# ebu/libear

Hardware: AMD Instinct MI355X
Metric: Msamples/s (higher is better)
Workload: dtype f32 io / f16x2-split MFMA, f32 accumulate

## Files before the change

include/earhip.h:

```cpp
#ifndef EARHIP_H
#define EARHIP_H

#include <stddef.h>
#include <stdint.h>

#ifdef __cplusplus
extern "C" {
#endif

#define EARHIP_VERSION 100

#define EARHIP_OK 0
#define EARHIP_INVALID_ARGUMENT 1
#define EARHIP_INTERNAL_ERROR 2
#define EARHIP_DEVICE_ERROR 3
#define EARHIP_NOT_IMPLEMENTED 4
#define EARHIP_UNKNOWN_LAYOUT 5
#define EARHIP_ADM_ERROR 6

int earhip_version(void);
const char *earhip_last_error(void);
int earhip_device_count(int *count);

typedef struct earhip_ctx earhip_ctx;
// ... 92 lines not shown

int earhip_layout_count(void);
const char *earhip_layout_name(int index);
int earhip_layout_num_channels(const char *layout, int *n_channels);
int earhip_layout_channel(const char *layout, int index, const char **name, double *azimuth,
                          double *elevation, int *is_lfe);
int earhip_layout_channel_ranges(const char *layout, int index, double azimuth_range[2],
                                 double elevation_range[2]);
int earhip_design_decorrelators_for_layout(const char *layout, int without_lfe, float *out);

typedef struct earhip_panner earhip_panner;
int earhip_panner_create(earhip_ctx *ctx, const char *layout, earhip_panner **out);
int earhip_panner_create_positions(earhip_ctx *ctx, const char *layout, int n_channels,
                                   const double *azimuth, const double *elevation,
                                   earhip_panner **out);
int earhip_panner_destroy(earhip_panner *p);
int earhip_panner_num_channels(const earhip_panner *p, int *n_channels);
int earhip_panner_calculate(earhip_panner *p, size_t npos, const double *azimuth,
                            const double *elevation, const double *distance, const double *gain,
                            const double *diffuse, float *direct, float *diffuse_out);
int earhip_panner_calculate_device(earhip_panner *p, size_t npos, const double *azimuth,
                                   const double *elevation, const double *distance,
                                   const double *gain, const double *diffuse, float *direct,
                                   float *diffuse_out);

int earhip_panner_calculate_extent(earhip_panner *p, size_t npos, const double *azimuth,
                                   const double *elevation, const double *distance,
                                   const double *width, const double *height, const double *depth,
                                   const double *gain, const double *diffuse, float *direct,
                                   float *diffuse_out);
int earhip_panner_calculate_extent_device(earhip_panner *p, size_t npos, const double *azimuth,
                                          const double *elevation, const double *distance,
                                          const double *width, const double *height,
                                          const double *depth, const double *gain,
                                          const double *diffuse, float *direct, float *diffuse_out);
int earhip_panner_missed(earhip_panner *p, unsigned *count);

int earhip_hoa_decode_matrix(earhip_ctx *ctx, const char *layout, int n_coef, const int *orders,
                             const int *degrees, const char *normalization, float *out);
int earhip_hoa_decode_matrix_positions(earhip_ctx *ctx, const char *layout, int n_channels,
                                       const double *azimuth, const double *elevation, int n_coef,
                                       const int *orders, const int *degrees,
                                       const char *normalization, float *out);

typedef struct earhip_direct_speakers earhip_direct_speakers;

typedef struct earhip_ds_metadata {
  int n_labels;
  const char *const *labels;
  int cartesian;
  double azimuth, elevation, distance;
  int has_azimuth_min, has_azimuth_max, has_elevation_min, has_elevation_max, has_distance_min,
      has_distance_max;
  double azimuth_min, azimuth_max, elevation_min, elevation_max, distance_min, distance_max;
  int screen_edge_lock_horizontal, screen_edge_lock_vertical;
  int has_low_pass, has_high_pass;
  double low_pass, high_pass;
  const char *audio_pack_format_id;
} earhip_ds_metadata;

int earhip_direct_speakers_create(earhip_ctx *ctx, const char *layout, int n_subst,
                                  const char *const *from, const char *const *to,
                                  earhip_direct_speakers **out);
int earhip_direct_speakers_create_positions(earhip_ctx *ctx, const char *layout, int n_channels,
                                            const double *azimuth, const double *elevation,
                                            int n_subst, const char *const *from,
                                            const char *const *to, earhip_direct_speakers **out);
int earhip_direct_speakers_destroy(earhip_direct_speakers *ds);
int earhip_direct_speakers_num_channels(const earhip_direct_speakers *ds, int *n_channels);
int earhip_direct_speakers_calculate(earhip_direct_speakers *ds, size_t n,
                                     const earhip_ds_metadata *md, float *gains,
                                     int *warnings_out);
int earhip_direct_speakers_missed(earhip_direct_speakers *ds, unsigned *count);

int earhip_conversion_to_polar(size_t n, const double *x, const double *y, const double *z,
                               const double *width, const double *height, const double *depth,
                               double *azimuth, double *elevation, double *distance,
                               double *width_out, double *height_out, double *depth_out);
int earhip_conversion_to_cartesian(size_t n, const double *azimuth, const double *elevation,
                                   const double *distance, const double *width,
                                   const double *height, const double *depth, double *x, double *y,
                                   double *z, double *width_out, double *height_out,
                                   double *depth_out);
int earhip_conversion_to_polar_device(earhip_ctx *ctx, size_t n, const double *x, const double *y,
                                      const double *z, const double *width, const double *height,
                                      const double *depth, double *azimuth, double *elevation,
                                      double *distance, double *width_out, double *height_out,
                                      double *depth_out, int *status);
int earhip_conversion_to_cartesian_device(earhip_ctx *ctx, size_t n, const double *azimuth,
                                          const double *elevation, const double *distance,
                                          const double *width, const double *height,
                                          const double *depth, double *x, double *y, double *z,
                                          double *width_out, double *height_out, double *depth_out,
                                          int *status);

typedef struct earhip_render earhip_render;

typedef struct earhip_render_config {
  int n_objects;
  int n_out;
  int block_size;
  int n_buses;
  const float *decorrelators;
  int n_taps;
  int delay;
  int max_blocks;
} earhip_render_config;

int earhip_render_create(earhip_ctx *ctx, const earhip_render_config *cfg,
                         earhip_render **out);
int earhip_render_destroy(earhip_render *r);
int earhip_render_set_object_points(earhip_render *r, int object, int npoints,
                                    const int64_t *times, const float *direct,
                                    const float *diffuse);
int earhip_render_commit(earhip_render *r);
int earhip_render_scratch_regrows(const earhip_render *r, long *count);
int earhip_render_reset(earhip_render *r, int64_t sample_time);
int earhip_render_process_device(earhip_render *r, size_t nblocks,
                                 const float *in_dev, size_t in_stride,
                                 float *out_dev, size_t out_stride);
int earhip_render_process(earhip_render *r, size_t nblocks, const float *const *in,
                          float *const *out);
typedef enum {
  EARHIP_PCM_S16 = 1,
  EARHIP_PCM_S24 = 2,
  EARHIP_PCM_S32 = 3,
  EARHIP_PCM_F32 = 4
} earhip_pcm_format;
int earhip_render_process_frames(earhip_render *r, size_t nblocks, const void *frames,
                                 earhip_pcm_format fmt, int frame_channels, int first_channel,
                                 float *const *out, int out_interleaved);
int earhip_render_process_frames_device(earhip_render *r, size_t nblocks, const void *frames_dev,
                                        earhip_pcm_format fmt, int frame_channels, int first_channel,
                                        float *out_dev, size_t out_stride, int out_interleaved);
typedef struct earhip_pcm_out {
  earhip_pcm_format format;
  int dither;
  uint32_t seed;
} earhip_pcm_out;
int earhip_render_process_frames_pcm(earhip_render *r, size_t nblocks, const void *frames,
                                     earhip_pcm_format fmt, int frame_channels, int first_channel,
                                     void *out_frames, const earhip_pcm_out *out);
int earhip_render_process_frames_pcm_device(earhip_render *r, size_t nblocks, const void *frames_dev,
                                            earhip_pcm_format fmt, int frame_channels,
                                            int first_channel, void *out_dev, size_t out_frame_bytes,
                                            size_t out_first_byte, const earhip_pcm_out *out);
int earhip_render_output_levels(earhip_render *r, float *peak, uint64_t *clipped, int reset);
int earhip_render_enable_timing(earhip_render *r, int enable);
int earhip_render_get_timing(earhip_render *r, double out[6]);
int earhip_render_gain_kernel(const earhip_render *r, int *kind);
int earhip_render_hinge_standby(earhip_render *r, int *standby);
int earhip_render_hinge_robust(earhip_render *r, int *robust);
int earhip_render_wide_form(earhip_render *r, int *wide);
int earhip_render_last_plan(const earhip_render *r, int out[4]);
int earhip_render_last_list_layout(const earhip_render *r, int *paired);
int earhip_render_last_tail_blocks(const earhip_render *r, int *blocks);
int earhip_render_last_host_chunks(const earhip_render *r, int *chunks);
int earhip_render_scratch_bytes(const earhip_render *r, size_t *bytes);

typedef struct earhip_comm earhip_comm;
int earhip_comm_unique_id(void *id128);
int earhip_comm_create(earhip_ctx *ctx, int rank, int world, const void *id128, earhip_comm **out);
int earhip_comm_destroy(earhip_comm *comm);
int earhip_comm_channel_range(int n_out, int rank, int world, int *padded_rows, int *lo, int *hi);
int earhip_render_exchange_device(earhip_comm *comm, int slot, const float *partial_dev,
                                  float *owned_dev, size_t rows_per_rank, size_t row_stride);
int earhip_comm_gather_device(earhip_comm *comm, int slot, const float *owned_dev, float *full_dev,
                              size_t rows_per_rank, size_t row_stride, int root);
int earhip_comm_wait(earhip_comm *comm, int slot);
int earhip_comm_last_exchange_ms(earhip_comm *comm, int slot, double *ms);
int earhip_comm_info(earhip_comm *comm, int info[4]);
int earhip_comm_link_probe(earhip_comm *comm, size_t bytes, int shift, int reps, double *GBps);

typedef struct earhip_loudness earhip_loudness;
int earhip_loudness_create(earhip_ctx *ctx, int n_channels, int sample_rate, const double *coeffs,
                           size_t max_steps, earhip_loudness **out);
typedef struct earhip_true_peak {
  int phases;
  int taps;
  const double *coeffs;
} earhip_true_peak;
int earhip_loudness_create_tp(earhip_ctx *ctx, int n_channels, int sample_rate, const double *coeffs,
                              size_t max_steps, const earhip_true_peak *tp, earhip_loudness **out);
int earhip_loudness_destroy(earhip_loudness *m);
int earhip_loudness_reset(earhip_loudness *m);
int earhip_loudness_process_device(earhip_loudness *m, size_t nsamples, const float *rows_dev, size_t stride);
int earhip_loudness_process(earhip_loudness *m, size_t nsamples, const float *const *rows);
int earhip_loudness_num_steps(earhip_loudness *m, size_t *steps);
int earhip_loudness_steps(earhip_loudness *m, size_t first, size_t n, double *energy);
int earhip_loudness_result(earhip_loudness *m, const double *weights, double *integrated,
                           double *max_momentary, double *max_short_term);
int earhip_loudness_peaks(earhip_loudness *m, float *true_peak, float *sample_peak);
int earhip_loudness_step_peaks(earhip_loudness *m, size_t first, size_t n, float *true_peak, float *sample_peak);
int earhip_loudness_result_range(earhip_loudness *m, const double *weights, double *lra, double *low,
                                 double *high);
int earhip_loudness_gate(size_t n_steps, int n_channels, const double *energy ,
                         const double *weights, double *integrated, double *max_momentary,
                         double *max_short_term);
int earhip_loudness_layout_weights(const char *layout, double *weights);
int earhip_loudness_range(size_t n_steps, int n_channels, const double *energy ,
                          const double *weights, double *lra, double *low, double *high);
int earhip_render_attach_loudness(earhip_render *r, earhip_loudness *m);

typedef struct earhip_firmix earhip_firmix;
typedef struct earhip_firmix_config {
  int n_in;
  int n_out;
  int block_size;
  int n_taps;
  const float *taps;
  int max_blocks;
} earhip_firmix_config;
int earhip_firmix_create(earhip_ctx *ctx, const earhip_firmix_config *config, earhip_firmix **out);
int earhip_firmix_destroy(earhip_firmix *fm);
int earhip_firmix_reset(earhip_firmix *fm);
int earhip_firmix_info(const earhip_firmix *fm, int info[5]);
int earhip_firmix_process_device(earhip_firmix *fm, size_t nblocks, const float *in_dev, size_t in_stride,
                                 float *out_dev, size_t out_stride);
int earhip_firmix_process(earhip_firmix *fm, size_t nblocks, const float *const *in, float *const *out);
int earhip_firmix_create_sets(earhip_ctx *ctx, const earhip_firmix_config *config, int n_sets, earhip_firmix **out);
int earhip_firmix_load_set(earhip_firmix *fm, int set, const float *taps);
int earhip_firmix_load_set_device(earhip_firmix *fm, int set, const float *taps_dev);
int earhip_firmix_select(earhip_firmix *fm, int set, int fade_blocks);
int earhip_firmix_state(const earhip_firmix *fm, int state[4]);
int earhip_firmix_set_info(const earhip_firmix *fm, int set, int info[2]);
int earhip_render_attach_firmix(earhip_render *r, earhip_firmix *fm, float *sink_dev, size_t sink_stride,
                                size_t sink_capacity);
int earhip_render_firmix_position(earhip_render *r, size_t *samples);

typedef struct earhip_limiter earhip_limiter;
typedef struct earhip_limiter_config {
  int n_channels;
  int sample_rate;
  float ceiling;
  int lookahead;
  int hold;
  int detect;
  const earhip_true_peak *tp;
  size_t max_samples;
} earhip_limiter_config;
int earhip_limiter_create(earhip_ctx *ctx, const earhip_limiter_config *config, earhip_limiter **out);
int earhip_limiter_destroy(earhip_limiter *lim);
int earhip_limiter_reset(earhip_limiter *lim);
int earhip_limiter_latency(const earhip_limiter *lim, int *samples);
int earhip_limiter_process_device(earhip_limiter *lim, size_t nsamples, const float *in_dev, size_t in_stride,
                                  float *out_dev, size_t out_stride, float *gain_dev);
int earhip_limiter_process(earhip_limiter *lim, size_t nsamples, const float *const *in, float *const *out,
                           float *gain);
int earhip_limiter_process_pcm_device(earhip_limiter *lim, size_t nsamples, const float *in_dev, size_t in_stride,
                                      void *out_dev, size_t out_frame_bytes, size_t out_first_byte,
                                      const earhip_pcm_out *out);
int earhip_limiter_output_levels(earhip_limiter *lim, float *peak, uint64_t *clipped, int reset);
int earhip_limiter_stats(earhip_limiter *lim, float *min_gain, uint64_t *limited_samples, int reset);
int earhip_render_attach_limiter(earhip_render *r, earhip_limiter *lim, float *sink_dev, size_t sink_stride,
                                 size_t sink_capacity);
int earhip_render_limiter_position(earhip_render *r, size_t *samples);

#ifdef __cplusplus
}
#endif
#endif
```

libear_amd/capi.py:

```python
import ctypes as C
import os

import numpy as np

from .build import lib_path

f32p = C.POINTER(C.c_float)
i64p = C.POINTER(C.c_int64)
pp_f32 = C.POINTER(f32p)

OK, INVALID_ARGUMENT, INTERNAL_ERROR, DEVICE_ERROR, NOT_IMPLEMENTED, UNKNOWN_LAYOUT, ADM_ERROR = 0, 1, 2, 3, 4, 5, 6


class EarHipError(Exception):
    def __init__(self, code, msg):
        super().__init__(msg)
        self.code = code


class InvalidArgument(EarHipError, ValueError):
    """maps to ear::invalid_argument"""


class InternalError(EarHipError, RuntimeError):
# ... 661 lines not shown

def pcm_format(fmt):
    name = _PCM_BY_CODE.get(fmt, fmt)
    if name not in _PCM:
        raise ValueError(f"unknown PCM format {fmt!r}")
    return _PCM[name]


class Renderer:

    def __init__(self, ctx, n_objects, n_out, block_size, decorrelators=None, delay=0, max_blocks=1):
        self.ctx = ctx
        self.M, self.N, self.B = n_objects, n_out, block_size
        self.K = 2 if decorrelators is not None else 1
        cfg = RenderConfig()
        cfg.n_objects, cfg.n_out, cfg.block_size, cfg.n_buses = n_objects, n_out, block_size, self.K
        if decorrelators is not None:
            self._dec = _f32(decorrelators).reshape(n_out, -1)
            cfg.decorrelators = _ptr(self._dec)
            cfg.n_taps = self._dec.shape[1]
        else:
            cfg.decorrelators = None
            cfg.n_taps = 0
        cfg.delay = delay
        cfg.max_blocks = max_blocks
        self.h = C.c_void_p()
        check(load().earhip_render_create(ctx.h, C.byref(cfg), C.byref(self.h)))

    def set_object_points(self, obj, times, direct, diffuse=None):
        t = np.ascontiguousarray(times, dtype=np.int64)
        d = _f32(direct).reshape(len(t), self.N)
        f = _f32(diffuse).reshape(len(t), self.N) if diffuse is not None else None
        check(load().earhip_render_set_object_points(self.h, obj, len(t), _ptr(t, i64p), _ptr(d),
                                                     _ptr(f) if f is not None else None))

    def commit(self):
        check(load().earhip_render_commit(self.h))

    def reset(self, sample_time=0):
        check(load().earhip_render_reset(self.h, C.c_int64(sample_time)))

    def process(self, x):
        x = _f32(x).reshape(self.M, -1)
        nblocks = x.shape[1] // self.B
        assert nblocks * self.B == x.shape[1]
        out = np.empty((self.N, x.shape[1]), np.float32)
        check(load().earhip_render_process(self.h, C.c_size_t(nblocks), _chan_ptrs(x), _chan_ptrs(out)))
        return out

    def process_into(self, x, out):
        assert x.dtype == np.float32 and out.dtype == np.float32 and x.flags["C_CONTIGUOUS"] and out.flags["C_CONTIGUOUS"]
        nblocks = x.shape[1] // self.B
        assert x.shape == (self.M, nblocks * self.B) and out.shape == (self.N, nblocks * self.B)
        check(load().earhip_render_process(self.h, C.c_size_t(nblocks), _chan_ptrs(x), _chan_ptrs(out)))
        return out

    def process_device(self, nblocks, in_ptr, in_stride, out_ptr, out_stride):
        check(load().earhip_render_process_device(self.h, C.c_size_t(nblocks), C.c_void_p(in_ptr),
                                                  C.c_size_t(in_stride), C.c_void_p(out_ptr),
                                                  C.c_size_t(out_stride)))

    def _frames_shape(self, x, fmt):
        code, dtype, cols = pcm_format(fmt)
        assert x.dtype == dtype and x.ndim == 2 and x.flags["C_CONTIGUOUS"], (x.dtype, dtype, x.shape)
        assert x.shape[1] % cols == 0
        frames, channels = x.shape[0], x.shape[1] // cols
        nblocks = frames // self.B
        assert nblocks * self.B == frames, "frames must be whole blocks"
        return code, nblocks, channels

    def process_frames(self, x, fmt, first_channel=0, interleaved_out=False):
        x = np.ascontiguousarray(x)
        frames = x.shape[0]
        out = np.empty((frames, self.N) if interleaved_out else (self.N, frames), np.float32)
        return self.process_frames_into(x, out, fmt, first_channel, interleaved_out)

    def process_frames_into(self, x, out, fmt, first_channel=0, interleaved_out=False):
        code, nblocks, channels = self._frames_shape(x, fmt)
        frames = nblocks * self.B
        assert out.dtype == np.float32 and out.flags["C_CONTIGUOUS"]
        assert out.shape == ((frames, self.N) if interleaved_out else (self.N, frames)), out.shape
        ptrs = (f32p * 1)(_ptr(out)) if interleaved_out else _chan_ptrs(out)
        check(load().earhip_render_process_frames(self.h, C.c_size_t(nblocks), C.c_void_p(x.ctypes.data), C.c_int(code),
                                                  C.c_int(channels), C.c_int(first_channel), ptrs, int(bool(interleaved_out))))
        return out

    def process_frames_device(self, nblocks, frames_ptr, fmt, frame_channels, first_channel, out_ptr, out_stride,
                              interleaved_out=False):
        code = pcm_format(fmt)[0] if isinstance(fmt, str) else int(fmt)
        check(load().earhip_render_process_frames_device(self.h, C.c_size_t(nblocks), C.c_void_p(frames_ptr), C.c_int(code),
                                                         C.c_int(frame_channels), C.c_int(first_channel), C.c_void_p(out_ptr),
                                                         C.c_size_t(out_stride), int(bool(interleaved_out))))

    def process_frames_pcm(self, x, fmt, first_channel=0, out_fmt="s16", dither=False, seed=0):
        x = np.ascontiguousarray(x)
        _, dtype, cols = pcm_format(out_fmt)
        out = np.empty((x.shape[0], self.N * cols), dtype)
        return self.process_frames_pcm_into(x, out, fmt, first_channel, out_fmt, dither, seed)

    def process_frames_pcm_into(self, x, out, fmt, first_channel=0, out_fmt="s16", dither=False, seed=0):
        code, nblocks, channels = self._frames_shape(x, fmt)
        ocode, dtype, cols = pcm_format(out_fmt)
        assert out.dtype == dtype and out.flags["C_CONTIGUOUS"] and out.shape == (nblocks * self.B, self.N * cols), out.shape
        spec = PcmOut(ocode, int(dither), int(seed) & 0xFFFFFFFF)
        check(load().earhip_render_process_frames_pcm(self.h, C.c_size_t(nblocks), C.c_void_p(x.ctypes.data), C.c_int(code),
                                                      C.c_int(channels), C.c_int(first_channel), C.c_void_p(out.ctypes.data),
                                                      C.byref(spec)))
        return out

    def process_frames_pcm_device(self, nblocks, frames_ptr, fmt, frame_channels, first_channel, out_ptr, out_frame_bytes,
                                  out_first_byte=0, out_fmt="s16", dither=False, seed=0):
        code = pcm_format(fmt)[0] if isinstance(fmt, str) else int(fmt)
        ocode = pcm_format(out_fmt)[0] if isinstance(out_fmt, str) else int(out_fmt)
        spec = PcmOut(ocode, int(dither), int(seed) & 0xFFFFFFFF)
        check(load().earhip_render_process_frames_pcm_device(self.h, C.c_size_t(nblocks), C.c_void_p(frames_ptr), C.c_int(code),
                                                             C.c_int(frame_channels), C.c_int(first_channel), C.c_void_p(out_ptr),
                                                             C.c_size_t(out_frame_bytes), C.c_size_t(out_first_byte),
                                                             C.byref(spec)))

    def output_levels(self, reset=False):
        peak, clipped = np.zeros(self.N, np.float32), np.zeros(self.N, np.uint64)
        check(load().earhip_render_output_levels(self.h, _ptr(peak), C.c_void_p(clipped.ctypes.data), int(bool(reset))))
        return peak, clipped

    def enable_timing(self, on=True):
        check(load().earhip_render_enable_timing(self.h, int(on)))

    def get_timing(self):
        out = (C.c_double * 6)()
        check(load().earhip_render_get_timing(self.h, out))
        return {"gain_mix_ms": out[0], "gain_mix_launches": out[1], "decor_ms": out[2],
                "decor_launches": out[3], "prep_ms": out[4], "prep_launches": out[5]}

    def gain_kernel(self):
        kind = C.c_int(-1)
        check(load().earhip_render_gain_kernel(self.h, C.byref(kind)))
        return kind.value

    def hinge_standby(self):
        flag = C.c_int(0)
        check(load().earhip_render_hinge_standby(self.h, C.byref(flag)))
        return bool(flag.value)

    def hinge_robust(self):
        flag = C.c_int(0)
        check(load().earhip_render_hinge_robust(self.h, C.byref(flag)))
        return bool(flag.value)

    def wide_form(self):
        flag = C.c_int(1)
        check(load().earhip_render_wide_form(self.h, C.byref(flag)))
        return None if flag.value < 0 else bool(flag.value)

    def scratch_bytes(self):
        v = C.c_size_t(0)
        check(load().earhip_render_scratch_bytes(self.h, C.byref(v)))
        return v.value

    def scratch_regrows(self):
        v = C.c_long(0)
        check(load().earhip_render_scratch_regrows(self.h, C.byref(v)))
        return v.value

    def last_tail_blocks(self):
        v = C.c_int(0)
        check(load().earhip_render_last_tail_blocks(self.h, C.byref(v)))
        return v.value

    def last_host_chunks(self):
        v = C.c_int(0)
        check(load().earhip_render_last_host_chunks(self.h, C.byref(v)))
        return v.value

    def last_list_layout(self):
        v = C.c_int(0)
        check(load().earhip_render_last_list_layout(self.h, C.byref(v)))
        return None if v.value < 0 else bool(v.value)

    def last_plan(self):
        out = (C.c_int * 4)()
        check(load().earhip_render_last_plan(self.h, out))
        return {"kernel": out[0], "tile": out[1], "ntiles": out[2], "gsplit": out[3]}

    def attach_loudness(self, meter):
        check(load().earhip_render_attach_loudness(self.h, meter.h if meter is not None else None))
        self._meter = meter

    def attach_fir_matrix(self, fm, sink_ptr=None, sink_stride=0, sink_capacity=0):
        check(load().earhip_render_attach_firmix(self.h, fm.h if fm is not None else None,
                                                 C.c_void_p(sink_ptr) if sink_ptr else None, C.c_size_t(sink_stride),
                                                 C.c_size_t(sink_capacity)))
        self._fir_matrix = fm

    def fir_matrix_position(self):
        v = C.c_size_t(0)
        check(load().earhip_render_firmix_position(self.h, C.byref(v)))
        return v.value

    def attach_limiter(self, lim, sink_ptr=None, sink_stride=0, sink_capacity=0):
        check(load().earhip_render_attach_limiter(self.h, lim.h if lim is not None else None,
                                                  C.c_void_p(sink_ptr) if sink_ptr else None, C.c_size_t(sink_stride),
                                                  C.c_size_t(sink_capacity)))
        self._limiter = lim

    def limiter_position(self):
        v = C.c_size_t(0)
        check(load().earhip_render_limiter_position(self.h, C.byref(v)))
        return v.value

    def close(self):
        if self.h:
            load().earhip_render_destroy(self.h)
            self.h = C.c_void_p()



def _f64(a):
    return np.ascontiguousarray(a, dtype=np.float64)


def loudness_gate(energy, weights):
    w = _f64(weights).reshape(-1)
    e = _f64(energy).reshape(-1, w.size)
    out = [C.c_double(0) for _ in range(3)]
    check(load().earhip_loudness_gate(C.c_size_t(e.shape[0]), C.c_int(w.size), C.c_void_p(e.ctypes.data), C.c_void_p(w.ctypes.data),
                                      *[C.byref(v) for v in out]))
    return tuple(v.value for v in out)


def loudness_range(energy, weights):
    w = _f64(weights).reshape(-1)
    e = _f64(energy).reshape(-1, w.size)
    out = [C.c_double(0) for _ in range(3)]
    check(load().earhip_loudness_range(C.c_size_t(e.shape[0]), C.c_int(w.size), C.c_void_p(e.ctypes.data), C.c_void_p(w.ctypes.data),
                                       *[C.byref(v) for v in out]))
    return tuple(v.value for v in out)


class _TruePeak(C.Structure):
    _fields_ = [("phases", C.c_int), ("taps", C.c_int), ("coeffs", C.c_void_p)]


def loudness_layout_weights(layout):
    n = C.c_int(0)
    check(load().earhip_layout_num_channels(layout.encode(), C.byref(n)))
    w = np.zeros(n.value, np.float64)
    check(load().earhip_loudness_layout_weights(layout.encode(), C.c_void_p(w.ctypes.data)))
    return w


class Loudness:

    def __init__(self, ctx, n_channels, sample_rate=48000, max_steps=36000, coeffs=None, true_peak=False):
        self.ctx, self.C = ctx, n_channels
        c = None if coeffs is None else _f64(coeffs).reshape(2, 5)
        self.h = C.c_void_p()
        kc = None if c is None else C.c_void_p(c.ctypes.data)
        if true_peak is False or true_peak is None:
            check(load().earhip_loudness_create(ctx.h, C.c_int(n_channels), C.c_int(sample_rate), kc, C.c_size_t(max_steps),
                                                C.byref(self.h)))
            return
        if true_peak is True:
            tp = _TruePeak(0, 0, None)
        else:
            phases, taps, table = true_peak
            table = _f64(table).reshape(-1)
            if table.size != max(int(phases), 0) * max(int(taps), 0):
                raise InvalidArgument(INVALID_ARGUMENT, "the true-peak table must be [phases][taps]")
            if table.size == 0:
                table = np.zeros(1)
            tp = _TruePeak(int(phases), int(taps), table.ctypes.data)
        check(load().earhip_loudness_create_tp(ctx.h, C.c_int(n_channels), C.c_int(sample_rate), kc, C.c_size_t(max_steps),
                                               C.byref(tp), C.byref(self.h)))

    def process(self, x):
        x = _f32(x).reshape(self.C, -1)
        check(load().earhip_loudness_process(self.h, C.c_size_t(x.shape[1]), _chan_ptrs(x)))

    def process_device(self, nsamples, rows_ptr, stride):
        check(load().earhip_loudness_process_device(self.h, C.c_size_t(nsamples), C.c_void_p(rows_ptr), C.c_size_t(stride)))

    def num_steps(self):
        v = C.c_size_t(0)
        check(load().earhip_loudness_num_steps(self.h, C.byref(v)))
        return v.value

    def steps(self, first=0, n=None):
        if n is None:
            n = self.num_steps() - first
        e = np.zeros((n, self.C), np.float64)
        check(load().earhip_loudness_steps(self.h, C.c_size_t(first), C.c_size_t(n), C.c_void_p(e.ctypes.data)))
        return e

    def result(self, weights):
        w = _f64(weights).reshape(self.C)
        out = [C.c_double(0) for _ in range(3)]
        check(load().earhip_loudness_result(self.h, C.c_void_p(w.ctypes.data), *[C.byref(v) for v in out]))
        return tuple(v.value for v in out)

    def peaks(self):
        t, s = np.zeros(self.C, np.float32), np.zeros(self.C, np.float32)
        check(load().earhip_loudness_peaks(self.h, C.c_void_p(t.ctypes.data), C.c_void_p(s.ctypes.data)))
        return t, s

    def step_peaks(self, first=0, n=None):
        if n is None:
# ... 174 lines not shown
```

libear_amd/csrc/api_core.hip:

```cpp
#include <cctype>
#include <cerrno>
#include <cmath>
#include <cstdlib>
#include <string>
#include <memory>
#include <mutex>

#include "common.h"
#include "curves.h"
#include "gain_kernels.h"
#include "gain_mfma.h"
#include "gain_h2.h"
#include "gain_h2_t1.h"
#include "gain_p2.h"
#include "gain_hg.h"
#include "gain_f32g.h"

namespace earhip {

static_assert(kSplitTile == 256, "MixLaunch::tile() and tiles_aligned(256, ...) assume the 4-wave tile");

static thread_local std::string g_last_error;
void set_last_error(const std::string &msg) { g_last_error = msg; }

size_t mix_lds_bytes(const ColumnPlan &cp, const MixLaunch &ml) {
  if (ml.wsplit <= 1 || ml.split || ml.pieces || ml.hinge) return 0;
  if (ml.mfma) return (size_t)cp.mgroups * ml.tpw * cp.nct * 16 * ml.tile() * sizeof(float);
  return (size_t)cp.ngroups * cp.nout * ml.tile() * sizeof(float);
}

template <int NCT, int NRT>
static void launch_mfma_t(const GainMixParams &P, dim3 grid, dim3 block, size_t lds,
                          hipStream_t s) {
  hipLaunchKernelGGL((k_gain_mix_mfma<NCT, NRT>), grid, block, lds, s, P);
}

template <int NOUT, int SPL, bool STRICT>
static void launch_mix_t(const GainMixParams &P, dim3 grid, dim3 block, size_t lds,
                         hipStream_t s) {
  hipLaunchKernelGGL((k_gain_mix<NOUT, SPL, STRICT>), grid, block, lds, s, P);
}

void launch_gain_mix(earhip_ctx *ctx, const CurveSet &cs, const MixLaunch &ml, bool strict,
                     int64_t t_call, int nsamples, const float *in_dev, size_t in_stride,
                     float *out_dev, size_t out_stride, size_t part_stride, SegDesc *desc,
                     hipEvent_t *ev) {
  const ColumnPlan &cp = cs.plan();
  const PointStore ps = cs.device();
  const int M = cs.M();
  const bool slots = ml.mfma && !ml.split && !ml.pieces && !ml.hinge && !ml.f32grid;
  if (slots && M > kMaxSlotObjects) fail_internal("slot lists address objects with 16 bits");
  if (ev) EARHIP_HIP(hipEventRecord(ev[0], ctx->stream));
  const bool fused_prep = slots && (size_t)ps.npoints <= (size_t)8 * M;
  LevelProbe probe;
  unsigned *level_cur = nullptr, *level_next = nullptr;
  unsigned *wide_cur = nullptr, *wide_next = nullptr;
  unsigned *gate = nullptr;
  ctx->last_gate_idx = -1;
  ctx->last_wide_idx = -1;
  unsigned *const record = ctx->record_slot;
  ctx->record_slot = nullptr;
  const bool hg_robust = ml.hinge && ctx->get(OPT_HG_ROBUST, 1) != 0;
  if ((ml.split || ml.pieces || ml.hinge) && ctx->x_scale_auto && in_stride % 4 == 0 && ((uintptr_t)in_dev & 15) == 0) {
    if (!ctx->level.p) ctx->level.alloc_zero(4, ctx->stream), ctx->lazy_allocs++;
    level_cur = ctx->level.p + ctx->level_idx;
    level_next = ctx->level.p + (ctx->level_idx ^ 1);
    if ((size_t)ml.ntiles * ml.gsplit >= 2 * (size_t)ctx->num_cus) wide_cur = ctx->level.p + 2 + ctx->level_idx;
    wide_next = ctx->level.p + 2 + (ctx->level_idx ^ 1);
    gate = ctx->level.p + 2 + ctx->level_idx;
    ctx->last_gate_idx = ml.hinge ? ctx->level_idx : -1;
    ctx->last_hinge_robust = hg_robust;
    ctx->last_wide_idx = wide_cur ? ctx->level_idx : -1;
    ctx->level_idx ^= 1;
    if (ctx->obj_level_cap < M) {
      EARHIP_HIP(hipStreamSynchronize(ctx->stream));
      ctx->obj_level_cap = M + M / 2 + 64;
      ctx->obj_level.alloc_zero(2 * (size_t)ctx->obj_level_cap, ctx->stream);
      ctx->lazy_allocs++;
    }
    probe.obj_level = ctx->obj_level.p;
    probe.level = level_cur;
    const int probe_runs = [&] {
      const int v = ctx->get(OPT_PROBE_RUNS);
      return v >= 1 && v <= 64 && (v & (v - 1)) == 0 ? v : 16;
    }();
    hipLaunchKernelGGL(k_level_probe, dim3((M + kProbeObjects - 1) / kProbeObjects), dim3(64 * kProbeObjects), 0, ctx->stream, in_dev,
                       in_stride, nsamples, M, level_cur, ctx->obj_level.p, ctx->obj_level_cap, probe_runs);
  }
  PieceLists pl;
  pl.pieces = reinterpret_cast<Piece *>(desc);
  pl.M = M;
  pl.paired = ml.paired ? 1 : 0;
  const int ptile = ml.hinge ? 64 * ml.pw : ml.tile();
  const int pnt = ml.hinge ? (nsamples + ptile - 1) / ptile : ml.ntiles;
  pl.slots = cs.piece_cap(ptile, ml.paired);
  pl.count = reinterpret_cast<int *>(pl.pieces + (size_t)pl.cap() * pnt);
  pl.ovf = pl.count + (size_t)8 * pnt;
  unsigned *slow_cur = nullptr, *slow_next = nullptr;
  if (ml.split) {
    if (ctx->tile_slow_cap < (size_t)ml.ntiles) {
      EARHIP_HIP(hipStreamSynchronize(ctx->stream));
      ctx->tile_slow_cap = std::max<size_t>(2 * (size_t)ml.ntiles, 1024);
      ctx->tile_slow.alloc_zero(2 * ctx->tile_slow_cap, ctx->stream);
      ctx->lazy_allocs++;
    }
    slow_cur = ctx->tile_slow.p + (size_t)ctx->tile_slow_idx * ctx->tile_slow_cap;
    slow_next = ctx->tile_slow.p + (size_t)(ctx->tile_slow_idx ^ 1) * ctx->tile_slow_cap;
    ctx->tile_slow_idx ^= 1;
  }
  HingeLists hl = hinge_lists(desc, M, ml.ntiles);
  if (ml.hinge) {
    if (M > kMaxHingeCached || (ml.tile() != 256 && ml.tile() != 512)) fail_internal("hinge lists: object count or tile out of range");
    if (!ps.kink_row0) fail_internal("hinge kernel: the curve set has no kink rows");
    if (!hinge_addressable(M, in_stride, nsamples, (size_t)ps.kink_row0 + ps.rows, ps.row)) fail_internal("hinge kernel: buffers beyond its 32-bit offsets");
    unsigned *obj_lv = probe.obj_level;
    if (gate) hipLaunchKernelGGL(k_hinge_gate, dim3((M + 255) / 256), dim3(256), 0, ctx->stream, obj_lv, ctx->obj_level_cap, M, level_cur, gate, wide_cur != nullptr, hg_robust);
    int tpw = 1;
    const size_t cached_max = std::min((size_t)kMaxHingeCached, ctx->hinge_build_lds / sizeof(HingeCached));
    if ((size_t)M > cached_max) fail_internal("hinge lists: more objects than the builder's LDS holds on this device");
    while (tpw < 8 && ml.ntiles / (2 * tpw) >= ctx->num_cus && (size_t)M * (2 * tpw) <= cached_max) tpw *= 2;
    if (ctx->has(OPT_HBUILD_TPW)) {
      const int v = ctx->get(OPT_HBUILD_TPW);
      if ((v == 1 || v == 2 || v == 4 || v == 8) && (size_t)M * v <= cached_max) tpw = v;
    }
    const HingeCached *stage = nullptr;
    if (ctx->get(OPT_BUILD_2K, 0) != 0) {
      HingeCached *st = reinterpret_cast<HingeCached *>(desc) + hinge_units((size_t)M, (size_t)ml.ntiles);
      stage = st;
      const dim3 cgrid((ml.ntiles + 63) / 64, (M + kClassifyObjects - 1) / kClassifyObjects);
      if (ml.tile() == 256)
        hipLaunchKernelGGL((k_hinge_classify<4>), cgrid, dim3(64 * kClassifyObjects), 0, ctx->stream, ps, M, ml.ntiles, t_call, t_call + nsamples, st,
                           obj_lv, level_cur, hg_robust ? nullptr : gate, hg_robust ? gate : nullptr);
      else
        hipLaunchKernelGGL((k_hinge_classify<8>), cgrid, dim3(64 * kClassifyObjects), 0, ctx->stream, ps, M, ml.ntiles, t_call, t_call + nsamples, st,
                           obj_lv, level_cur, hg_robust ? nullptr : gate, hg_robust ? gate : nullptr);
      if (!ctx->has(OPT_HBUILD_TPW)) {
        tpw = 1;
        while (tpw < 8 && ml.ntiles / (2 * tpw) >= 2 * ctx->num_cus) tpw *= 2;
      }
    }
    const dim3 bgrid((ml.ntiles + tpw - 1) / tpw);
    const size_t lds = stage ? 0 : sizeof(HingeCached) * (size_t)M * tpw;
#define EARHIP_HBUILD_ONE(T_, NW_)                                                                                    \
  hipLaunchKernelGGL((k_hinge_build<T_, NW_>), bgrid, dim3(kHingeBuildThreads), lds, ctx->stream, ps, M, ml.ntiles, t_call, \
                     t_call + nsamples, hl, obj_lv, level_cur, hg_robust ? nullptr : gate, hg_robust ? gate : nullptr, stage);
#define EARHIP_HBUILD_CASE(T_)                                                                                        \
  if (tpw == T_) {                                                                                                    \
    if (ml.tile() == 256) EARHIP_HBUILD_ONE(T_, 4)                                                                    \
    else EARHIP_HBUILD_ONE(T_, 8)                                                                                     \
  }
    EARHIP_HBUILD_CASE(1) EARHIP_HBUILD_CASE(2) EARHIP_HBUILD_CASE(4) EARHIP_HBUILD_CASE(8)
#undef EARHIP_HBUILD_CASE
#undef EARHIP_HBUILD_ONE
  }
  const bool one_pass = ml.pieces || ml.hinge;
  if (ml.pieces || (ml.hinge && gate && !hg_robust)) {
    if (M > kMaxPieceObjects || ptile > kPieceMaxTile) fail_internal("piece lists: object index or tile out of range");
    unsigned *obj_lv = probe.obj_level;
    int tpw = 1;
    while (tpw < 8 && pnt / (2 * tpw) >= ctx->num_cus) tpw *= 2;
    if (ctx->has(OPT_BUILD_TPW)) {
      const int v = ctx->get(OPT_BUILD_TPW);
      if (v == 1 || v == 2 || v == 4 || v == 8) tpw = v;
    }
    const dim3 bgrid((pnt + tpw - 1) / tpw);
    PairRec *stage = nullptr;
    if (ctx->has(OPT_BUILD_2K) ? ctx->get(OPT_BUILD_2K) != 0 : ml.paired) {
      stage = reinterpret_cast<PairRec *>(desc) + piece_units((size_t)M, (size_t)pnt, (size_t)pl.slots);
      hipLaunchKernelGGL(k_piece_classify, dim3((pnt + 63) / 64, (M + kClassifyObjects - 1) / kClassifyObjects), dim3(64 * kClassifyObjects), 0,
                         ctx->stream, ps, M, pnt, ptile, t_call, t_call + nsamples, pl.paired, stage, obj_lv, level_cur,
                         ml.hinge ? gate : nullptr);
    }
#define EARHIP_BUILD_CASE(T_)                                                                                          \
  if (tpw == T_)                                                                                                       \
    hipLaunchKernelGGL(k_piece_build<T_>, bgrid, dim3(kBuildThreads), 0, ctx->stream, ps, M, pnt, ptile, t_call, \
                       t_call + nsamples, pl, obj_lv, level_cur, ml.hinge ? gate : nullptr, ctx->obj_level_cap, wide_cur, stage);
    EARHIP_BUILD_CASE(1) EARHIP_BUILD_CASE(2) EARHIP_BUILD_CASE(4) EARHIP_BUILD_CASE(8)
#undef EARHIP_BUILD_CASE
  }
  if (!fused_prep && !one_pass) {
    const dim3 ogrid((M + 15) / 16);
    QuietMark qm;
    if (probe.obj_level) {
      qm.obj_level = probe.obj_level, qm.cap = ctx->obj_level_cap, qm.level = level_cur;
      qm.wide = ml.split ? wide_cur : nullptr;
    }
    if (ml.ntiles >= 2048)
      hipLaunchKernelGGL(k_seg_prep<4>, dim3((ml.ntiles + 63) / 64, ogrid.x), dim3(256), 0, ctx->stream, ps, M,
                         ml.ntiles, ml.tile(), t_call, t_call + nsamples, desc, qm, slow_cur);
    else
      hipLaunchKernelGGL(k_seg_prep<2>, dim3((ml.ntiles + 31) / 32, ogrid.x), dim3(256), 0, ctx->stream, ps, M,
                         ml.ntiles, ml.tile(), t_call, t_call + nsamples, desc, qm, slow_cur);
  }
  SlotLists sl;
  sl.slots = reinterpret_cast<Slot *>(desc + (size_t)M * ml.ntiles);
  sl.count = reinterpret_cast<int *>(sl.slots + (size_t)kTileSlots * M * ml.ntiles);
  sl.ovf = sl.count + (size_t)4 * ml.ntiles;
  sl.M = M;
  if (slots)
    hipLaunchKernelGGL(k_slot_list, dim3(ml.ntiles), dim3(256), 0, ctx->stream, ps, M, ml.tile(),
                       t_call, t_call + nsamples, fused_prep ? nullptr : desc, sl);
  if (ev) EARHIP_HIP(hipEventRecord(ev[1], ctx->stream));
  GainMixParams P;
  P.mode_word = gate;
  P.record = gate ? record : nullptr;
  P.sl = sl;
  P.in = in_dev;
  P.in_stride = in_stride;
  P.out = out_dev;
  P.out_stride = out_stride;
  P.part_stride = part_stride;
  P.desc = desc;
  P.ps = ps;
  P.t_call = t_call;
  P.nsamples = nsamples;
  P.ntiles = ml.ntiles;
  P.M = M;
  P.ncols = cs.ncols();
  P.ngroups = ml.mfma ? cp.mgroups : cp.ngroups;
  P.wsplit = ml.wsplit;
  P.tiles_per_wg = ml.mfma ? ml.tpw : 1;
  P.vec_ok = (in_stride % 4 == 0 && out_stride % 4 == 0 && part_stride % 4 == 0 &&
              ((uintptr_t)in_dev & 15) == 0 && ((uintptr_t)out_dev & 15) == 0)
                 ? 1
                 : 0;
  const dim3 grid(ml.mfma ? (ml.ntiles + ml.tpw - 1) / ml.tpw : ml.ntiles, ml.gsplit,
                  ml.mfma ? cp.mnz : cp.nz);
  const dim3 block(64 * P.ngroups * P.tiles_per_wg * ml.wsplit);
  const size_t lds = mix_lds_bytes(cp, ml);
  if (ev) EARHIP_HIP(hipEventRecord(ev[2], ctx->stream));
  bool launched = false;
  if (ml.hinge) {
    const dim3 bgrid(ml.ntiles, ml.gsplit, cp.mnz * cp.mgroups);
    const float xs = std::ldexp(1.0f, ctx->x_scale_log2);
    const float *gs = cs.column_scales();
#define EARHIP_HG_LAUNCH(NCT_, NW_)                                                                                  \
  hipLaunchKernelGGL((k_gain_mix_hg<NCT_, NW_>), bgrid, dim3(64 * NW_), 0, ctx->stream, P, hl, xs, gs, level_cur,     \
                     level_next, wide_cur, wide_next, hg_robust ? nullptr : gate, hg_robust ? gate : nullptr);
#define EARHIP_HG_CASE(NCT_)                                                                                          \
  if (cp.nct == NCT_) {                                                                                               \
    if (ml.tile() == 256) EARHIP_HG_LAUNCH(NCT_, 4)                                                                   \
    else EARHIP_HG_LAUNCH(NCT_, 8)                                                                                    \
  }
    EARHIP_HG_CASE(1) EARHIP_HG_CASE(2) EARHIP_HG_CASE(3)
#undef EARHIP_HG_CASE
#undef EARHIP_HG_LAUNCH
    launched = true;
  }
  if (ml.pieces || (ml.hinge && gate && !hg_robust)) {
    int wgs = std::max(8, (ctx->num_cus * (ml.pw == 4 ? 2 : 1) / std::max(1, ml.gsplit * cp.mnz * cp.mgroups)) & ~7);
    if (ctx->has(OPT_P2_WGS)) wgs = ctx->get(OPT_P2_WGS) > 0 ? ctx->get(OPT_P2_WGS) : pnt;
    if (!p2_persistent(cp.nct, ml.pw, ml.paired)) wgs = pnt;
    const dim3 bgrid(std::min(pnt, wgs), ml.gsplit, cp.mnz * cp.mgroups);
    const float xs = std::ldexp(1.0f, ctx->x_scale_log2);
    const float *gs = cs.column_scales();
#define EARHIP_P2_LAUNCH(NCT_, NW_, PR_)                                                                             \
  hipLaunchKernelGGL((k_gain_mix_p2<NCT_, NW_, PR_>), bgrid, dim3(64 * NW_), 0, ctx->stream, P, pl, xs, gs,         \
                     level_cur, level_next, wide_cur, wide_next, ml.hinge ? gate : nullptr, pnt);
#define EARHIP_P2_CASE(NCT_, PR_)                                                                                   \
  if (cp.nct == NCT_ && ml.paired == PR_) {                                                                         \
    if (ml.pw == 4) EARHIP_P2_LAUNCH(NCT_, 4, PR_)                                                                  \
    else EARHIP_P2_LAUNCH(NCT_, 8, PR_)                                                                             \
  }
    EARHIP_P2_CASE(1, false) EARHIP_P2_CASE(2, false) EARHIP_P2_CASE(3, false)
    EARHIP_P2_CASE(1, true) EARHIP_P2_CASE(2, true) EARHIP_P2_CASE(3, true)
#undef EARHIP_P2_CASE
#undef EARHIP_P2_LAUNCH
    launched = true;
  }
  if (ml.f32grid) {
    if (nsamples % kF32GridTile != 0) fail_internal("f32 grid kernel: the call is not whole tiles");
    const dim3 bgrid(ml.ntiles, ml.gsplit, cp.mnz * cp.mgroups);
#define EARHIP_F32G_CASE(NCT_)                                                                       \
  if (cp.nct == NCT_) hipLaunchKernelGGL((k_gain_mix_f32g<NCT_>), bgrid, dim3(512), 0, ctx->stream, P, ps.zero_row);
    EARHIP_F32G_CASE(1) EARHIP_F32G_CASE(2) EARHIP_F32G_CASE(3)
#undef EARHIP_F32G_CASE
    launched = true;
  }
  if (ml.split) {
    const int per_cu = ml.tile() == 512 ? 1 : (cp.nct == 1 ? 3 : 2);
    int wgs = std::max(8, (ctx->num_cus * per_cu / std::max(1, ml.gsplit * cp.mnz * cp.mgroups)) & ~7);
    if (ctx->has(OPT_H2_WGS)) wgs = std::max(1, ctx->get(OPT_H2_WGS));
    wgs = std::max(wgs, ((ml.ntiles + 63) / 64 + 7) & ~7);
    P.tile_runs = ctx->has(OPT_H2_RUNS) ? (ctx->get(OPT_H2_RUNS) != 0) : 0;
    if (!h2_persistent(cp.nct, ml.tile() == 512 ? 8 : 4)) wgs = ml.ntiles;
    const dim3 bgrid(std::min(ml.ntiles, wgs), ml.gsplit, cp.mnz * cp.mgroups);
    const float xs = std::ldexp(1.0f, ctx->x_scale_log2);
    const float *gs = cs.column_scales();
    const bool two_launches = ctx->get(OPT_H2_PAIR, 0) != 0;
#define EARHIP_H2_LAUNCH(NCT_, NW_, WIDE_)                                                                          \
  hipLaunchKernelGGL((k_gain_mix_h2<NCT_, NW_, WIDE_>), bgrid, dim3(64 * NW_), 0, ctx->stream, P, ps.zero_row, xs,  \
                     gs, level_cur, level_next, slow_cur, slow_next, wide_cur, wide_next);
#define EARHIP_H2T1_LAUNCH(NCT_, NW_, WIDE_)                                                                        \
  hipLaunchKernelGGL((k_gain_mix_h2_t1<NCT_, NW_, WIDE_>), bgrid, dim3(64 * NW_), 0, ctx->stream, P, ps.zero_row, xs, \
                     gs, level_cur, level_next, slow_cur, slow_next, wide_cur, wide_next);
#define EARHIP_H2_CASE(NCT_)                                                                                        \
  if (cp.nct == NCT_) {                                                                                             \
    if (ml.tile() == 512) {                                                                                         \
      if (wide_cur && !two_launches) EARHIP_H2_LAUNCH(NCT_, 8, 2)                                                   \
      else {                                                                                                        \
        if (wide_cur) EARHIP_H2_LAUNCH(NCT_, 8, 0)                                                                  \
        EARHIP_H2_LAUNCH(NCT_, 8, 1)                                                                                \
      }                                                                                                             \
    } else if (NCT_ == 1) {                                                                                         \
      if (wide_cur) EARHIP_H2_LAUNCH(1, 4, 0)                                                                       \
      EARHIP_H2_LAUNCH(1, 4, 1)                                                                                     \
    } else {                                                                                                        \
      if (wide_cur) EARHIP_H2T1_LAUNCH(NCT_, 4, false)                                                              \
      EARHIP_H2T1_LAUNCH(NCT_, 4, true)                                                                             \
    }                                                                                                               \
  }
    EARHIP_H2_CASE(1) EARHIP_H2_CASE(2) EARHIP_H2_CASE(3)
#undef EARHIP_H2_CASE
#undef EARHIP_H2_LAUNCH
#undef EARHIP_H2T1_LAUNCH
    launched = true;
  }
#define EARHIP_MIX_CASE(NOUT_, SPL_, STRICT_)                                   \
  if (cp.nout == NOUT_ && ml.spl == SPL_ && strict == STRICT_) {                 \
    launch_mix_t<NOUT_, SPL_, STRICT_>(P, grid, block, lds, ctx->stream);        \
    launched = true;                                                             \
  }
#define EARHIP_MFMA_CASE(NCT_, NRT_)                                            \
  if (slots && cp.nct == NCT_ && ml.nrt == NRT_) {                                          \
    launch_mfma_t<NCT_, NRT_>(P, grid, block, lds, ctx->stream);                 \
    launched = true;                                                             \
  }
  EARHIP_MFMA_CASE(1, 8) EARHIP_MFMA_CASE(2, 8) EARHIP_MFMA_CASE(3, 8)
  EARHIP_MFMA_CASE(1, 4) EARHIP_MFMA_CASE(2, 4) EARHIP_MFMA_CASE(3, 4)
#undef EARHIP_MFMA_CASE
  if (!ml.mfma && !launched) {
  EARHIP_MIX_CASE(8, 4, false) EARHIP_MIX_CASE(8, 4, true)
  EARHIP_MIX_CASE(16, 4, false) EARHIP_MIX_CASE(16, 4, true)
  EARHIP_MIX_CASE(24, 4, false) EARHIP_MIX_CASE(24, 4, true)
  EARHIP_MIX_CASE(8, 2, false) EARHIP_MIX_CASE(8, 2, true)
  EARHIP_MIX_CASE(16, 2, false) EARHIP_MIX_CASE(16, 2, true)
  EARHIP_MIX_CASE(24, 2, false) EARHIP_MIX_CASE(24, 2, true)
  }
#undef EARHIP_MIX_CASE
  if (!launched) fail_internal("no gain_mix instantiation for this column plan");
  if (ev) EARHIP_HIP(hipEventRecord(ev[3], ctx->stream));
  EARHIP_HIP(hipGetLastError());
}

void reserve_call_words(earhip_ctx *ctx, int M, size_t max_samples) {
  if (!ctx->level.p) ctx->level.alloc_zero(4, ctx->stream);
  const size_t ntiles = (max_samples + 255) / 256;
  const bool grow_obj = ctx->obj_level_cap < M, grow_tiles = ctx->tile_slow_cap < ntiles;
  if (grow_obj || grow_tiles) EARHIP_HIP(hipStreamSynchronize(ctx->stream));
  if (grow_obj) {
    ctx->obj_level_cap = M + M / 2 + 64;
    ctx->obj_level.alloc_zero(2 * (size_t)ctx->obj_level_cap, ctx->stream);
  }
  if (grow_tiles) {
    ctx->tile_slow_cap = std::max<size_t>(ntiles + ntiles / 4, 1024);
    ctx->tile_slow.alloc_zero(2 * ctx->tile_slow_cap, ctx->stream);
    ctx->tile_slow_idx = 0;
  }
}

size_t hinge_build_allow_lds(const hipDeviceProp_t &prop) {
  const size_t want = 128 * 1024, dflt = 64 * 1024;
  const size_t device_max = std::max((size_t)prop.sharedMemPerBlock, (size_t)prop.maxSharedMemoryPerMultiProcessor);
  size_t ask = std::min(want, device_max > 4096 ? device_max - 4096 : dflt);
  if (ask <= dflt) return dflt;
  bool ok = true;
#define EARHIP_HBUILD_ATTR(T_, NW_)                                                                       \
  ok = ok && hipFuncSetAttribute(reinterpret_cast<const void *>(&k_hinge_build<T_, NW_>),                 \
                                 hipFuncAttributeMaxDynamicSharedMemorySize, (int)ask) == hipSuccess;
  EARHIP_HBUILD_ATTR(1, 4) EARHIP_HBUILD_ATTR(2, 4) EARHIP_HBUILD_ATTR(4, 4) EARHIP_HBUILD_ATTR(8, 4)
  EARHIP_HBUILD_ATTR(1, 8) EARHIP_HBUILD_ATTR(2, 8) EARHIP_HBUILD_ATTR(4, 8) EARHIP_HBUILD_ATTR(8, 8)
#undef EARHIP_HBUILD_ATTR
  if (!ok) (void)hipGetLastError();
  return ok ? ask : dflt;
}

struct GainStage {
  earhip_ctx *ctx;
  int n_in, n_out;
  CurveSet curves;
  DevBuf<SegDesc> desc;
  DevBuf<float> parts;
  std::vector<float> rows;
  bool force_ramp;
  GainStage(earhip_ctx *c, int ni, int no, bool ramp = false)
      : ctx(c), n_in(ni), n_out(no), curves(ni, no, 1, ramp), force_ramp(ramp) {}

  void run_device(int64_t t_call, int nsamples, const float *in_dev, size_t in_stride,
                  float *out_dev, size_t out_stride) {
    curves.commit(ctx);
    const bool strict = ctx->strict || n_in == 1 || force_ramp;
    MixLaunch ml = plan_mix(ctx, curves.plan(), n_in, nsamples, strict, 32,
                            curves.aligned_tile(t_call), curves.ramp_share(), curves.gain_scale(), curves.point_density_all(),
                            curves.pair_waste(256), curves.pair_waste(512), curves.hinge_exact_share(in_stride, (size_t)nsamples), false,
                            curves.deltas_per_pair(256));
    if (ml.hinge) curves.ensure_kinks(ctx);
    desc.reserve(scratch_units(curves, ml, n_in));
    if (ml.gsplit == 1) {
      launch_gain_mix(ctx, curves, ml, strict, t_call, nsamples, in_dev, in_stride, out_dev,
                      out_stride, 0, desc.p, nullptr);
    } else {
      const size_t row_stride = ((size_t)nsamples + 3) & ~(size_t)3;
      const size_t part_stride = row_stride * n_out;
      parts.reserve(part_stride * ml.gsplit);
      launch_gain_mix(ctx, curves, ml, strict, t_call, nsamples, in_dev, in_stride, parts.p,
                      row_stride, part_stride, desc.p, nullptr);
      hipLaunchKernelGGL(k_sum_parts, dim3((nsamples + 255) / 256, n_out), dim3(256), 0,
                         ctx->stream, parts.p, part_stride, ml.gsplit, row_stride, n_out,
                         nsamples, out_dev, out_stride);
      EARHIP_HIP(hipGetLastError());
    }
  }

  void run_host(int64_t t_call, const float *const *in, float *const *out, int64_t r0,
                int64_t r1) {
    const int n = (int)(r1 - r0);
    if (n <= 0) return;
    const size_t stride = ((size_t)n + 3) & ~(size_t)3;
    ctx->pin_in.reserve(stride * n_in);
    ctx->pin_out.reserve(stride * n_out);
    ctx->dev_in.reserve(stride * n_in);
    ctx->dev_out.reserve(stride * n_out);
    for (int c = 0; c < n_in; c++)
      std::memcpy(ctx->pin_in.p + c * stride, in[c] + r0, sizeof(float) * n);
    EARHIP_HIP(hipMemcpyAsync(ctx->dev_in.p, ctx->pin_in.p, sizeof(float) * stride * n_in,
                              hipMemcpyHostToDevice, ctx->stream));
    run_device(t_call, n, ctx->dev_in.p, stride, ctx->dev_out.p, stride);
    EARHIP_HIP(hipMemcpyAsync(ctx->pin_out.p, ctx->dev_out.p, sizeof(float) * stride * n_out,
                              hipMemcpyDeviceToHost, ctx->stream));
    EARHIP_HIP(hipStreamSynchronize(ctx->stream));
    for (int c = 0; c < n_out; c++)
      std::memcpy(out[c] + r0, ctx->pin_out.p + c * stride, sizeof(float) * n);
  }
};

}

using namespace earhip;

static const char *const kOptNames[OPT_COUNT] = {
    "SPL", "MFMA", "XSCALE", "WAVES", "TPW", "NRT", "H2_TILE", "H2_WGS", "H2_RUNS", "P2_TILE", "P2_PAIRS", "P2_WGS", "HINGE", "HG_TILE", "HBUILD_TPW",
    "BUILD_TPW", "K2_WG", "K2_OWN_BLOCK", "RUN", "GSPLIT", "PROBE_RUNS", "BLOCK_GROUPS", "DEBUG_TIMING", "TAILCUT", "HOST_CHUNK_MB", "HOST_THREADS", "HG_ROBUST", "BUILD_2K", "HOST_BIND", "HOST_NT", "HOST_FIRST", "H2_PAIR"};

static int parse_option_value(const std::string &key, const char *text) {
  char *end = nullptr;
  errno = 0;
  const long v = std::strtol(text, &end, 10);
  while (end && *end && std::isspace((unsigned char)*end)) end++;
  if (end == text || (end && *end) || errno == ERANGE || v < -(1L << 30) || v > (1L << 30))
    fail_invalid("option '" + key + "': '" + std::string(text) + "' is not an integer");
  return (int)v;
}

void earhip_ctx::apply_options() {
  spl = 4, use_mfma = 3, x_scale_log2 = 14, x_scale_auto = true, max_waves = 4, tiles_per_wg = 4, tiles_per_wg_forced = false, nrt = 8;
  if (has(OPT_SPL) && (get(OPT_SPL) == 2 || get(OPT_SPL) == 4)) spl = get(OPT_SPL);
  if (has(OPT_MFMA)) use_mfma = get(OPT_MFMA);
  if (has(OPT_XSCALE) && get(OPT_XSCALE) >= -64 && get(OPT_XSCALE) <= 64)
    x_scale_log2 = get(OPT_XSCALE), x_scale_auto = false;
  if (has(OPT_WAVES) && get(OPT_WAVES) >= 1 && get(OPT_WAVES) <= 8) max_waves = get(OPT_WAVES);
  if (has(OPT_TPW) && get(OPT_TPW) >= 1 && get(OPT_TPW) <= 8) tiles_per_wg = get(OPT_TPW), tiles_per_wg_forced = true;
  if (has(OPT_NRT) && (get(OPT_NRT) == 4 || get(OPT_NRT) == 8)) nrt = get(OPT_NRT);
}

struct earhip_gain_interp {
  std::unique_ptr<GainStage> stage;
};

struct PolicyCache {
  std::vector<std::unique_ptr<GainStage>> stages;
  GainStage *get(earhip_ctx *ctx, int n_in, int n_out, bool ramp) {
    for (auto &s : stages)
      if (s->n_in == n_in && s->n_out == n_out && s->force_ramp == ramp) return s.get();
    stages.emplace_back(new GainStage(ctx, n_in, n_out, ramp));
    return stages.back().get();
  }
};
static std::vector<std::pair<earhip_ctx *, std::unique_ptr<PolicyCache>>> g_policy;
static std::mutex g_policy_mutex;
static PolicyCache *policy_cache(earhip_ctx *ctx) {
  std::lock_guard<std::mutex> lock(g_policy_mutex);
  for (auto &p : g_policy)
    if (p.first == ctx) return p.second.get();
  g_policy.emplace_back(ctx, std::unique_ptr<PolicyCache>(new PolicyCache));
  return g_policy.back().second.get();
}

static __global__ void k_clock_probe(unsigned long long *out) {
  out[0] = clock64();
  out[1] = wall_clock64();
}

static __global__ void __launch_bounds__(256) k_read_linear(const f32x4 *in, float *out, size_t n4) {
  f32x4 acc = {0.0f, 0.0f, 0.0f, 0.0f};
  size_t i = (size_t)blockIdx.x * 256 + threadIdx.x;
  const size_t step = (size_t)gridDim.x * 256;
  for (; i + 3 * step < n4; i += 4 * step) {
    const f32x4 a = __builtin_nontemporal_load(in + i), b = __builtin_nontemporal_load(in + i + step);
    const f32x4 c = __builtin_nontemporal_load(in + i + 2 * step), d = __builtin_nontemporal_load(in + i + 3 * step);
    acc += (a + b) + (c + d);
  }
  for (; i < n4; i += step) acc += __builtin_nontemporal_load(in + i);
  if (acc[0] + acc[1] + acc[2] + acc[3] == 123.456f) out[0] = 1.0f;
}
static __global__ void __launch_bounds__(256) k_read_rows(const float *in, float *out, int rows, size_t stride) {
  constexpr int DEPTH = 4;
  const int lane = threadIdx.x & 63, w = threadIdx.x >> 6, li = lane & 15, kg = lane >> 4;
  const float *base = in + (size_t)blockIdx.x * 256 + w * 64 + li * 4;
  auto row = [&](int r) { return base + (size_t)min(r, rows - 1) * stride; };
  f32x4 acc = {0.0f, 0.0f, 0.0f, 0.0f};
  f32x4 ring[DEPTH][8];
#pragma unroll
  for (int d = 0; d < DEPTH; d++)
#pragma unroll
    for (int q = 0; q < 8; q++)
      ring[d][q] = __builtin_nontemporal_load((const f32x4 *)row(d * 32 + kg * 8 + q));
  for (int r0 = 0; r0 < rows; r0 += 32 * DEPTH) {
#pragma unroll
    for (int d = 0; d < DEPTH; d++) {
#pragma unroll
      for (int q = 0; q < 8; q++) acc += ring[d][q];
      const int rn = r0 + 32 * DEPTH + d * 32;
      if (rn < rows)
#pragma unroll
        for (int q = 0; q < 8; q++)
          ring[d][q] = __builtin_nontemporal_load((const f32x4 *)row(rn + kg * 8 + q));
    }
  }
  if (acc[0] + acc[1] + acc[2] + acc[3] == 123.456f) out[0] = 1.0f;
}

extern "C" {

int earhip_debug_read_bandwidth(earhip_ctx *ctx, const float *in_dev, size_t rows, size_t stride,
                                size_t nsamples, int reps, double ms[2]) {
  return guarded([&] {
    require(ctx != nullptr && in_dev != nullptr && ms != nullptr, "NULL argument");
    require(rows >= 1 && rows < ((size_t)1 << 24) && reps >= 1 && reps <= 1000, "rows / reps out of range");
    require(stride % 256 == 0 && nsamples % 256 == 0 && nsamples >= 256 && nsamples <= stride &&
                ((uintptr_t)in_dev & 15) == 0,
            "buffer must be 16-byte aligned with stride and nsamples multiples of 256");
    ctx->use();
    if (!ctx->level.p) ctx->level.alloc_zero(4, ctx->stream);
    float *sink = reinterpret_cast<float *>(ctx->level.p);
    hipEvent_t e[4];
    for (auto &x : e) EARHIP_HIP(hipEventCreate(&x));
    const size_t n4 = rows * stride / 4;
    const unsigned lin_blocks = (unsigned)std::min<size_t>((n4 + 255) / 256, (size_t)ctx->num_cus * 32);
    auto linear = [&] {
      hipLaunchKernelGGL(k_read_linear, dim3(lin_blocks), dim3(256), 0, ctx->stream,
                         reinterpret_cast<const f32x4 *>(in_dev), sink, n4);
    };
    auto pattern = [&] {
      hipLaunchKernelGGL(k_read_rows, dim3((unsigned)(nsamples / 256)), dim3(256), 0, ctx->stream, in_dev, sink,
                         (int)rows, stride);
    };
    linear();
    EARHIP_HIP(hipEventRecord(e[0], ctx->stream));
    for (int i = 0; i < reps; i++) linear();
    EARHIP_HIP(hipEventRecord(e[1], ctx->stream));
    pattern();
    EARHIP_HIP(hipEventRecord(e[2], ctx->stream));
    for (int i = 0; i < reps; i++) pattern();
    EARHIP_HIP(hipEventRecord(e[3], ctx->stream));
    EARHIP_HIP(hipGetLastError());
    EARHIP_HIP(hipEventSynchronize(e[3]));
    float t = 0.0f;
    EARHIP_HIP(hipEventElapsedTime(&t, e[0], e[1]));
    ms[0] = (double)t / reps;
    EARHIP_HIP(hipEventElapsedTime(&t, e[2], e[3]));
    ms[1] = (double)t / reps;
    for (auto &x : e) (void)hipEventDestroy(x);
  });
}

int earhip_debug_copy_bandwidth(earhip_ctx *ctx, void *host, size_t bytes, int reps, double ms[2]) {
  return guarded([&] {
    require(ctx != nullptr && host != nullptr && ms != nullptr, "NULL argument");
    require(bytes >= 4 && reps >= 1 && reps <= 1000, "bytes / reps out of range");
    ctx->use();
    DevBuf<char> dev;
    dev.alloc(bytes);
    hipEvent_t e[2];
    for (auto &x : e) EARHIP_HIP(hipEventCreate(&x));
    for (int dir = 0; dir < 2; dir++) {
      auto copy = [&] {
        if (dir == 0) EARHIP_HIP(hipMemcpyAsync(dev.p, host, bytes, hipMemcpyHostToDevice, ctx->stream));
        else EARHIP_HIP(hipMemcpyAsync(host, dev.p, bytes, hipMemcpyDeviceToHost, ctx->stream));
      };
      copy();
      EARHIP_HIP(hipEventRecord(e[0], ctx->stream));
      for (int i = 0; i < reps; i++) copy();
      EARHIP_HIP(hipEventRecord(e[1], ctx->stream));
      EARHIP_HIP(hipEventSynchronize(e[1]));
      float t = 0.0f;
// ... 336 lines not shown
```

libear_amd/csrc/api_render.hip:

```cpp
#include <cmath>
#include <cstdlib>
#include <atomic>
#include <chrono>
#include <condition_variable>
#include <memory>
#include <mutex>
#include <thread>
#include <vector>


#include "common.h"
#include "curves.h"
#include "host_gather.h"
#include "pcm_kernels.h"
#include "pcm_out_kernels.h"
#include "fft_kernels.h"
#include "render_kernels.h"

using namespace earhip;

namespace earhip {
std::vector<cf> make_twiddles(int L) {
  std::vector<cf> tw(L);
  const double pi = 3.14159265358979323846264338327950288;
// ... 87 lines not shown
  std::vector<std::thread> threads;
  std::mutex mu;
  std::condition_variable go, finished_cv;
  uint64_t generation = 0;
  int finished = 0;
  bool quit = false;
  const float *const *in = nullptr;
  float *dst = nullptr;
  size_t n = 0;
  size_t cstart[kMaxGroups + 1] = {0};
  int M = 0, groups = 0;
  const unsigned char *src_bytes = nullptr;
  unsigned char *dst_bytes = nullptr;
  size_t unit = 0;
  std::atomic<int> done[kMaxGroups];
  int nthreads() const { return (int)threads.size(); }
  size_t group_len(int g) const { return cstart[g + 1] - cstart[g]; }
  void start(int count) {
    for (int t = 0; t < count; t++)
      threads.emplace_back([this, t] {
        uint64_t seen = 0;
        int my_node = -1;
        for (;;) {
          int want_node;
          const cpu_set_t *want_cpus;
          {
            std::unique_lock<std::mutex> lk(mu);
            go.wait(lk, [&] { return quit || generation != seen; });
            if (quit) return;
            seen = generation;
            want_node = job_node, want_cpus = job_cpus;
          }
          if (want_node != my_node) {
            if (want_node >= 0 && want_cpus) {
              if (sched_setaffinity(0, sizeof(cpu_set_t), want_cpus) == 0) my_node = want_node;
            } else if (numa.ok && sched_setaffinity(0, sizeof(cpu_set_t), &numa.allowed) == 0) {
              my_node = -1;
            }
          }
          const int nt = nthreads();
          for (int g = 0; g < groups; g++) {
            const size_t len = group_len(g), at = cstart[g];
            float *base = dst + (size_t)M * at;
            if (src_bytes) {
              size_t lo, hi;
              range_slice(len * unit, t, nt, &lo, &hi);
              const size_t o = at * unit + lo;
              if (hi > lo) {
                if (streaming) stream_copy_bytes(dst_bytes + o, src_bytes + o, hi - lo);
                else std::memcpy(dst_bytes + o, src_bytes + o, hi - lo);
              }
#if defined(__x86_64__)
              if (streaming) _mm_sfence();
#endif
            } else if (streaming) {
              for (int m = t; m < M; m += nt) stream_copy(base + (size_t)m * len, in[m] + at, len);
#if defined(__x86_64__)
              _mm_sfence();
#endif
            } else {
              for (int m = t; m < M; m += nt) std::memcpy(base + (size_t)m * len, in[m] + at, sizeof(float) * len);
            }
            done[g].fetch_add(1, std::memory_order_release);
          }
          std::lock_guard<std::mutex> lk(mu);
          if (++finished == nt) finished_cv.notify_one();
        }
      });
  }
  void submit(const float *const *in_, float *dst_, size_t n_, const size_t *starts, int nchunks, int M_, bool bind, bool nt) {
    const int node = bind && numa.ok ? NumaMap::rows_node(in_, M_, n_) : -1;
    std::lock_guard<std::mutex> lk(mu);
    in = in_, dst = dst_, n = n_, M = M_;
    src_bytes = nullptr;
    for (int g = 0; g <= nchunks; g++) cstart[g] = starts[g];
    streaming = nt;
    job_cpus = numa.cpus_of(node);
    job_node = job_cpus ? node : -1;
    groups = nchunks;
    for (auto &d : done) d.store(0);
    finished = 0;
    generation++;
    go.notify_all();
  }
  void submit_range(const void *src, void *dst_, size_t unit_, const size_t *starts, int nchunks, bool bind, bool nt) {
    const int node = bind && numa.ok ? NumaMap::range_node(src, starts[nchunks] * unit_) : -1;
    std::lock_guard<std::mutex> lk(mu);
    src_bytes = static_cast<const unsigned char *>(src), dst_bytes = static_cast<unsigned char *>(dst_), unit = unit_;
    in = nullptr, dst = nullptr, n = starts[nchunks], M = 0;
    for (int g = 0; g <= nchunks; g++) cstart[g] = starts[g];
    streaming = nt;
    job_cpus = numa.cpus_of(node);
    job_node = job_cpus ? node : -1;
    groups = nchunks;
    for (auto &d : done) d.store(0);
    finished = 0;
    generation++;
    go.notify_all();
  }
  void wait_all() {
    std::unique_lock<std::mutex> lk(mu);
    finished_cv.wait(lk, [&] { return finished == nthreads(); });
  }
  ~GatherPool() {
    {
      std::lock_guard<std::mutex> lk(mu);
      quit = true;
    }
    go.notify_all();
    for (auto &th : threads) th.join();
  }
};

struct StreamPipe {
  hipStream_t in = nullptr, out = nullptr;
  hipEvent_t ev_in[GatherPool::kMaxGroups], ev_k[GatherPool::kMaxGroups], ev_out[GatherPool::kMaxGroups];
  bool made = false;
  void make() {
    if (made) return;
    EARHIP_HIP(hipStreamCreateWithFlags(&in, hipStreamNonBlocking));
    EARHIP_HIP(hipStreamCreateWithFlags(&out, hipStreamNonBlocking));
    for (int i = 0; i < GatherPool::kMaxGroups; i++) {
      EARHIP_HIP(hipEventCreateWithFlags(&ev_in[i], hipEventDisableTiming));
      EARHIP_HIP(hipEventCreateWithFlags(&ev_k[i], hipEventDisableTiming));
      EARHIP_HIP(hipEventCreateWithFlags(&ev_out[i], hipEventDisableTiming));
    }
    made = true;
  }
  ~StreamPipe() {
    if (!made) return;
    for (int i = 0; i < GatherPool::kMaxGroups; i++) {
      (void)hipEventDestroy(ev_in[i]);
      (void)hipEventDestroy(ev_k[i]);
      (void)hipEventDestroy(ev_out[i]);
    }
    (void)hipStreamDestroy(in);
    (void)hipStreamDestroy(out);
  }
};

struct earhip_render {
  earhip_ctx *ctx = nullptr;
  int M = 0, N = 0, B = 0, K = 1, D = 0, T = 0;
  int Bk = 0, Lk = 0;
  int NP = 1;
  std::unique_ptr<CurveSet> curves;
  int64_t t = 0;
  int last_plan[3] = {0, 0, 0};
  int last_paired = -1;
  size_t last_scratch_bytes = 0;
  long scratch_regrows = 0;
  DevBuf<unsigned> rec;
  bool last_gated = false;
  bool last_device_form = false;
  bool last_hg_robust = false;
  int last_kind = -1;
  int run_len = 11;
  bool run_len_set = false;

  DevBuf<SegDesc> desc;
  DevBuf<float> bus;
  int max_gsplit = 1;
  DevBuf<cf> H, tw;
  DevBuf<float> tail[2], dly[2], hist[2];
  DevBuf<float> ztail, zdly, zhist;
  bool fresh = true;
  int cur = 0;
  DevBuf<float> d_in, d_out;
  PinBuf<float> p_in, p_out;
  std::unique_ptr<GatherPool> gather;
  StreamPipe pipe;
  int last_host_chunks = 0;
  PinBuf<unsigned char> p_bytes;
  DevBuf<unsigned char> d_bytes;
  DevBuf<float> d_ilv, d_rows, d_rows_out;
  DevBuf<unsigned char> d_pcm;
  PinBuf<unsigned char> p_pcm;
  DevBuf<unsigned> d_peak;
  DevBuf<unsigned long long> d_clip;
  bool timing = false;
  bool last_timed = false;
  int timing_every = 1;
  long timing_calls = 0;
  hipEvent_t ev[6] = {nullptr, nullptr, nullptr, nullptr, nullptr, nullptr};
  struct Pending { hipEvent_t e[6]; bool has_k2; bool continues; };
  std::vector<Pending> pending;
  std::vector<hipEvent_t> pool;
  double acc_ms[3] = {0, 0, 0};
  double acc_n[3] = {0, 0, 0};

  ~earhip_render() {
    for (auto &p : pending)
      for (auto e : p.e)
        if (e) (void)hipEventDestroy(e);
    for (auto e : pool) (void)hipEventDestroy(e);
  }

  hipEvent_t get_event() {
    if (!pool.empty()) {
      hipEvent_t e = pool.back();
      pool.pop_back();
      return e;
    }
    hipEvent_t e;
    EARHIP_HIP(hipEventCreate(&e));
    return e;
  }

  void drain_timing() {
    EARHIP_HIP(hipStreamSynchronize(ctx->stream));
    for (auto &p : pending) {
      float ms = 0;
      const double one = p.continues ? 0.0 : 1.0;
      EARHIP_HIP(hipEventElapsedTime(&ms, p.e[0], p.e[1]));
      acc_ms[2] += ms; acc_n[2] += one;
      EARHIP_HIP(hipEventElapsedTime(&ms, p.e[2], p.e[3]));
      acc_ms[0] += ms; acc_n[0] += one;
      if (p.has_k2) {
        EARHIP_HIP(hipEventElapsedTime(&ms, p.e[4], p.e[5]));
        acc_ms[1] += ms; acc_n[1] += one;
      }
      for (auto e : p.e)
        if (e) pool.push_back(e);
    }
    pending.clear();
  }

  size_t direct_stride(const float *const *ch, int count, size_t n) const {
    if (ctx->host_ranges.empty() || count < 1) return 0;
    const uintptr_t a0 = (uintptr_t)ch[0];
    const uintptr_t step = count > 1 ? (uintptr_t)ch[1] - a0 : sizeof(float) * n;
    if ((a0 & 15) != 0 || step % 16 != 0 || step < sizeof(float) * n || step > ((uintptr_t)1 << 40)) return 0;
    for (int c = 1; c < count; c++)
      if ((uintptr_t)ch[c] - (uintptr_t)ch[c - 1] != step) return 0;
    return ctx->host_reachable(ch[0], step * (count - 1) + sizeof(float) * n) ? (size_t)(step / sizeof(float)) : 0;
  }

  void reserve_levels() {
    if (d_peak.p) return;
    EARHIP_HIP(hipStreamSynchronize(ctx->stream));
    d_peak.alloc_zero((size_t)kLevelSlots * N, ctx->stream);
    d_clip.alloc_zero((size_t)kLevelSlots * N, ctx->stream);
  }
  void zero_levels() {
    if (!d_peak.p) return;
    EARHIP_HIP(hipMemsetAsync(d_peak.p, 0, sizeof(unsigned) * kLevelSlots * N, ctx->stream));
    EARHIP_HIP(hipMemsetAsync(d_clip.p, 0, sizeof(unsigned long long) * kLevelSlots * N, ctx->stream));
  }
  void reserve_pcm_out(size_t bytes, bool pinned) {
    reserve_levels();
    d_pcm.reserve(bytes);
    if (pinned) p_pcm.reserve(bytes);
  }

  HostChunkPlan host_plan(size_t nblocks, bool direct) const {
    return plan_host_chunks(nblocks, B, M, direct, ctx->has(OPT_HOST_CHUNK_MB), ctx->get(OPT_HOST_CHUNK_MB), ctx->get(OPT_HOST_FIRST, 0));
  }

  MixLaunch plan_call(size_t nblocks, size_t in_stride) {
    const int nsamples = (int)(nblocks * (size_t)B);
    MixLaunch ml = plan_mix(ctx, curves->plan(), M, nsamples, ctx->strict, max_gsplit, curves->aligned_tile(t),
                            curves->ramp_share(), curves->gain_scale(), curves->point_density_all(), curves->pair_waste(256), curves->pair_waste(512),
                            curves->hinge_exact_share(in_stride, (size_t)nsamples), curves->tiles_aligned(kF32GridTile, t),
                            curves->deltas_per_pair(256));
    const size_t bus_stride = ((size_t)nsamples + 3) & ~(size_t)3;
    while (ml.gsplit > 1 && bus_stride * K * N * ml.gsplit > bus.n) ml.gsplit /= 2;
    return ml;
  }

  size_t last_in_stride = 0;
  void reserve_for_curves() {
    size_t need = 0;
    bool hinge = false;
    const size_t lens[3] = {(size_t)T, (size_t)std::max(1, T / 2), (size_t)1};
    for (size_t nb : lens) {
      const MixLaunch ml = plan_call(nb, last_in_stride ? last_in_stride : nb * (size_t)B);
      need = std::max(need, scratch_units(*curves, ml, M));
      hinge = hinge || ml.hinge;
    }
    if (hinge) curves->ensure_kinks(ctx);
    if (need > desc.n) {
      EARHIP_HIP(hipStreamSynchronize(ctx->stream));
      desc.reserve(need + need / 4);
    }
  }

  int resident_workgroups(const MixLaunch &ml) const {
    if (!(ml.split || ml.pieces || ml.hinge)) return 0;
    return ctx->num_cus * (ml.tile() >= 512 ? 1 : 2);
  }

  earhip_loudness *meter = nullptr;
  void check_meter(size_t nblocks) const {
    if (meter) loudness_check_room(meter, nblocks * (size_t)B);
  }
  earhip_firmix *fm = nullptr;
  float *fm_sink = nullptr;
  size_t fm_sink_stride = 0, fm_sink_cap = 0, fm_pos = 0;
  void check_firmix(size_t nblocks) const {
    if (!fm) return;
    firmix_check_room(fm, nblocks);
    if (fm_pos + nblocks * (size_t)B > fm_sink_cap)
      fail_invalid("the call would pass the FIR matrix's sink_capacity (nothing was rendered)");
  }
  earhip_limiter *lim = nullptr;
  float *lim_sink = nullptr;
  size_t lim_sink_stride = 0, lim_sink_cap = 0, lim_pos = 0;
  void check_limiter(size_t nblocks) const {
    if (!lim) return;
    limiter_check_room(lim, nblocks * (size_t)B);
    if (lim_pos + nblocks * (size_t)B > lim_sink_cap)
      fail_invalid("the call would pass the limiter's sink_capacity (nothing was rendered)");
  }
  void process_device(size_t nblocks, const float *in_dev, size_t in_stride, float *out_dev, size_t out_stride) {
    if (!meter && !fm && !lim) return render_spans(nblocks, in_dev, in_stride, out_dev, out_stride);
    if (meter) loudness_check_room(meter, nblocks * (size_t)B);
    check_firmix(nblocks);
    check_limiter(nblocks);
    render_spans(nblocks, in_dev, in_stride, out_dev, out_stride);
    if (meter) loudness_feed(meter, nblocks * (size_t)B, out_dev, out_stride);
    if (fm) {
      firmix_feed(fm, nblocks, out_dev, out_stride, fm_sink + fm_pos, fm_sink_stride);
      fm_pos += nblocks * (size_t)B;
    }
    if (lim) {
      limiter_feed(lim, nblocks * (size_t)B, out_dev, out_stride, lim_sink + lim_pos, lim_sink_stride);
      lim_pos += nblocks * (size_t)B;
    }
  }
  void render_spans(size_t nblocks, const float *in_dev, size_t in_stride, float *out_dev, size_t out_stride) {
    MixLaunch whole;
    bool have_plan = false;
    if (!ctx->strict && ctx->get(OPT_TAILCUT, 1) != 0 && nblocks >= 2) {
      last_in_stride = in_stride;
      if (curves->dirty()) {
        curves->commit(ctx);
        reserve_for_curves();
      }
      const MixLaunch ml = whole = plan_call(nblocks, in_stride);
      have_plan = true;
      const int W = resident_workgroups(ml);
      if (W > 0 && ml.gsplit == 1 && ml.ntiles > W) {
        const size_t tile = (size_t)ml.tile();
        const size_t full = (size_t)ml.ntiles / (size_t)W, rest = (size_t)ml.ntiles % (size_t)W;
        const size_t main_samples = full * (size_t)W * tile;
        const size_t eighths = (size_t)std::min(std::max(ctx->get(OPT_TAILCUT, 2), 0), 7);
        if (rest > 0 && rest <= (size_t)W * eighths / 8 && main_samples % (size_t)B == 0) {
          const size_t main_blocks = main_samples / (size_t)B;
          process_span(main_blocks, in_dev, in_stride, out_dev, out_stride, false);
          const int kind = last_kind, plan3[3] = {last_plan[0], last_plan[1], last_plan[2]};
          const size_t scratch = last_scratch_bytes;
          const bool gated = last_gated, device_form = last_device_form, hg_robust = last_hg_robust;
          const int paired = last_paired;
          process_span(nblocks - main_blocks, in_dev + main_samples, in_stride, out_dev + main_samples, out_stride, true);
          last_kind = kind;
          last_gated = gated, last_device_form = device_form, last_paired = paired, last_hg_robust = hg_robust;
          for (int i = 0; i < 3; i++) last_plan[i] = plan3[i];
          last_scratch_bytes = scratch;
          last_tail_blocks = (int)(nblocks - main_blocks);
          return;
        }
      }
    }
    last_tail_blocks = 0;
    process_span(nblocks, in_dev, in_stride, out_dev, out_stride, false, have_plan ? &whole : nullptr);
  }
  int last_tail_blocks = 0;

  void process_span(size_t nblocks, const float *in_dev, size_t in_stride, float *out_dev,
                    size_t out_stride, bool continues, const MixLaunch *planned = nullptr) {
    const int nsamples = (int)(nblocks * (size_t)B);
    last_in_stride = in_stride;
    if (curves->dirty()) {
      curves->commit(ctx);
      reserve_for_curves();
    }
    const bool strict = ctx->strict;
    MixLaunch ml = planned ? *planned : plan_call(nblocks, in_stride);
    if (ml.hinge) curves->ensure_kinks(ctx);

    last_kind = ml.f32grid ? 2 : ml.hinge ? 5 : ml.pieces ? 4 : ml.split ? 3 : ml.mfma ? 1 : 0;
    {
      const size_t need = scratch_units(*curves, ml, M);
      if (need > desc.n) {
        EARHIP_HIP(hipStreamSynchronize(ctx->stream));
        desc.reserve(need + need / 2);
        scratch_regrows++;
      }
      last_scratch_bytes = need * 16;
    }
    const size_t bus_stride = ((size_t)nsamples + 3) & ~(size_t)3;
    const size_t part_stride = bus_stride * K * N;
    if (part_stride * ml.gsplit > bus.n) fail_internal("bus buffer too small for this launch plan");
    last_paired = (ml.pieces || ml.hinge) ? (ml.paired ? 1 : 0) : -1;
    last_plan[0] = ml.tile();
    last_plan[1] = ml.ntiles;
    last_plan[2] = ml.gsplit;
    Pending pd;
    hipEvent_t *evp = nullptr;
    const bool timed = timing && (continues ? last_timed : (timing_calls++ % timing_every) == 0);
    last_timed = timed;
    if (timed) {
      for (int i = 0; i < 6; i++) pd.e[i] = get_event();
      pd.has_k2 = K == 2;
      pd.continues = continues;
      evp = pd.e;
    }
    const long lazy_before = ctx->lazy_allocs;
    ctx->record_slot = rec.p + (continues ? 1 : 0);
    if (K == 1) {
      if (ml.gsplit == 1) {
        launch_gain_mix(ctx, *curves, ml, strict, t, nsamples, in_dev, in_stride, out_dev,
                        out_stride, 0, desc.p, evp);
      } else {
        launch_gain_mix(ctx, *curves, ml, strict, t, nsamples, in_dev, in_stride, bus.p,
                        bus_stride, part_stride, desc.p, evp);
        hipLaunchKernelGGL(k_sum_parts, dim3((nsamples + 255) / 256, N), dim3(256), 0,
                           ctx->stream, bus.p, part_stride, ml.gsplit, bus_stride, N, nsamples,
                           out_dev, out_stride);
        EARHIP_HIP(hipGetLastError());
      }
    } else {
      launch_gain_mix(ctx, *curves, ml, strict, t, nsamples, in_dev, in_stride, bus.p,
                      bus_stride, part_stride, desc.p, evp);
      DecorParams P;
      P.bus = bus.p;
      P.bus_stride = bus_stride;
      P.part_stride = part_stride;
      P.nparts = ml.gsplit;
      const bool wave_k2 = Lk == 1024 && NP == 1 && !ctx->get(OPT_K2_WG);
      const int kblocks = (int)(nblocks * (size_t)(B / Bk));
      if (wave_k2 && ml.gsplit > 1) {
        if (evp) EARHIP_HIP(hipEventRecord(evp[4], ctx->stream));
        hipLaunchKernelGGL(k_sum_parts, dim3((nsamples + 255) / 256, K * N), dim3(256), 0, ctx->stream, bus.p,
                           part_stride, ml.gsplit, bus_stride, K * N, nsamples, bus.p, bus_stride);
        EARHIP_HIP(hipGetLastError());
        P.nparts = 1;
      }
      P.out = out_dev;
      P.out_stride = out_stride;
      P.tw = tw.p;
      P.dly_in = fresh ? zdly.p : dly[cur].p;
      P.dly_out = dly[cur ^ 1].p;
      P.N = N;
      P.T = kblocks;
      const int R = wave_k2 && !run_len_set ? wave_run_len(kblocks, N, ctx->num_cus) : run_len;
      P.R = R;
      P.D = D;
      P.hist_len = (NP - 1) * Bk;
      P.hist_in = fresh ? zhist.p : hist[cur].p;
      P.hist_out = hist[cur ^ 1].p;
      const dim3 grid((unsigned)((kblocks + R - 1) / R), N);
      if (evp && P.nparts == ml.gsplit) EARHIP_HIP(hipEventRecord(evp[4], ctx->stream));
      for (int part = 0; part < NP; part++) {
        P.H = H.p + (size_t)part * N * Lk;
        P.tail_in = (fresh ? ztail.p : tail[cur].p) + (fresh ? 0 : (size_t)part * N * Bk);
        P.tail_out = tail[cur ^ 1].p + (size_t)part * N * Bk;
        P.shift = part * Bk;
        P.accumulate = part > 0 ? 1 : 0;
        if (wave_k2) {
          hipLaunchKernelGGL(k_decorrelate_wave, dim3((grid.x + kDecorWaves - 1) / kDecorWaves, grid.y), dim3(64 * kDecorWaves),
                             0, ctx->stream, P);
          EARHIP_HIP(hipGetLastError());
        } else {
          launch_decor(Lk, P, grid, ctx->stream, true);
        }
      }
      if (evp) EARHIP_HIP(hipEventRecord(evp[5], ctx->stream));
      cur ^= 1;
      fresh = false;
    }
    if (timed) pending.push_back(pd);
    last_gated = ctx->last_gate_idx >= 0;
    last_device_form = ctx->last_wide_idx >= 0;
    last_hg_robust = last_gated && ctx->last_hinge_robust;
    if (ctx->lazy_allocs != lazy_before) scratch_regrows++;
    t += nsamples;
  }
};

extern "C" {

int earhip_render_create(earhip_ctx *ctx, const earhip_render_config *cfg, earhip_render **out) {
  return guarded([&] {
    require(ctx != nullptr && cfg != nullptr && out != nullptr, "NULL argument");
    require(cfg->n_objects >= 1 && cfg->n_out >= 1, "n_objects and n_out must be >= 1");
    require(cfg->n_buses == 1 || cfg->n_buses == 2, "n_buses must be 1 or 2");
    FftShape shape;
    require(cfg->block_size >= 16 && cfg->block_size <= 4096 && fft_make_shape(2 * cfg->block_size, &shape),
            "block_size must be in [16, 4096]");
    require(cfg->max_blocks >= 1, "max_blocks must be >= 1");
    require((int64_t)cfg->max_blocks * cfg->block_size < ((int64_t)1 << 30),
            "max_blocks * block_size too large");
    require(cfg->delay >= 0, "delay must be >= 0");
    if (cfg->n_buses == 2) {
      require(cfg->decorrelators != nullptr && cfg->n_taps >= 1,
              "n_buses == 2 needs decorrelator filters");
      require((cfg->n_taps + cfg->block_size - 1) / cfg->block_size <= 64,
              "decorrelator filters of more than 64 blocks are not supported by the fused render "
              "(use BlockConvolver)");
    } else {
      require(cfg->delay == 0, "delay needs n_buses == 2");
    }
    ctx->use();
    std::unique_ptr<earhip_render> r(new earhip_render);
    r->ctx = ctx;
    r->M = cfg->n_objects;
    r->N = cfg->n_out;
    r->B = cfg->block_size;
    r->K = cfg->n_buses;
    r->D = cfg->delay;
    r->T = cfg->max_blocks;
    r->Bk = r->B;
    if (r->K == 2 && r->B > 512 && r->B % 512 == 0 && cfg->n_taps <= 512 && !ctx->get(OPT_K2_OWN_BLOCK)) r->Bk = 512;
    r->Lk = 2 * r->Bk;
    if (r->Lk == 2048) r->run_len = 7;
    if (ctx->has(OPT_RUN)) {
      const int v = ctx->get(OPT_RUN);
      if (v >= 1 && v <= 255) r->run_len = v | 1, r->run_len_set = true;
    }
    r->curves.reset(new CurveSet(r->M, r->K * r->N, r->K, false));
    const size_t max_samples = (size_t)r->T * r->B;
    reserve_call_words(ctx, r->M, max_samples);
    r->rec.alloc_zero(2, ctx->stream);
    const size_t min_tile = (size_t)std::min(16 * ctx->nrt, std::min(64 * ctx->spl, 256));
    const size_t max_tiles = (max_samples + min_tile - 1) / min_tile;
    r->desc.alloc((size_t)r->M * ((max_samples + 255) / 256) + 1);
    (void)max_tiles;
    r->max_gsplit = 16;
    if (ctx->has(OPT_GSPLIT)) {
      const int v = ctx->get(OPT_GSPLIT);
      if (v >= 1 && v <= 32) r->max_gsplit = v;
    }
    r->bus.alloc_zero((size_t)r->K * r->N * bus_samples_bound(ctx, max_samples, r->max_gsplit), ctx->stream);
    if (r->K == 2) {
      const auto tw = make_twiddles(r->Lk);
      r->tw.alloc(r->Lk);
      EARHIP_HIP(hipMemcpy(r->tw.p, tw.data(), sizeof(cf) * r->Lk, hipMemcpyHostToDevice));
      r->NP = (cfg->n_taps + r->Bk - 1) / r->Bk;
      const size_t rows = (size_t)r->NP * r->N;
      std::vector<float> parts(rows * r->Bk, 0.0f);
      for (int n = 0; n < r->N; n++)
        for (int t = 0; t < cfg->n_taps; t++)
          parts[((size_t)(t / r->Bk) * r->N + n) * r->Bk + t % r->Bk] = cfg->decorrelators[(size_t)n * cfg->n_taps + t];
      DevBuf<float> taps;
      taps.alloc(parts.size());
      EARHIP_HIP(hipMemcpy(taps.p, parts.data(), sizeof(float) * parts.size(), hipMemcpyHostToDevice));
      r->H.alloc(rows * r->Lk);
      launch_spectrum(r->Lk, taps.p, r->Bk, r->Bk, r->tw.p, r->H.p, (int)rows, ctx->stream);
      EARHIP_HIP(hipStreamSynchronize(ctx->stream));
      std::vector<cf> h(rows * r->Lk);
      EARHIP_HIP(hipMemcpy(h.data(), r->H.p, sizeof(cf) * h.size(), hipMemcpyDeviceToHost));
      for (size_t n = 0; n < rows; n++) {
        cf *hn = h.data() + n * r->Lk;
        hn[0].y = 0.0f;
        hn[r->Bk].y = 0.0f;
        for (int k = 1; k < r->Bk; k++) hn[r->Lk - k] = cf_conj(hn[k]);
      }
      EARHIP_HIP(hipMemcpy(r->H.p, h.data(), sizeof(cf) * h.size(), hipMemcpyHostToDevice));
      const size_t hist_n = (size_t)r->N * std::max((r->NP - 1) * r->Bk, 1);
      for (int i = 0; i < 2; i++) {
        r->tail[i].alloc_zero(rows * r->Bk, ctx->stream);
        r->dly[i].alloc_zero((size_t)r->N * std::max(r->D, 1), ctx->stream);
        r->hist[i].alloc_zero(hist_n, ctx->stream);
        if (i == 0) {
          r->ztail.alloc_zero((size_t)r->N * r->Bk, ctx->stream);
          r->zdly.alloc_zero((size_t)r->N * std::max(r->D, 1), ctx->stream);
          r->zhist.alloc_zero(hist_n, ctx->stream);
        }
      }
    }
    EARHIP_HIP(hipStreamSynchronize(ctx->stream));
    *out = r.release();
  });
}

int earhip_render_destroy(earhip_render *r) {
  return guarded([&] {
    if (!r) return;
    (void)hipSetDevice(r->ctx->device);
    (void)hipStreamSynchronize(r->ctx->stream);
    delete r;
  });
}

int earhip_render_set_object_points(earhip_render *r, int object, int npoints,
                                    const int64_t *times, const float *direct,
                                    const float *diffuse) {
  return guarded([&] {
    require(r != nullptr, "render must not be NULL");
    require(npoints >= 1, "interp_points must not be empty");
    require(times != nullptr && direct != nullptr, "times/direct must not be NULL");
    require(r->K == 1 || diffuse != nullptr, "diffuse gains must not be NULL when n_buses == 2");
    const int N = r->N, cols = r->K * N;
    std::vector<float> rows((size_t)npoints * cols);
    for (int k = 0; k < npoints; k++) {
      std::memcpy(&rows[(size_t)k * cols], direct + (size_t)k * N, sizeof(float) * N);
      if (r->K == 2)
        std::memcpy(&rows[(size_t)k * cols + N], diffuse + (size_t)k * N, sizeof(float) * N);
    }
    r->curves->set_object(object, npoints, times, rows.data());
  });
}

int earhip_render_commit(earhip_render *r) {
  return guarded([&] {
    require(r != nullptr, "render must not be NULL");
    r->ctx->use();
    r->curves->commit(r->ctx);
    r->reserve_for_curves();
  });
}

int earhip_render_reset(earhip_render *r, int64_t sample_time) {
  return guarded([&] {
    require(r != nullptr, "render must not be NULL");
    r->ctx->use();
    r->t = sample_time;
    r->fresh = true;
    r->zero_levels();
  });
}

int earhip_render_attach_loudness(earhip_render *r, earhip_loudness *m) {
  return guarded([&] {
    require(r != nullptr, "render must not be NULL");
    if (m) {
// ... 449 lines not shown
    require(out_frames != nullptr, "out_frames must not be NULL");
    require(So == 3 || reinterpret_cast<uintptr_t>(out_frames) % So == 0, "out_frames not aligned to the sample size");
    if (nblocks == 0) return;
    process_frames_host(r, nblocks, frames, fmt, frame_channels, first_channel, nullptr, 1, out, out_frames);
  });
}

int earhip_render_process_frames_pcm_device(earhip_render *r, size_t nblocks, const void *frames_dev, earhip_pcm_format fmt,
                                            int frame_channels, int first_channel, void *out_dev, size_t out_frame_bytes,
                                            size_t out_first_byte, const earhip_pcm_out *out) {
  return guarded([&] {
    check_frames_args(r, nblocks, frames_dev, fmt, frame_channels, first_channel);
    const size_t So = check_pcm_out(out);
    require(out_dev != nullptr, "out_dev must not be NULL");
    require(So == 3 || reinterpret_cast<uintptr_t>(out_dev) % So == 0, "out_dev not aligned to the sample size");
    require(out_frame_bytes >= (size_t)r->N * So, "out_frame_bytes smaller than n_out samples");
    require(out_first_byte <= out_frame_bytes - (size_t)r->N * So, "out_first_byte + n_out samples exceed out_frame_bytes");
    require(So == 3 || (out_frame_bytes % So == 0 && out_first_byte % So == 0), "out_frame_bytes / out_first_byte not multiples of the sample size");
    if (nblocks == 0) return;
    earhip_ctx *ctx = r->ctx;
    ctx->use();
    const size_t S = (size_t)pcm_sample_bytes(fmt);
    const size_t n = nblocks * r->B, cap = (size_t)r->T * r->B;
    if (r->d_rows.n < cap * r->M || r->d_rows_out.n < cap * r->N) {
      EARHIP_HIP(hipStreamSynchronize(ctx->stream));
      r->d_rows.reserve(cap * r->M);
      r->d_rows_out.reserve(cap * r->N);
    }
    r->reserve_levels();
    launch_pcm_to_rows(fmt, frames_dev, (size_t)frame_channels * S, (size_t)first_channel * S, r->M, n, r->d_rows.p, n, ctx->stream);
    const int64_t t0 = r->t;
    r->process_device(nblocks, r->d_rows.p, n, r->d_rows_out.p, n);
    launch_rows_to_pcm(*out, r->d_rows_out.p, n, r->N, n, static_cast<unsigned char *>(out_dev), out_frame_bytes, out_first_byte,
                       r->d_peak.p, r->d_clip.p, t0, ctx->stream);
  });
}

int earhip_render_output_levels(earhip_render *r, float *peak, uint64_t *clipped, int reset) {
  return guarded([&] {
    require(r != nullptr, "render must not be NULL");
    require(peak != nullptr && clipped != nullptr, "peak and clipped must not be NULL");
    earhip_ctx *ctx = r->ctx;
    ctx->use();
    EARHIP_HIP(hipStreamSynchronize(ctx->stream));
    if (!r->d_peak.p) {
      for (int c = 0; c < r->N; c++) peak[c] = 0.f, clipped[c] = 0;
      return;
    }
    const size_t cnt = (size_t)kLevelSlots * r->N;
    std::vector<unsigned> pk(cnt);
    std::vector<unsigned long long> cl(cnt);
    EARHIP_HIP(hipMemcpy(pk.data(), r->d_peak.p, sizeof(unsigned) * cnt, hipMemcpyDeviceToHost));
    EARHIP_HIP(hipMemcpy(cl.data(), r->d_clip.p, sizeof(unsigned long long) * cnt, hipMemcpyDeviceToHost));
    for (int c = 0; c < r->N; c++) {
      unsigned m = 0;
      uint64_t sum = 0;
      for (int k = 0; k < kLevelSlots; k++) m = std::max(m, pk[(size_t)k * r->N + c]), sum += cl[(size_t)k * r->N + c];
      std::memcpy(&peak[c], &m, sizeof(float));
      clipped[c] = sum;
    }
    if (reset) r->zero_levels();
  });
}

int earhip_debug_k2_prof(earhip_ctx *ctx, unsigned long long *out64) {
  return guarded([&] {
    require(ctx != nullptr && out64 != nullptr, "NULL argument");
#ifdef EARHIP_K2_PROF
    ctx->use();
    EARHIP_HIP(hipStreamSynchronize(ctx->stream));
    EARHIP_HIP(hipMemcpyFromSymbol(out64, HIP_SYMBOL(g_k2_prof), sizeof(unsigned long long) * 64));
#else
    fail_invalid("this build has no K2 phase stamps (-DEARHIP_K2_PROF)");
#endif
  });
}

int earhip_render_enable_timing(earhip_render *r, int enable) {
  return guarded([&] {
    require(r != nullptr, "render must not be NULL");
    r->ctx->use();
    if (r->timing) r->drain_timing();
    r->timing = enable != 0;
    r->timing_every = enable > 1 ? enable : 1;
    r->timing_calls = 0;
    for (int i = 0; i < 3; i++) r->acc_ms[i] = r->acc_n[i] = 0;
  });
}

int earhip_render_get_timing(earhip_render *r, double out[6]) {
  return guarded([&] {
    require(r != nullptr && out != nullptr, "NULL argument");
    r->ctx->use();
    r->drain_timing();
    out[0] = r->acc_ms[0]; out[1] = r->acc_n[0];
    out[2] = r->acc_ms[1]; out[3] = r->acc_n[1];
    out[4] = r->acc_ms[2]; out[5] = r->acc_n[2];
  });
}

int earhip_render_gain_kernel(const earhip_render *r, int *kind) {
  return guarded([&] {
    require(r != nullptr && kind != nullptr, "NULL argument");
    *kind = r->last_kind;
  });
}

int earhip_render_hinge_standby(earhip_render *r, int *standby) {
  return guarded([&] {
    require(r != nullptr && standby != nullptr, "NULL argument");
    *standby = 0;
    earhip_ctx *ctx = r->ctx;
    if (r->last_kind != 5 || !r->last_gated || r->last_hg_robust) return;
    ctx->use();
    unsigned word = 0;
    EARHIP_HIP(hipMemcpyAsync(&word, r->rec.p, sizeof(word), hipMemcpyDeviceToHost, ctx->stream));
    EARHIP_HIP(hipStreamSynchronize(ctx->stream));
    if (!(word & kModeRecorded)) fail_internal("no gain kernel recorded the call's mode word");
    *standby = (word & kGateHingeUnsafe) ? 1 : 0;
  });
}

int earhip_render_hinge_robust(earhip_render *r, int *robust) {
  return guarded([&] {
    require(r != nullptr && robust != nullptr, "NULL argument");
    *robust = 0;
    earhip_ctx *ctx = r->ctx;
    if (r->last_kind != 5 || !r->last_hg_robust) return;
    ctx->use();
    unsigned word = 0;
    EARHIP_HIP(hipMemcpyAsync(&word, r->rec.p, sizeof(word), hipMemcpyDeviceToHost, ctx->stream));
    EARHIP_HIP(hipStreamSynchronize(ctx->stream));
    if (!(word & kModeRecorded)) fail_internal("no gain kernel recorded the call's mode word");
    *robust = hinge_span_exceeded(word, r->M) ? 1 : 0;
  });
}

int earhip_render_wide_form(earhip_render *r, int *wide) {
  return guarded([&] {
    require(r != nullptr && wide != nullptr, "NULL argument");
    *wide = 1;
    earhip_ctx *ctx = r->ctx;
    if (r->last_kind < 3) *wide = -1;
    if (r->last_kind < 3 || !r->last_device_form) return;
    ctx->use();
    unsigned word = 0;
    EARHIP_HIP(hipMemcpyAsync(&word, r->rec.p, sizeof(word), hipMemcpyDeviceToHost, ctx->stream));
    EARHIP_HIP(hipStreamSynchronize(ctx->stream));
    if (!(word & kModeRecorded)) fail_internal("no gain kernel recorded the call's mode word");
    *wide = (word & 1u) ? 1 : 0;
  });
}

int earhip_render_scratch_bytes(const earhip_render *r, size_t *bytes) {
  return guarded([&] {
    require(r != nullptr && bytes != nullptr, "NULL argument");
    *bytes = r->last_scratch_bytes;
  });
}

int earhip_render_scratch_regrows(const earhip_render *r, long *count) {
  return guarded([&] {
    require(r != nullptr && count != nullptr, "NULL argument");
    *count = r->scratch_regrows;
  });
}

int earhip_render_last_tail_blocks(const earhip_render *r, int *blocks) {
  return guarded([&] {
    require(r != nullptr && blocks != nullptr, "NULL argument");
    *blocks = r->last_tail_blocks;
  });
}

int earhip_render_last_host_chunks(const earhip_render *r, int *chunks) {
  return guarded([&] {
    require(r != nullptr && chunks != nullptr, "NULL argument");
    *chunks = r->last_host_chunks;
  });
}

int earhip_render_last_list_layout(const earhip_render *r, int *paired) {
  return guarded([&] {
    require(r != nullptr && paired != nullptr, "NULL argument");
    *paired = r->last_paired;
  });
}

int earhip_render_last_plan(const earhip_render *r, int out[4]) {
  return guarded([&] {
    require(r != nullptr && out != nullptr, "NULL argument");
    out[0] = r->last_kind;
    for (int i = 0; i < 3; i++) out[1 + i] = r->last_plan[i];
  });
}

}

namespace earhip {
size_t pcm_out_check(const earhip_pcm_out *out) { return check_pcm_out(out); }
int pcm_level_slots() { return kLevelSlots; }
void pcm_out_rows(const earhip_pcm_out &o, const float *in, size_t in_stride, int N, size_t len, unsigned char *out, size_t frame_bytes,
                  size_t first_byte, unsigned *peak, unsigned long long *clipped, int64_t t0, hipStream_t s) {
  launch_rows_to_pcm(o, in, in_stride, N, len, out, frame_bytes, first_byte, peak, clipped, t0, s);
}
}
```

libear_amd/csrc/common.h:

```cpp
#pragma once

#include <hip/hip_runtime.h>

#include <cstdint>
#include <cstdio>
#include <string>
#include <vector>

#include "../../include/earhip.h"

namespace earhip {

struct Error {
  int code;
  std::string msg;
};

void set_last_error(const std::string &msg);

template <typename F>
int guarded(F &&f) {
  try {
    f();
    return EARHIP_OK;
  } catch (const Error &e) {
    set_last_error(e.msg);
    return e.code;
  } catch (const std::bad_alloc &) {
    set_last_error("out of host memory");
    return EARHIP_INTERNAL_ERROR;
  } catch (const std::exception &e) {
    set_last_error(e.what());
    return EARHIP_INTERNAL_ERROR;
  }
}

[[noreturn]] inline void fail_invalid(const std::string &m) {
  throw Error{EARHIP_INVALID_ARGUMENT, m};
}
[[noreturn]] inline void fail_internal(const std::string &m) {
  throw Error{EARHIP_INTERNAL_ERROR, "internal error: " + m};
}
inline void require(bool ok, const char *m) {
  if (!ok) fail_invalid(m);
}

#define EARHIP_HIP(expr)                                                        \
  do {                                                                          \
    hipError_t e_ = (expr);                                                     \
    if (e_ != hipSuccess)                                                       \
      throw ::earhip::Error{EARHIP_DEVICE_ERROR,                                \
                            std::string("internal error: HIP: ") +              \
                                hipGetErrorString(e_) + " in " #expr};          \
  } while (0)

inline bool is_pow2(size_t v) { return v && !(v & (v - 1)); }

template <typename T>
struct DevBuf {
  T *p = nullptr;
  size_t n = 0;
  DevBuf() = default;
  DevBuf(const DevBuf &) = delete;
  DevBuf &operator=(const DevBuf &) = delete;
  ~DevBuf() { release(); }
  void release() {
    if (p) (void)hipFree(p);
    p = nullptr;
    n = 0;
  }
  void alloc(size_t count) {
    release();
    if (count == 0) count = 1;
    EARHIP_HIP(hipMalloc((void **)&p, count * sizeof(T)));
    n = count;
  }
  void alloc_zero(size_t count, hipStream_t s) {
    alloc(count);
    EARHIP_HIP(hipMemsetAsync(p, 0, n * sizeof(T), s));
  }
  void reserve(size_t count) {
    if (count > n) alloc(count);
  }
};

template <typename T>
struct PinBuf {
  T *p = nullptr;
  size_t n = 0;
  PinBuf() = default;
  PinBuf(const PinBuf &) = delete;
  PinBuf &operator=(const PinBuf &) = delete;
  ~PinBuf() {
    if (p) (void)hipHostFree(p);
  }
  void reserve(size_t count) {
    if (count <= n) return;
    if (p) (void)hipHostFree(p);
    p = nullptr;
    n = 0;
    EARHIP_HIP(hipHostMalloc((void **)&p, count * sizeof(T), hipHostMallocDefault));
    n = count;
  }
};

}

struct earhip_vbs;
namespace earhip {
void vbs_orphan(earhip_vbs *v);
}

namespace earhip {
enum Opt {
  OPT_SPL, OPT_MFMA, OPT_XSCALE, OPT_WAVES, OPT_TPW, OPT_NRT,
  OPT_H2_TILE, OPT_H2_WGS, OPT_H2_RUNS, OPT_P2_TILE, OPT_P2_PAIRS, OPT_P2_WGS, OPT_HINGE, OPT_HG_TILE, OPT_HBUILD_TPW, OPT_BUILD_TPW,
  OPT_K2_WG, OPT_K2_OWN_BLOCK, OPT_RUN, OPT_GSPLIT,
  OPT_PROBE_RUNS, OPT_BLOCK_GROUPS, OPT_DEBUG_TIMING, OPT_TAILCUT, OPT_HOST_CHUNK_MB, OPT_HOST_THREADS, OPT_HG_ROBUST, OPT_BUILD_2K,
  OPT_HOST_BIND, OPT_HOST_NT, OPT_HOST_FIRST, OPT_H2_PAIR, OPT_COUNT
};
struct OptVal {
  bool set = false;
  int v = 0;
};
}

struct earhip_ctx {
  earhip::OptVal opt[earhip::OPT_COUNT];
  bool has(earhip::Opt o) const { return opt[o].set; }
  int get(earhip::Opt o, int dflt = 0) const { return opt[o].set ? opt[o].v : dflt; }
  void apply_options();
  int device = 0;
  hipStream_t stream = nullptr;
  bool own_stream = false;
  bool strict = false;
  int spl = 4;
  int use_mfma = 3;
  int x_scale_log2 = 14;
  bool x_scale_auto = true;
  earhip::DevBuf<unsigned> level;
  int level_idx = 0;
  int last_gate_idx = -1;
  bool last_hinge_robust = false;
  int last_wide_idx = -1;
  earhip::DevBuf<unsigned> tile_slow;
  size_t tile_slow_cap = 0;
  int tile_slow_idx = 0;
  earhip::DevBuf<unsigned> obj_level;
  int obj_level_cap = 0;
  long lazy_allocs = 0;
  unsigned *record_slot = nullptr;
  int max_waves = 4;
  int tiles_per_wg = 4;
  bool tiles_per_wg_forced = false;
  int nrt = 8;
  int num_cus = 256;
  size_t hinge_build_lds = 64 * 1024;
  struct HostRange {
    const char *base;
    size_t bytes;
    bool owned;
  };
  std::vector<HostRange> host_ranges;
  std::vector<earhip_vbs *> pinned_adapters;
  bool host_reachable(const void *p, size_t bytes) const {
    const char *c = static_cast<const char *>(p);
    for (const auto &r : host_ranges)
      if (c >= r.base && c + bytes <= r.base + r.bytes) return true;
    return false;
  }
  earhip::PinBuf<float> pin_in, pin_out;
  earhip::DevBuf<float> dev_in, dev_out, dev_pts;
  void use() const { EARHIP_HIP(hipSetDevice(device)); }
};

namespace earhip {
int panner_create(earhip_ctx *ctx, const char *layout, int n_channels, const double *azimuth, const double *elevation,
                  earhip_panner **out, bool with_extent);
}

struct earhip_loudness;
namespace earhip {
void loudness_check_room(const earhip_loudness *m, size_t nsamples);
void loudness_feed(earhip_loudness *m, size_t nsamples, const float *rows, size_t stride);
const earhip_ctx *loudness_ctx(const earhip_loudness *m);
int loudness_channels(const earhip_loudness *m);
}

struct earhip_firmix;
namespace earhip {
void firmix_check_room(const earhip_firmix *fm, size_t nblocks);
void firmix_feed(earhip_firmix *fm, size_t nblocks, const float *in, size_t in_stride, float *out, size_t out_stride);
const earhip_ctx *firmix_ctx(const earhip_firmix *fm);
int firmix_inputs(const earhip_firmix *fm);
int firmix_outputs(const earhip_firmix *fm);
int firmix_block(const earhip_firmix *fm);
}

struct earhip_limiter;
namespace earhip {
void limiter_check_room(const earhip_limiter *lim, size_t nsamples);
void limiter_feed(earhip_limiter *lim, size_t nsamples, const float *in, size_t in_stride, float *out, size_t out_stride);
const earhip_ctx *limiter_ctx(const earhip_limiter *lim);
int limiter_channels(const earhip_limiter *lim);
size_t pcm_out_check(const earhip_pcm_out *out);
int pcm_level_slots();
void pcm_out_rows(const earhip_pcm_out &o, const float *in, size_t in_stride, int N, size_t len, unsigned char *out, size_t frame_bytes,
                  size_t first_byte, unsigned *peak, unsigned long long *clipped, int64_t t0, hipStream_t s);
}
```

libear_amd/csrc/curves.h:

```cpp
#pragma once

#include <chrono>
#include <cmath>
#include <cstdio>
#include <cstdlib>

#include <algorithm>
#include <cstring>
#include <vector>

#include "common.h"
#include "gain_kernels.h"
#include "gain_p2.h"
#include "gain_hg.h"
#include "gain_f32g.h"

namespace earhip {

struct ColumnPlan {
  int nout = 24;
  int ngroups = 1;
  int nz = 1;
  int nct = 1;
  int mgroups = 1;
  int mnz = 1;
  int row = 24;
  static ColumnPlan make(int ncols) {
    ColumnPlan p;
    int groups = (ncols + 23) / 24;
    const int per = (ncols + groups - 1) / groups;
    p.nout = per <= 8 ? 8 : per <= 16 ? 16 : 24;
    groups = (ncols + p.nout - 1) / p.nout;
    p.ngroups = std::min(groups, 8);
    p.nz = (groups + p.ngroups - 1) / p.ngroups;
    int mg = (ncols + 47) / 48;
    p.nct = mg > 1 ? 3 : (ncols + 15) / 16;
    p.mgroups = std::min(mg, 8);
    p.mnz = (mg + p.mgroups - 1) / p.mgroups;
    p.row = std::max(p.nz * p.ngroups * p.nout, p.mnz * p.mgroups * p.nct * 16);
    return p;
  }
};

struct CurveImage {
  ObjHdr *hdr;
  int32_t *off, *cnt;
  int64_t *time;
  uint8_t *flat;
  PointRec *rec;
  float *gain;
};
static __global__ void __launch_bounds__(256)
k_curve_upload(CurveImage src, CurveImage dst, const int32_t *changed, int row) {
  const int m = changed[blockIdx.x];
  const int off = src.off[m], n = src.cnt[m];
  if (threadIdx.x == 0) dst.off[m] = off, dst.cnt[m] = n, dst.hdr[m] = src.hdr[m];
  for (int i = threadIdx.x; i < n; i += 256) {
    dst.time[off + i] = src.time[off + i];
    dst.flat[off + i] = src.flat[off + i];
    dst.rec[off + i] = src.rec[off + i];
  }
  const size_t g0 = (size_t)off * row, gn = (size_t)n * row;
  const float4 *sg = reinterpret_cast<const float4 *>(src.gain + g0);
  float4 *dg = reinterpret_cast<float4 *>(dst.gain + g0);
  for (size_t i = threadIdx.x; i < gn / 4; i += 256) dg[i] = sg[i];
}

class CurveSet {
 public:
  CurveSet(int M, int ncols, int nbus = 1, bool force_ramp = false)
      : M_(M), ncols_(ncols), nbus_(nbus), force_ramp_(force_ramp), plan_(ColumnPlan::make(ncols)), obj_(M) {
    for (int m = 0; m < M; m++) {
      obj_[m].t.assign(1, 0);
      obj_[m].g.assign(plan_.row, 0.0f);
      obj_[m].flat.assign(1, 0);
      obj_[m].dirty = true;
      dirty_list_.push_back(m);
    }
    cmax_.assign(plan_.row, 0.0f);
    obj_cmax_.assign((size_t)M * plan_.row, 0.0f);
    cm_scratch_.assign(plan_.row, 0.0f);
    shrunk_cols_.assign(plan_.row, 0);
    dirty_list_.reserve(M);
    for (auto &p : phases_) p.items.reserve(M);
  }
  ~CurveSet() {
    if (staged_) (void)hipEventDestroy(staged_);
  }
  int M() const { return M_; }
  int ncols() const { return ncols_; }
  const ColumnPlan &plan() const { return plan_; }

  void set_object(int m, int npoints, const int64_t *times, const float *rows,
                  const uint8_t *flat_override = nullptr) {
    if (m < 0 || m >= M_) fail_invalid("object index out of range");
    if (npoints < 1) fail_invalid("interp_points must not be empty");
    if (npoints > kMaxPointsPerObject) fail_invalid("too many interpolation points for one object");
    for (int k = 1; k < npoints; k++) {
      if (times[k] < times[k - 1]) fail_invalid("interpolation points are not sorted");
      if (times[k] - times[k - 1] > (int64_t)0x7fffffff)
        fail_invalid("interpolation ramp longer than 2^31-1 samples is not supported");
    }
    Obj &o = obj_[m];
    const size_t row = (size_t)plan_.row;
    o.t.assign(times, times + npoints);
    o.g.assign((size_t)npoints * row, 0.0f);
    for (int k = 0; k < npoints; k++)
      std::memcpy(&o.g[(size_t)k * row], rows + (size_t)k * ncols_, sizeof(float) * ncols_);
    o.flat.assign(npoints, 0);
    const int bc = ncols_ / nbus_;
    for (int k = 1; k < npoints; k++) {
      if (flat_override) {
        o.flat[k] = flat_override[k];
        continue;
      }
      for (int b = 0; b < nbus_; b++) {
        bool same = true;
        for (int c = b * bc; same && c < (b + 1) * bc; c++)
          same = rows[(size_t)(k - 1) * ncols_ + c] == rows[(size_t)k * ncols_ + c];
        if (same) o.flat[k] |= (uint8_t)(1 << b);
      }
    }
    {
      int w = 1;
      for (int k = 1; k < npoints; k++) {
        const bool repeat = o.t[k] == o.t[w - 1] && std::memcmp(&o.g[(size_t)k * row], &o.g[(size_t)(w - 1) * row], sizeof(float) * row) == 0;
        if (repeat) continue;
        if (w != k) {
          o.t[w] = o.t[k];
          o.flat[w] = o.flat[k];
          std::memmove(&o.g[(size_t)w * row], &o.g[(size_t)k * row], sizeof(float) * row);
        }
        w++;
      }
      o.t.resize(w);
      o.flat.resize(w);
      o.g.resize((size_t)w * row);
    }
    if (!o.dirty) o.dirty = true, dirty_list_.push_back(m);
  }

  void commit(earhip_ctx *ctx) {
    if (dirty_list_.empty()) return;
#ifdef EARHIP_COMMIT_TIMING
    static double acc[6] = {0, 0, 0, 0, 0, 0};
    static long ncalls = 0;
    auto now = [] { return std::chrono::duration<double, std::micro>(std::chrono::steady_clock::now().time_since_epoch()).count(); };
    double tq = now();
    auto lap = [&](int i) { const double t = now(); acc[i] += t - tq; tq = t; };
    struct Print { ~Print() { if (ncalls) fprintf(stderr, "commit timing (us/call over %ld): sync %.2f regions %.2f mirror+stats %.2f finish %.2f upload %.2f tail %.2f\n", ncalls, acc[0]/ncalls, acc[1]/ncalls, acc[2]/ncalls, acc[3]/ncalls, acc[4]/ncalls, acc[5]/ncalls); } };
    static Print printer;
    ncalls++;
#define EARHIP_LAP(i) lap(i)
#else
#define EARHIP_LAP(i)
#endif
    const size_t row = (size_t)plan_.row;
    if (staged_) EARHIP_HIP(hipEventSynchronize(staged_));
    EARHIP_LAP(0);
    bool full_upload = !uploaded_once_;
    for (int m : dirty_list_) {
      Obj &o = obj_[m];
      const int n = (int)o.t.size();
      if (n > o.cap) {
        abandoned_ += (size_t)o.cap;
        o.cap = std::max(16, n + n / 2);
        o.off = (int)arena_used_;
        arena_used_ += (size_t)o.cap;
      }
    }
    if (abandoned_ > arena_used_ / 2 && abandoned_ > 4096) {
      arena_used_ = 2;
      abandoned_ = 0;
      for (int m = 0; m < M_; m++) {
        Obj &o = obj_[m];
        o.cap = std::max(16, (int)o.t.size() + (int)o.t.size() / 2);
        o.off = (int)arena_used_;
        arena_used_ += (size_t)o.cap;
        if (!o.dirty) o.dirty = true, dirty_list_.push_back(m);
      }
      full_upload = true;
    }
    if (arena_used_ >= ((size_t)1 << 31)) fail_invalid("too many interpolation points");
    if (arena_used_ > arena_cap_) {
      const size_t cap = arena_used_ + arena_used_ / 2 + 64;
      EARHIP_HIP(hipStreamSynchronize(ctx->stream));
      PinBuf<int64_t> nt;
      PinBuf<uint8_t> nf;
      PinBuf<PointRec> nr;
      PinBuf<float> ng;
      nt.reserve(cap), nf.reserve(cap), nr.reserve(cap), ng.reserve(cap * row);
      if (arena_cap_) {
        std::memcpy(nt.p, h_time_.p, arena_cap_ * sizeof(int64_t));
        std::memcpy(nf.p, h_flat_.p, arena_cap_);
        std::memcpy(nr.p, h_rec_.p, arena_cap_ * sizeof(PointRec));
        std::memcpy(ng.p, h_gain_.p, arena_cap_ * row * sizeof(float));
      } else {
        std::memset(ng.p, 0, 2 * row * sizeof(float));
        std::memset(nt.p, 0, 2 * sizeof(int64_t));
        std::memset(nf.p, 0, 2);
        std::memset(nr.p, 0, 2 * sizeof(PointRec));
      }
      std::swap(h_time_.p, nt.p), std::swap(h_time_.n, nt.n);
      std::swap(h_flat_.p, nf.p), std::swap(h_flat_.n, nf.n);
      std::swap(h_rec_.p, nr.p), std::swap(h_rec_.n, nr.n);
      std::swap(h_gain_.p, ng.p), std::swap(h_gain_.n, ng.n);
      d_time_.alloc(cap), d_flat_.alloc(cap), d_rec_.alloc(cap), d_gain_.alloc(cap * row * (kinks_ ? 2 : 1));
      arena_cap_ = cap;
      full_upload = true;
    }
    if (!h_off_.p) {
      h_off_.reserve(M_), h_cnt_.reserve(M_), h_changed_.reserve(M_), h_gcol_.reserve(row), h_hdr_.reserve(M_);
      d_off_.alloc(M_), d_cnt_.alloc(M_), d_gcol_.alloc(row), d_hdr_.alloc(M_);
    }
    EARHIP_LAP(1);
    const float old_scale = gain_scale();
    bool cmax_shrunk = false;
    for (int m : dirty_list_) {
      Obj &o = obj_[m];
      const int n = (int)o.t.size();
      h_off_.p[m] = o.off;
      h_cnt_.p[m] = n;
      h_hdr_.p[m] = ObjHdr{o.off, n, o.t[0], o.t[n - 1], 0};
      std::memcpy(h_time_.p + o.off, o.t.data(), (size_t)n * sizeof(int64_t));
      std::memcpy(h_flat_.p + o.off, o.flat.data(), (size_t)n);
      std::memcpy(h_gain_.p + (size_t)o.off * row, o.g.data(), (size_t)n * row * sizeof(float));
      for (int k = 0; k < n; k++) {
        PointRec &r = h_rec_.p[o.off + k];
        r.time = o.t[k];
        const int64_t len = k ? o.t[k] - o.t[k - 1] : 0;
        r.scale = len > 0 ? 1.0f / (float)len : 0.0f;
        r.flat = o.flat[k];
      }
      float *cm = obj_cmax_.data() + (size_t)m * row;
      if (o.has_stats) cmax_shrunk = retire(o.st, cm) || cmax_shrunk;
      o.st = stats_of(o, cm);
      admit(o.st, cm);
      o.has_stats = true;
    }
    if (cmax_shrunk) {
      for (size_t c = 0; c < row; c++) {
        if (!shrunk_cols_[c]) continue;
        shrunk_cols_[c] = 0;
        float v = 0.0f;
        for (int m = 0; m < M_; m++) {
          const float a = obj_cmax_[(size_t)m * row + c];
          v = a <= v ? v : a;
        }
        cmax_[c] = v;
      }
    }
    EARHIP_LAP(2);
    finish_stats();
    const float set_scale = gain_scale();
    bool gcol_changed = !uploaded_once_ || set_scale != old_scale;
    for (size_t c = 0; c < row; c++) {
      const float cm = cmax_[c];
      int e;
      std::frexp(cm, &e);
      const float v = (cm >= 1e-30f && cm < 1e30f) ? std::ldexp(1.0f, 14 - e) : (set_scale > 0.0f ? set_scale : 1.0f);
      gcol_changed = gcol_changed || v != h_gcol_.p[c];
      h_gcol_.p[c] = v;
    }
    EARHIP_LAP(3);
    if (gcol_changed) EARHIP_HIP(hipMemcpyAsync(d_gcol_.p, h_gcol_.p, row * sizeof(float), hipMemcpyHostToDevice, ctx->stream));
    if (full_upload || dirty_list_.size() > (size_t)M_ / 4) {
      EARHIP_HIP(hipMemcpyAsync(d_off_.p, h_off_.p, M_ * sizeof(int32_t), hipMemcpyHostToDevice, ctx->stream));
      EARHIP_HIP(hipMemcpyAsync(d_cnt_.p, h_cnt_.p, M_ * sizeof(int32_t), hipMemcpyHostToDevice, ctx->stream));
      EARHIP_HIP(hipMemcpyAsync(d_hdr_.p, h_hdr_.p, M_ * sizeof(ObjHdr), hipMemcpyHostToDevice, ctx->stream));
      EARHIP_HIP(hipMemcpyAsync(d_time_.p, h_time_.p, arena_used_ * sizeof(int64_t), hipMemcpyHostToDevice, ctx->stream));
      EARHIP_HIP(hipMemcpyAsync(d_flat_.p, h_flat_.p, arena_used_, hipMemcpyHostToDevice, ctx->stream));
      EARHIP_HIP(hipMemcpyAsync(d_rec_.p, h_rec_.p, arena_used_ * sizeof(PointRec), hipMemcpyHostToDevice, ctx->stream));
      EARHIP_HIP(hipMemcpyAsync(d_gain_.p, h_gain_.p, arena_used_ * row * sizeof(float), hipMemcpyHostToDevice, ctx->stream));
    } else {
      for (size_t i = 0; i < dirty_list_.size(); i++) h_changed_.p[i] = dirty_list_[i];
      CurveImage src{h_hdr_.p, h_off_.p, h_cnt_.p, h_time_.p, h_flat_.p, h_rec_.p, h_gain_.p};
      CurveImage dst{d_hdr_.p, d_off_.p, d_cnt_.p, d_time_.p, d_flat_.p, d_rec_.p, d_gain_.p};
      hipLaunchKernelGGL(k_curve_upload, dim3((unsigned)dirty_list_.size()), dim3(256), 0, ctx->stream, src, dst, h_changed_.p,
                         (int)row);
      EARHIP_HIP(hipGetLastError());
    }
    EARHIP_LAP(4);
    if (kinks_) {
      const bool all = full_upload || gcol_changed || dirty_list_.size() > (size_t)M_ / 4;
      if (!all)
        for (size_t i = 0; i < dirty_list_.size(); i++) h_changed_.p[i] = dirty_list_[i];
      derive_kinks(ctx, all ? nullptr : h_changed_.p, all ? M_ : (int)dirty_list_.size());
    }
    if (!staged_) EARHIP_HIP(hipEventCreateWithFlags(&staged_, hipEventDisableTiming));
    EARHIP_HIP(hipEventRecord(staged_, ctx->stream));
    for (int m : dirty_list_) obj_[m].dirty = false;
    dirty_list_.clear();
    uploaded_once_ = true;
    EARHIP_LAP(5);
  }
#undef EARHIP_LAP

  void ensure_kinks(earhip_ctx *ctx) {
    if (kinks_) return;
    kinks_ = true;
    const size_t row = (size_t)plan_.row;
    EARHIP_HIP(hipStreamSynchronize(ctx->stream));
    d_gain_.alloc(arena_cap_ * row * 2);
    EARHIP_HIP(hipMemcpyAsync(d_gain_.p, h_gain_.p, arena_used_ * row * sizeof(float), hipMemcpyHostToDevice, ctx->stream));
    derive_kinks(ctx, nullptr, M_);
    if (!staged_) EARHIP_HIP(hipEventCreateWithFlags(&staged_, hipEventDisableTiming));
    EARHIP_HIP(hipEventRecord(staged_, ctx->stream));
  }
  bool has_kinks() const { return kinks_; }
  bool dirty() const { return !dirty_list_.empty(); }

  bool tiles_aligned(int tile, int64_t t_call) const {
    const int64_t d = t_call >= t_ref_ ? t_call - t_ref_ : t_ref_ - t_call;
    return d % tile == 0 && grid_ % (uint64_t)tile == 0;
  }

  int aligned_tile(int64_t t_call) const {
    const int grids[2] = {512, 256};
    for (int gi = 0; gi < 2; gi++) {
      const int64_t G = grids[gi];
      const int si = 1 - gi;
      int off_grid_limit = M_ / 64;
      if (ramp_share() < 0.5) {
        const double deltas = deltas_per_pair(si ? 512 : 256);
        off_grid_limit = (int)(M_ * std::min(1.0 / 64, deltas / 200.0));
      }
      if (tiles_aligned((int)G, t_call)) return (int)G;
      if (grid_off_[gi] <= off_grid_limit && (((t_call - grid_phase_[gi]) % G) + G) % G == 0) return (int)G;
    }
    return 0;
  }

  double deltas_per_pair(int tile) const {
    const int gi = tile >= 512 ? 1 : 0;
    return tot_.tiles[gi] > 0 ? tot_.incid[gi] / tot_.tiles[gi] * moving_share() : 0.0;
  }
  double moving_share() const { return M_ > 0 ? (double)tot_.moving / M_ : 0.0; }
  double point_density_all() const { return point_density() * moving_share(); }
  double ramp_share() const { return tot_.span > 0 ? tot_.ramp / tot_.span : 0.0; }
  double point_density() const { return tot_.span > 0 ? tot_.npts / tot_.span : 0.0; }
  double pair_waste(int tile) const {
    const int gi = tile >= 512 ? 1 : 0;
    return (tot_.incid[gi] - tot_.touched[gi]) / std::max(1.0, tot_.tiles[gi] + tot_.incid[gi]);
  }
  double hinge_exact_share(size_t in_stride, size_t nsamples) const {
    if (force_ramp_ || !hinge_addressable((size_t)M_, in_stride, nsamples, 2 * arena_cap_, (size_t)plan_.row)) return 2.0;
    return tot_.span > 0 ? std::min(1.0, tot_.bad / std::max(1.0, tot_.span / kHingeTile)) : 0.0;
  }

  int piece_cap(int tile, bool paired) const {
    const int gi = tile >= 512 ? 1 : 0;
    const long slots = paired ? (long)((M_ + 63) & ~63) + 2 * tot_.sum_r7[gi] : (long)M_ + tot_.sum_r15[gi];
    return (int)std::min<long>(slots + 128, (long)kPieceCapPerObject * M_ + 128);
  }

  float gain_scale() const {
    if (!(gain_max_ < 1e30f)) return 0.0f;
    if (gain_max_ < 1e-18f) return 1.0f;
    int e;
    std::frexp(gain_max_, &e);
    return std::ldexp(1.0f, 14 - e);
  }

  const float *column_scales() const { return d_gcol_.p; }

  PointStore device() const {
    PointStore ps;
    ps.hdr = d_hdr_.p;
    ps.off = d_off_.p;
    ps.cnt = d_cnt_.p;
    ps.time = d_time_.p;
    ps.flat = d_flat_.p;
    ps.rec = d_rec_.p;
    ps.gain = d_gain_.p;
    ps.row = plan_.row;
    ps.bus_cols = ncols_ / nbus_;
    ps.nbus = nbus_;
    ps.zero_row = 0;
    ps.npoints = (int)tot_.points;
    ps.rows = (int)arena_used_;
    ps.kink_row0 = kinks_ ? (int)arena_cap_ : 0;
    ps.force_ramp = force_ramp_ ? 1 : 0;
    return ps;
  }

 private:
  void derive_kinks(earhip_ctx *ctx, const int32_t *objects, int count) {
    const size_t row = (size_t)plan_.row;
    uint32_t *kink = reinterpret_cast<uint32_t *>(d_gain_.p + arena_cap_ * row);
    EARHIP_HIP(hipMemsetAsync(kink, 0, 2 * row * sizeof(uint32_t), ctx->stream));
    hipLaunchKernelGGL(k_kink_rows, dim3((unsigned)count), dim3(256), 0, ctx->stream, d_off_.p, d_cnt_.p, d_rec_.p, d_gain_.p, kink,
                       d_gcol_.p, objects, (int)row, nbus_);
    EARHIP_HIP(hipGetLastError());
  }
  struct ObjStats {
    uint64_t gcd = 0;
    int64_t first = 0;
    int64_t phase[2] = {-1, -1};
    double span = 0, ramp = 0, npts = 0, bad = 0, points = 0;
    double incid[2] = {0, 0}, touched[2] = {0, 0}, tiles[2] = {0, 0};
    int maxr[2] = {0, 0};
  };
  struct Obj {
    std::vector<int64_t> t;
    std::vector<float> g;
    std::vector<uint8_t> flat;
    int off = 0, cap = 0;
    bool dirty = false, has_stats = false;
    ObjStats st;
  };

  ObjStats stats_of(const Obj &o, float *cm) const {
    ObjStats s;
    const auto &t = o.t;
    const size_t row = (size_t)plan_.row, n = t.size();
    const int allflat = (1 << nbus_) - 1;
    s.first = t[0];
    s.points = (double)n;
    for (size_t k = 1; k < n && s.gcd != 1; k++) {
      uint64_t a = (uint64_t)(t[k] - t[k - 1]), b = s.gcd;
      while (a) {
        const uint64_t r = b % a;
        b = a;
        a = r;
      }
      s.gcd = b;
    }
    const int64_t grids[2] = {512, 256};
    for (int gi = 0; gi < 2; gi++) {
      const int64_t G = grids[gi];
      const int64_t p0 = ((t[0] % G) + G) % G;
      bool same = s.gcd % (uint64_t)G == 0;
      s.phase[gi] = same ? p0 : -1;
    }
    for (size_t k = 1; k < n; k++) {
      const int64_t len = t[k] - t[k - 1];
      const bool is_ramp = (o.flat[k] & allflat) != allflat;
      s.span += (double)len;
      if (is_ramp) s.ramp += (double)len;
      if (len < kHingeMinLen) s.bad += is_ramp ? 1.0 + (double)len / kHingeTile : 0.5;
    }
    if (n > 1) s.npts = (double)(n - 1);
    for (int gi = 0; gi < 2; gi++) {
      const int64_t T = gi ? 512 : 256;
      auto tile_of = [T](int64_t a) { return a >= 0 ? a / T : -((-a + T - 1) / T); };
      if (n > 1) s.tiles[gi] = (double)(t.back() - t.front()) / (double)T;
      int64_t last_tile = INT64_MIN;
      for (size_t k = 1; k < n; k++) {
        if ((o.flat[k] & allflat) == allflat) continue;
        const int64_t a = t[k] > t[k - 1] ? t[k - 1] : t[k] - 1, b = t[k];
        const int64_t ta = tile_of(a), tb = tile_of(b - 1);
        s.incid[gi] += (double)(tb - ta + 1);
        s.touched[gi] += (double)(tb - ta + 1) - (ta == last_tile ? 1.0 : 0.0);
        last_tile = tb;
      }
    }
    for (int gi = 0; gi < 2; gi++) {
      const int64_t T = gi ? 512 : 256;
      auto is_r = [&](size_t k) { return (o.flat[k] & allflat) != allflat; };
      auto ra = [&](size_t k) { return t[k] > t[k - 1] ? t[k - 1] : t[k] - 1; };
      int best = 0, inside = 0;
      size_t j = 1;
      for (size_t i = 1; i < n; i++) {
        if (!is_r(i)) continue;
        if (j < i) j = i, inside = 0;
        while (j < n && (!is_r(j) || ra(j) < t[i] - 1 + T)) {
          if (is_r(j)) inside++;
          j++;
        }
        best = std::max(best, inside);
        inside--;
      }
      s.maxr[gi] = force_ramp_ ? 1 : best;
    }
    for (size_t c = 0; c < row; c++) cm[c] = 0.0f;
    for (size_t k = 0; k < n; k++) {
      const float *g = o.g.data() + k * row;
      for (size_t c = 0; c < row; c++) {
        const float a = std::fabs(g[c]);
        cm[c] = a <= cm[c] ? cm[c] : a;
      }
    }
    return s;
  }
  bool retire(const ObjStats &s, const float *cm) {
    tot_.span -= s.span, tot_.ramp -= s.ramp, tot_.npts -= s.npts, tot_.bad -= s.bad, tot_.points -= s.points;
    tot_.moving -= s.npts > 0 ? 1 : 0;
    for (int gi = 0; gi < 2; gi++) {
      tot_.incid[gi] -= s.incid[gi], tot_.touched[gi] -= s.touched[gi], tot_.tiles[gi] -= s.tiles[gi];
      tot_.sum_r15[gi] -= std::min(s.maxr[gi], kPieceMaxPerObject), tot_.sum_r7[gi] -= std::min(s.maxr[gi], kPairMaxPerObject);
      if (s.phase[gi] >= 0) phases_[gi].add(s.phase[gi], -1);
    }
    grid_stale_ = true;
    bool shrunk = false;
    for (size_t c = 0; c < cmax_.size(); c++) {
      const bool was_max = cm[c] != cm[c] || (cm[c] > 0.0f && !(cm[c] < cmax_[c]));
      if (was_max) shrunk_cols_[c] = 1, shrunk = true;
    }
    return shrunk;
  }
  void admit(const ObjStats &s, const float *cm) {
    tot_.span += s.span, tot_.ramp += s.ramp, tot_.npts += s.npts, tot_.bad += s.bad, tot_.points += s.points;
    tot_.moving += s.npts > 0 ? 1 : 0;
    for (int gi = 0; gi < 2; gi++) {
      tot_.incid[gi] += s.incid[gi], tot_.touched[gi] += s.touched[gi], tot_.tiles[gi] += s.tiles[gi];
      tot_.sum_r15[gi] += std::min(s.maxr[gi], kPieceMaxPerObject), tot_.sum_r7[gi] += std::min(s.maxr[gi], kPairMaxPerObject);
      if (s.phase[gi] >= 0) phases_[gi].add(s.phase[gi], +1);
    }
    grid_stale_ = true;
    for (size_t c = 0; c < cmax_.size(); c++) cmax_[c] = cm[c] <= cmax_[c] ? cmax_[c] : cm[c];
  }
  void finish_stats() {
    if (grid_stale_) {
      t_ref_ = obj_[0].st.first;
      uint64_t g = 0;
      auto fold = [&g](uint64_t a) {
        uint64_t b = g;
        while (a) {
          const uint64_t r = b % a;
          b = a;
          a = r;
        }
        g = b;
      };
      for (int m = 0; m < M_ && g != 1; m++) {
        const ObjStats &s = obj_[m].st;
        fold(s.gcd);
        fold((uint64_t)(s.first >= t_ref_ ? s.first - t_ref_ : t_ref_ - s.first));
      }
      grid_ = g;
      grid_stale_ = false;
    }
    for (int gi = 0; gi < 2; gi++) {
      int64_t best = 0;
      int best_n = 0;
      for (const auto &kv : phases_[gi].items)
        if (kv.second > best_n) best_n = kv.second, best = kv.first;
      grid_phase_[gi] = best;
      grid_off_[gi] = M_ - best_n;
    }
    float gmax = 0.0f;
    for (float v : cmax_) gmax = v <= gmax ? gmax : v;
    gain_max_ = gmax;
  }

  int M_, ncols_, nbus_;
  bool force_ramp_;
  ColumnPlan plan_;
  std::vector<Obj> obj_;
  std::vector<int> dirty_list_;
  bool uploaded_once_ = false;
  size_t arena_used_ = 2, arena_cap_ = 0, abandoned_ = 0;
  struct Totals {
    double span = 0, ramp = 0, npts = 0, bad = 0, points = 0;
    long moving = 0;
    double incid[2] = {0, 0}, touched[2] = {0, 0}, tiles[2] = {0, 0};
    long sum_r15[2] = {0, 0}, sum_r7[2] = {0, 0};
  } tot_;
  struct PhaseCounts {
    std::vector<std::pair<int64_t, int>> items;
    void add(int64_t phase, int d) {
      for (size_t i = 0; i < items.size(); i++)
        if (items[i].first == phase) {
          items[i].second += d;
          if (items[i].second <= 0) items[i] = items.back(), items.pop_back();
          return;
        }
      if (d > 0) items.emplace_back(phase, d);
    }
  } phases_[2];
  std::vector<float> obj_cmax_;
  std::vector<float> cm_scratch_;
  std::vector<uint8_t> shrunk_cols_;
  bool grid_stale_ = true;
  int64_t t_ref_ = 0;
  uint64_t grid_ = 0;
  int64_t grid_phase_[2] = {0, 0};
  int grid_off_[2] = {0, 0};
  std::vector<float> cmax_;
  float gain_max_ = 0;
  DevBuf<int32_t> d_off_, d_cnt_;
  DevBuf<ObjHdr> d_hdr_;
  PinBuf<ObjHdr> h_hdr_;
  DevBuf<int64_t> d_time_;
  DevBuf<uint8_t> d_flat_;
  DevBuf<PointRec> d_rec_;
  DevBuf<float> d_gcol_, d_gain_;
  bool kinks_ = false;
  PinBuf<float> h_gcol_, h_gain_;
  PinBuf<int32_t> h_off_, h_cnt_, h_changed_;
  PinBuf<int64_t> h_time_;
  PinBuf<uint8_t> h_flat_;
  PinBuf<PointRec> h_rec_;
  hipEvent_t staged_ = nullptr;
};

struct MixLaunch {
  bool mfma;
  bool split = false;
  bool wide = false;
  bool pieces = false;
  int pw = 2;
  bool paired = false;
  bool f32grid = false;
  bool hinge = false;
  int hinge_tile = 512;
  int spl;
  int nrt;
  int ntiles, wsplit, gsplit;
  int tpw = 1;
  int tile() const { return f32grid ? kF32GridTile : hinge ? hinge_tile : pieces ? 64 * pw : split ? (wide ? 512 : 256) : mfma ? 16 * nrt : 64 * spl; }
};

inline MixLaunch plan_mix(const earhip_ctx *ctx, const ColumnPlan &cp, int M, int nsamples,
                          bool strict, int max_gsplit, int aligned_tile = 0, double ramp_share = 1.0,
                          float gain_scale = 0.0f, double point_density = 0.0, double pair_waste256 = 1.0,
                          double pair_waste512 = 1.0, double hinge_exact_share = 2.0, bool grid512_strict = false,
                          double deltas256 = 0.0) {
  const bool aligned = aligned_tile >= 256;
  MixLaunch L;
  L.mfma = !strict && ctx->use_mfma;
  L.split = L.mfma && M >= 32 && gain_scale > 0.0f && ctx->use_mfma != 5 && ctx->use_mfma != 6 &&
            (ctx->use_mfma == 4 || (ctx->use_mfma == 3 && aligned));
  const int forced = ctx->get(OPT_H2_TILE);
  L.pieces = L.mfma && !L.split && M >= 32 && M <= kMaxPieceObjects && gain_scale > 0.0f &&
             (ctx->use_mfma == 3 || ctx->use_mfma == 5 || ctx->use_mfma == 6);
  if ((ctx->use_mfma == 5 || ctx->use_mfma == 6) && L.pieces) L.split = false;
  if (L.pieces) {
    const int ptile = ctx->get(OPT_P2_TILE);
    const double kPairWaste = 0.06;
    const double kMostlyRamping = cp.nct == 3 && M <= 1024 ? 0.7 : 0.5;
    const bool paired_by_rule = pair_waste256 < kPairWaste && ramp_share < kMostlyRamping;
    L.paired = paired_by_rule;
    if (ctx->has(OPT_P2_PAIRS)) L.paired = ctx->get(OPT_P2_PAIRS) != 0;
    const bool long_call = nsamples / 512 >= 2 * ctx->num_cus;
    L.pw = ptile == 512 ? 8 : ptile == 256 ? 4 : (L.paired && long_call && pair_waste512 < kPairWaste) ? 8 : 4;
    const double kHingeExact = 0.005, kHingeRamps = 0.5;
    const int hinge_max = (int)std::min((size_t)kMaxHingeCached, ctx->hinge_build_lds / 16);
    L.hinge = M <= hinge_max && hinge_exact_share <= kHingeExact && ramp_share >= kHingeRamps && !(paired_by_rule && L.paired);
    if (ctx->has(OPT_HINGE)) L.hinge = ctx->get(OPT_HINGE) != 0 && M <= hinge_max && hinge_exact_share <= 1.0;
    if (ctx->use_mfma == 6) L.hinge = M <= hinge_max && hinge_exact_share <= 1.0;
    if (ctx->use_mfma == 5) L.hinge = false;
    if (L.hinge && !ctx->has(OPT_HINGE) && ctx->use_mfma == 3 && cp.nct == 3 && deltas256 > 0.0 && point_density > 0.0) {
      const double hinge_est = 0.56 + 0.077 * (point_density * 512.0), lists_est = 0.151 + 0.238 * (1.0 + deltas256);
      if (lists_est < 0.97 * hinge_est) L.hinge = false;
    }
    if (L.hinge) {
      if (ctx->has(OPT_HG_TILE)) L.hinge_tile = ctx->get(OPT_HG_TILE) == 256 ? 256 : 512;
      L.pieces = false, L.paired = false, L.pw = 4;
    }
  }
  L.wide = L.split && aligned_tile >= 512 && forced != 256 && (forced == 512 || nsamples / 512 >= 2 * ctx->num_cus);
  L.f32grid = L.mfma && !L.split && !L.pieces && !L.hinge && ctx->use_mfma == 1 && grid512_strict && gain_scale > 0.0f &&
              nsamples % kF32GridTile == 0 && M >= 16;
  if (L.mfma && !L.split && !L.pieces && !L.hinge && !L.f32grid && M > kMaxSlotObjects) L.mfma = false;
  L.spl = ctx->spl;
  L.nrt = ctx->nrt;
  L.ntiles = (nsamples + L.tile() - 1) / L.tile();
  if (L.split || L.pieces || L.hinge || L.f32grid) {
    L.wsplit = 1;
    L.tpw = 1;
    int g = 1;
    const int nz = cp.mnz * cp.mgroups;
    while (g < max_gsplit && L.ntiles * nz * g < 2 * ctx->num_cus && M / (g * 2) >= 64) g *= 2;
    L.gsplit = g;
    return L;
  }
  if (strict) {
    L.wsplit = 1;
    L.gsplit = 1;
    return L;
  }
  const int groups = L.mfma ? cp.mgroups : cp.ngroups;
  if (L.mfma) L.tpw = std::max(1, std::min(std::min(ctx->tiles_per_wg, L.ntiles), ctx->max_waves / groups));
  if (L.mfma && !ctx->tiles_per_wg_forced) L.tpw = std::max(1, std::min(L.tpw, (ctx->max_waves / groups) / std::max(1, (M + 127) / 128)));
  L.wsplit = std::max(1, std::min(std::max(1, ctx->max_waves / (groups * L.tpw)), std::max(1, M / 8)));
  const int per_wg = std::max(1, M / L.wsplit);
  int g = 1;
  const int want = 2 * ctx->num_cus;
  while (g < max_gsplit && (L.ntiles / L.tpw) * (L.mfma ? cp.mnz : cp.nz) * g < want && per_wg / (g * 2) >= 8) g *= 2;
  L.gsplit = g;
  return L;
}

inline size_t bus_samples_bound(const earhip_ctx *ctx, size_t max_samples, int max_gsplit) {
  const size_t pad = (max_samples + 3) & ~(size_t)3;
  const size_t tpw_max = (size_t)std::max(1, std::min(ctx->tiles_per_wg, ctx->max_waves));
  const size_t split_tiles = (size_t)4 * ctx->num_cus + max_gsplit;
  const size_t split = std::max(split_tiles * 512, split_tiles * tpw_max * 16 * (size_t)ctx->nrt) + 4 * (size_t)max_gsplit;
  return std::max(pad, std::min(pad * (size_t)max_gsplit, split));
}

size_t mix_lds_bytes(const ColumnPlan &cp, const MixLaunch &ml);
void reserve_call_words(earhip_ctx *ctx, int M, size_t max_samples);

inline size_t scratch_units(const CurveSet &cs, const MixLaunch &ml, int M) {
  const size_t nt = (size_t)ml.ntiles;
  if (ml.hinge) {
    const size_t pnt = nt * (size_t)std::max(1, ml.tile() / (64 * ml.pw));
    return std::max(hinge_units((size_t)M, nt) + (size_t)M * nt,
                    piece_units((size_t)M, pnt, (size_t)cs.piece_cap(64 * ml.pw, ml.paired)) + (size_t)M * pnt);
  }
  if (ml.pieces) return piece_units((size_t)M, nt, (size_t)cs.piece_cap(ml.tile(), ml.paired)) + (size_t)M * nt;
  if (ml.split || ml.f32grid || !ml.mfma) return (size_t)M * nt + 1;
  return desc_units((size_t)M, nt);
}

void launch_gain_mix(earhip_ctx *ctx, const CurveSet &cs, const MixLaunch &ml, bool strict,
                     int64_t t_call, int nsamples, const float *in_dev, size_t in_stride,
                     float *out_dev, size_t out_stride, size_t part_stride, SegDesc *desc,
                     hipEvent_t *ev );

}
```

libear_amd/csrc/gain_h2.h:

```cpp
#pragma once

#include <hip/hip_runtime.h>

#include <type_traits>

#include "gain_kernels.h"
#include "gain_mfma.h"

namespace earhip {

typedef uint32_t u32x4 __attribute__((ext_vector_type(4)));
typedef float f32x2 __attribute__((ext_vector_type(2)));

constexpr int kSplitTile = 256;
constexpr int kSplitChunk = 32;

typedef _Float16 f16x8 __attribute__((ext_vector_type(8)));
typedef _Float16 f16x2_t __attribute__((ext_vector_type(2)));

__device__ __forceinline__ uint32_t pack_f16(float a, float b) {
  const f32x2 v = {a, b};
  return __builtin_bit_cast(uint32_t, __builtin_convertvector(v, f16x2_t));
}
__device__ __forceinline__ float f16_lo(uint32_t u) { return (float)__builtin_bit_cast(f16x2_t, u)[0]; }
__device__ __forceinline__ float f16_hi(uint32_t u) { return (float)__builtin_bit_cast(f16x2_t, u)[1]; }
__device__ __forceinline__ float sub_f16_lo(float v, uint32_t u) {
  float r;
  asm("v_fma_mix_f32 %0, %1, -1.0, %2 op_sel:[0,0,0] op_sel_hi:[1,0,0]" : "=v"(r) : "v"(u), "v"(v));
  return r;
}
__device__ __forceinline__ float sub_f16_hi(float v, uint32_t u) {
  float r;
  asm("v_fma_mix_f32 %0, %1, -1.0, %2 op_sel:[1,0,0] op_sel_hi:[1,0,0]" : "=v"(r) : "v"(u), "v"(v));
  return r;
}

constexpr float kLowPieceScale = 2048.0f;
__device__ __forceinline__ uint32_t scale_f16x2_down(uint32_t h) {
  const f16x2_t k = {(_Float16)0.00048828125f, (_Float16)0.00048828125f};
  return __builtin_bit_cast(uint32_t, __builtin_bit_cast(f16x2_t, h) * k);
}

__device__ __forceinline__ f32x4 mfma_f16(const u32x4 &a, const u32x4 &b, const f32x4 &c) {
  return __builtin_amdgcn_mfma_f32_16x16x32_f16(__builtin_bit_cast(f16x8, a), __builtin_bit_cast(f16x8, b), c,
                                                0, 0, 0);
}

constexpr bool h2_persistent(int nct, int nw) { return nw == 8 || nct == 1; }
template <int NCT, int NW, int FORM>
__global__ void __launch_bounds__(64 * NW, NCT == 1 && NW == 8 ? 2 : (NW == 4 ? 2 : 1))
k_gain_mix_h2(GainMixParams P, int zero_row, float x_scale, const float *__restrict__ gcol, const unsigned *level_cur,
              unsigned *level_next, const unsigned *slow_cur, unsigned *slow_next, const unsigned *wide_cur, unsigned *wide_next) {
  if (FORM != 2 && wide_cur && ((*wide_cur & 1u) != 0u) != (FORM == 1)) return;
  constexpr int NRT = 4, TS = 16 * NRT, CH = kSplitChunk;
  constexpr int NQ = CH / NW;
  constexpr int NFRAG = 2 * NCT * 3;
  __shared__ u32x4 bfrag[2][NFRAG + 6][64];
  constexpr int OP = TS + 4;
  __shared__ __attribute__((aligned(16))) float otile[NW][16 * OP];
  __shared__ float inv_gcol[16 * NCT];
  __shared__ unsigned long long redo_tiles[NW];
  auto body = [&](auto wide_tag) __attribute__((always_inline)) {
  constexpr bool WIDE = decltype(wide_tag)::value;
  if (threadIdx.x < 16 * NCT) inv_gcol[threadIdx.x] = 1.0f / gcol[blockIdx.z * 16 * NCT + threadIdx.x];
  __syncthreads();
  const int lane = threadIdx.x & 63;
  const int w = __builtin_amdgcn_readfirstlane(threadIdx.x >> 6);
  const int li = lane & 15, kg = lane >> 4;
  const int ntl = P.ntiles, gx = gridDim.x;
  const bool runs = P.tile_runs != 0;
  const int run_first = (int)(((int64_t)ntl * blockIdx.x) / gx), run_end = (int)(((int64_t)ntl * (blockIdx.x + 1)) / gx);
  const int vb0 = runs ? run_first : (int)blockIdx.x, vstep = runs ? 1 : gx;
  const int vb_last = runs ? max(run_end - 1, run_first) : ntl - 1;
  const int my_tiles = runs ? run_end - run_first : (ntl - (int)blockIdx.x + gx - 1) / gx;
  auto tile_at = [&](int vb) { return runs ? min(vb, ntl - 1) : xcd_tile(vb, ntl); };
  if (blockIdx.x == 0 && blockIdx.y == 0 && blockIdx.z == 0 && threadIdx.x == 0) {
    if (wide_next) *wide_next = 0u;
    record_mode(P, wide_cur != nullptr);
  }
  if (level_cur) {
    const unsigned lv = *level_cur;
    if (lv) {
      const int E = max(-60, min(20, (int)(lv >> 23) - 127));
      x_scale = __uint_as_float((unsigned)(127 + 7 - E) << 23);
    }
    if (blockIdx.x == 0 && blockIdx.y == 0 && blockIdx.z == 0 && threadIdx.x == 0) *level_next = 0;
  }
  const int nparts = gridDim.y;
  const int part = blockIdx.y;
  const int m_lo = (int)(((int64_t)P.M * part) / nparts);
  const int m_hi = (int)(((int64_t)P.M * (part + 1)) / nparts);
  const int col0 = blockIdx.z * 16 * NCT;
  const float *__restrict__ gain = P.ps.gain;
  const unsigned rowlen = (unsigned)P.ps.row;
  auto tile_first = [&](int t) { return t * (TS * NW) + w * TS; };
  auto tile_length = [&](int t) { return max(0, min(TS, P.nsamples - tile_first(t))); };
  auto opaque_lane = [&]() __attribute__((always_inline)) {
    int l = lane;
    asm volatile("" : "+v"(l));
    return l;
  };

  f32x4 tot0[NRT][NCT], tot1[NRT][NCT];
  auto clear_totals = [&]() {
#pragma unroll
    for (int r = 0; r < NRT; r++)
#pragma unroll
      for (int c = 0; c < NCT; c++) tot0[r][c] = tot1[r][c] = f32x4{0.0f, 0.0f, 0.0f, 0.0f};
  };
  clear_totals();

  auto single_object = [&](int t, int m, float sx, bool sg, int khint = -1) __attribute__((always_inline)) {
    const int tile_s0 = tile_first(t), tile_len = tile_length(t);
    if (tile_len <= 0) return;
    const int64_t tile_t0 = P.t_call + tile_s0, tile_t1 = tile_t0 + tile_len;
    const int ol = opaque_lane(), li = ol & 15, kg = ol >> 4;
    float gsc[NCT];
#pragma unroll
    for (int c = 0; c < NCT; c++) gsc[c] = sg ? gcol[col0 + c * 16 + li] : 1.0f;
    const int base = P.ps.off[m], n = P.ps.cnt[m];
    const float *row = P.in + (size_t)m * P.in_stride + tile_s0;
    const bool is_b = kg & 1;
    const bool slot0 = kg < 2;
    int k;
    if (khint >= 0) {
      k = min(khint, n);
      while (k < n && P.ps.time[base + k] <= tile_t0) k++;
    } else {
      k = upper_bound_time(P.ps.time + base, n, tile_t0);
    }
    int cur = 0;
    while (cur < tile_len) {
      const SegDesc dk = describe_segment(P.ps, base, n, k, tile_t0, tile_t1);
      const int r1 = min(seg_r1(dk.info), tile_len);
      if (r1 > cur) {
        const bool ramp = dk.info & kSegRamp;
        float a[NRT], gv[NCT];
#pragma unroll
        for (int r = 0; r < NRT; r++) {
          const int s = li * NRT + r;
          const float x = row[min(s, tile_len - 1)];
          const float p = (float)(dk.d0 + s) * dk.scale;
          float coef = ramp ? (is_b ? p : 1.0f - p) : (is_b ? 0.0f : 1.0f);
          coef = (slot0 && s >= cur && s < r1) ? coef : 0.0f;
          a[r] = (x * coef) * sx;
        }
        const int grow = dk.row + ((ramp && is_b && slot0) ? 1 : 0);
        const float *gp = gain + (size_t)grow * rowlen + col0 + li;
#pragma unroll
        for (int c = 0; c < NCT; c++) gv[c] = gp[c * 16] * gsc[c];
#pragma unroll
        for (int r = 0; r < NRT; r++)
#pragma unroll
          for (int c = 0; c < NCT; c++)
            tot0[r][c] = __builtin_amdgcn_mfma_f32_16x16x4f32(a[r], gv[c], tot0[r][c], 0, 0, 0);
        cur = r1;
      }
      if (!(dk.info & kSegMulti)) break;
      k++;
    }
  };

  const int nobj = m_hi - m_lo;
  const int nch = (P.vec_ok && nobj >= CH) ? (nobj + CH - 1) / CH : 0;
  auto flush_tile = [&](int t, float inv_x, bool col_scaled) __attribute__((always_inline)) {
    const int tile_s0 = tile_first(t), tile_len = tile_length(t);
    if (tile_len > 0) {
      const int ol = opaque_lane(), li = ol & 15, kg = ol >> 4;
      const float wf0 = (float)(w * TS + kg * 16 - (TS * NW) / 2);
      float inv_gc[NCT];
#pragma unroll
      for (int c = 0; c < NCT; c++) inv_gc[c] = col_scaled ? inv_gcol[c * 16 + li] : 1.0f;
      float *op = P.out + (size_t)blockIdx.y * P.part_stride + tile_s0;
      const bool whole = P.vec_ok && tile_len == TS;
#pragma unroll
      for (int c = 0; c < NCT; c++) {
        if (whole) {
          float *ot = otile[w];
#pragma unroll
          for (int e = 0; e < 4; e++) {
            f32x4 v;
#pragma unroll
            for (int r = 0; r < NRT; r++)
              v[r] = (__builtin_fmaf(wf0 + (float)(4 * e + r), tot1[r][c][e], tot0[r][c][e]) * inv_x) * inv_gc[c];
            *reinterpret_cast<f32x4 *>(ot + li * OP + kg * 16 + e * 4) = v;
          }
#pragma unroll
          for (int j = 0; j < 4; j++) {
            const int cl = 4 * j + kg, col = col0 + c * 16 + cl;
            const f32x4 v = *reinterpret_cast<const f32x4 *>(ot + cl * OP + li * 4);
            if (col < P.ncols) __builtin_nontemporal_store(v, reinterpret_cast<f32x4 *>(op + (size_t)col * P.out_stride + li * 4));
          }
          continue;
        }
        const int col = col0 + c * 16 + li;
        if (col >= P.ncols) continue;
        float *o = op + (size_t)col * P.out_stride;
#pragma unroll
        for (int e = 0; e < 4; e++) {
          const int s = kg * 16 + e * 4;
          f32x4 v;
#pragma unroll
          for (int r = 0; r < NRT; r++)
            v[r] = (__builtin_fmaf(wf0 + (float)(4 * e + r), tot1[r][c][e], tot0[r][c][e]) * inv_x) * inv_gc[c];
          if (P.vec_ok && s + 3 < tile_len) {
            *reinterpret_cast<f32x4 *>(o + s) = v;
          } else {
#pragma unroll
            for (int i = 0; i < 4; i++)
              if (s + i < tile_len) o[s + i] = v[i];
          }
        }
      }

    }
    clear_totals();
  };

  if (lane == 0) redo_tiles[w] = 0ull;
  if (nch > 0) {
    const int nvec = (P.nsamples + 3) & ~3;
    const unsigned xrow = (unsigned)(kg * 8) * (unsigned)P.in_stride * 4u;
    const int xsl = w * TS + li * NRT;
    struct Stage {
      int tile, c;
    };
    int left = my_tiles * nch;
    int vb_c = vb0;
    auto next_stage = [&](const Stage &s) __attribute__((always_inline)) {
      Stage n;
      const bool wrap = s.c + 1 == nch;
      n.c = wrap ? 0 : s.c + 1;
      if (wrap) vb_c = min(vb_c + vstep, vb_last);
      n.tile = wrap ? tile_at(vb_c) : s.tile;
      return n;
    };
    const unsigned bcol_e = (unsigned)(col0 + min(lane, 16 * NCT - 1));
    const float g_scale = gcol[bcol_e];
    const int blane = (w * NQ / 8) * 16 + (lane & 15);
    const int bfr = lane < 16 * NCT ? (lane >> 4) * 3 : NFRAG;
    const int bfr1 = lane < 16 * NCT ? NCT * 3 : 3;
    auto chunk_base = [&](int c) { return min(m_lo + c * CH, m_hi - CH); };

    auto load_x_part = [&](const Stage &st, bool live, f32x4 (&x)[8], int q0, int n) {
      const int ts0 = st.tile * (TS * NW);
      const char *bp = reinterpret_cast<const char *>(P.in + (live ? (size_t)chunk_base(st.c) * P.in_stride + ts0 : 0));
      const size_t rstride = live ? P.in_stride * sizeof(float) : 0;
      const unsigned xo = live ? xrow + 4u * (unsigned)min(xsl, nvec - 4 - ts0) : 0u;
#pragma unroll
      for (int q = 0; q < 8; q++)
        if (q >= q0 && q < q0 + n)
          x[q] = __builtin_nontemporal_load(reinterpret_cast<const f32x4 *>(bp + (size_t)q * rstride + xo));
    };
    auto load_x = [&](const Stage &st, bool live, f32x4 (&x)[8]) { load_x_part(st, live, x, 0, 8); };
    typedef const SegDesc __attribute__((address_space(4))) *ConstDesc;
    struct ChunkDesc {
      SegDesc d[NQ];
    };
    auto load_desc = [&](const Stage &st) {
      ConstDesc dp = (ConstDesc)(P.desc + (size_t)st.tile * P.M + chunk_base(st.c) + w * NQ);
      ChunkDesc D;
#pragma unroll
      for (int q = 0; q < NQ; q++) {
        D.d[q].row = dp[q].row;
        D.d[q].d0 = dp[q].d0;
        D.d[q].scale = dp[q].scale;
        D.d[q].info = dp[q].info;
      }
      return D;
    };
    struct ChunkCoef {
      float p0[NQ], scale[NQ];
    };
    auto load_gains = [&](const ChunkDesc &R, int cc, ChunkCoef &D, float (&S)[NQ], float (&E)[NQ]) {
      const int m0 = chunk_base(cc) + w * NQ;
#pragma unroll
      for (int q = 0; q < NQ; q++) {
        const SegDesc d = R.d[q];
        const bool valid = m0 + q >= m_lo + cc * CH && !(d.info & (kSegMulti | kSegQuiet));
        const unsigned rs = (unsigned)(valid ? d.row : zero_row);
        const unsigned re = (valid && (d.info & kSegRamp)) ? (unsigned)d.row + 1u : rs;
        D.p0[q] = d.scale != 0.0f ? (float)(d.d0 + (TS * NW) / 2) * d.scale : 0.0f;
        D.scale[q] = d.scale;
        const float *rps = gain + (size_t)rs * rowlen, *rpe = gain + (size_t)re * rowlen;
        S[q] = rps[bcol_e];
        E[q] = rpe[bcol_e];
      }
    };
    auto store_b = [&](const ChunkCoef &D, const float (&S)[NQ], const float (&E)[NQ], int buf, int part) {
      uint32_t h[NQ / 2], l[NQ / 2], hs[NQ / 2];
#pragma unroll
      for (int i = 0; i < NQ / 2; i++) {
        float v[2];
#pragma unroll
        for (int j = 0; j < 2; j++) {
          const int q = 2 * i + j;
          v[j] = (part == 0 ? __builtin_fmaf(1.0f - D.p0[q], S[q], D.p0[q] * E[q]) : D.scale[q] * (E[q] - S[q])) *
                 g_scale;
        }
        const uint32_t H = pack_f16(v[0], v[1]);
        h[i] = H;
        l[i] = pack_f16(sub_f16_lo(v[0], H), sub_f16_hi(v[1], H));
        hs[i] = WIDE ? scale_f16x2_down(H) : 0u;
      }
      u32x4 *f = &bfrag[buf][bfr][blane] + (part ? bfr1 * 64 : 0);
      if constexpr (NQ == 8) {
        f[0] = u32x4{h[0], h[1], h[2], h[3]};
        f[64] = u32x4{l[0], l[1], l[2], l[3]};
        if constexpr (WIDE) f[128] = u32x4{hs[0], hs[1], hs[2], hs[3]};
      } else {
        typedef uint32_t u32x2 __attribute__((ext_vector_type(2)));
        u32x2 *g = reinterpret_cast<u32x2 *>(f) + (w & 1);
        g[0] = u32x2{h[0], h[1]};
        g[128] = u32x2{l[0], l[1]};
        if constexpr (WIDE) g[256] = u32x2{hs[0], hs[1]};
      }
    };

    f32x4 X0[8], X1[8];
    ChunkDesc L;
    Stage sa, sb, sc;
    sa.tile = tile_at(vb_c);
    sa.c = 0;
    sb = next_stage(sa);
    sc = next_stage(sb);
    int ka = 0;
    {
      float S[NQ], E[NQ];
      ChunkCoef D;
      L = load_desc(sa);
      load_gains(L, 0, D, S, E);
      load_x(sa, true, X0);
      load_x(sb, left > 1, X1);
      store_b(D, S, E, 0, 0);
      store_b(D, S, E, 0, 1);
      L = load_desc(sb);
    }
    auto chunk = [&](int buf, f32x4 (&xc)[8]) __attribute__((always_inline)) {
      __syncthreads();
      float S[NQ], E[NQ];
      ChunkCoef D;
      load_gains(L, sb.c, D, S, E);
      L = load_desc(sc);
      __builtin_amdgcn_sched_barrier(0);

      u32x4 ah[NRT], al[NRT];
#pragma unroll
      for (int qp = 0; qp < 4; qp++)
#pragma unroll
        for (int rp = 0; rp < NRT; rp += 2) {
          const f32x2 s0 = f32x2{xc[2 * qp][rp], xc[2 * qp][rp + 1]} * x_scale;
          const f32x2 s1 = f32x2{xc[2 * qp + 1][rp], xc[2 * qp + 1][rp + 1]} * x_scale;
          const uint32_t H0 = pack_f16(s0[0], s1[0]), H1 = pack_f16(s0[1], s1[1]);
          constexpr float LOW = WIDE ? kLowPieceScale : 1.0f;
          const f32x2 r0 = f32x2{sub_f16_lo(s0[0], H0), sub_f16_lo(s0[1], H1)} * LOW;
          const f32x2 r1 = f32x2{sub_f16_hi(s1[0], H0), sub_f16_hi(s1[1], H1)} * LOW;
          ah[rp][qp] = H0;
          ah[rp + 1][qp] = H1;
          al[rp][qp] = pack_f16(r0[0], r1[0]);
          al[rp + 1][qp] = pack_f16(r0[1], r1[1]);
        }
      constexpr int XB = 2 * NCT >= 4 ? 4 : 2 * NCT;
      __builtin_amdgcn_sched_barrier(0);
      constexpr int NBLK = 2 * NCT;
      u32x4 b[2][2], b2;
      auto load_b = [&](int blk, u32x4 (&bb)[2]) {
#pragma unroll
        for (int q = 0; q < 2; q++) bb[q] = bfrag[buf][((blk & 1) * NCT + (blk >> 1)) * 3 + q][lane];
      };
      load_b(0, b[0]);
      __builtin_amdgcn_sched_group_barrier(0x100, 2, 0);
#pragma unroll
      for (int blk = 0; blk < NBLK; blk++) {
        u32x4(&bc)[2] = b[blk & 1];
        const int ct = blk >> 1;
        if constexpr (WIDE) b2 = bfrag[buf][((blk & 1) * NCT + (blk >> 1)) * 3 + 2][lane];
        if (blk + 1 < NBLK) load_b(blk + 1, b[(blk + 1) & 1]);
        f32x4(&tt)[NRT][NCT] = (blk & 1) == 0 ? tot0 : tot1;
        if constexpr (WIDE) {
#pragma unroll
          for (int r = 0; r < NRT; r++) tt[r][ct] = mfma_f16(ah[r], bc[1], tt[r][ct]);
#pragma unroll
          for (int r = 0; r < NRT; r++) tt[r][ct] = mfma_f16(al[r], b2, tt[r][ct]);
        } else {
#pragma unroll
          for (int r = 0; r < NRT; r++) tt[r][ct] = mfma_f16(al[r], bc[0], tt[r][ct]);
#pragma unroll
          for (int r = 0; r < NRT; r++) tt[r][ct] = mfma_f16(ah[r], bc[1], tt[r][ct]);
        }
#pragma unroll
        for (int r = 0; r < NRT; r++) tt[r][ct] = mfma_f16(ah[r], bc[0], tt[r][ct]);
        if (blk < XB) load_x_part(sc, left > 2, xc, blk * (8 / XB), 8 / XB);
        const bool conv0 = blk == NBLK - 2, conv1 = blk == NBLK - 1;
        if (conv0) store_b(D, S, E, buf ^ 1, 0);
        if (conv1) store_b(D, S, E, buf ^ 1, 1);
        if constexpr (WIDE) {
          if (blk + 1 < NBLK) __builtin_amdgcn_sched_group_barrier(0x100, 3, 0);
          else __builtin_amdgcn_sched_group_barrier(0x100, 1, 0);
        } else {
          if (blk + 1 < NBLK) __builtin_amdgcn_sched_group_barrier(0x100, 2, 0);
        }
        if (conv0 || conv1) {
#pragma unroll
          for (int k = 0; k < 12; k++) {
            __builtin_amdgcn_sched_group_barrier(0x008, 1, 0);
            __builtin_amdgcn_sched_group_barrier(0x002, 5, 0);
          }
        } else if (blk < XB) {
#pragma unroll
          for (int k = 0; k < 8 / XB; k++) {
            __builtin_amdgcn_sched_group_barrier(0x008, 12 / (8 / XB), 0);
            __builtin_amdgcn_sched_group_barrier(0x002, 2, 0);
            __builtin_amdgcn_sched_group_barrier(0x020, 1, 0);
          }
        } else {
          __builtin_amdgcn_sched_group_barrier(0x008, 12, 0);
        }
      }
    };
    auto tile_end = [&](int t) __attribute__((always_inline)) {
      {
        typedef const unsigned __attribute__((address_space(4))) *ConstWord;
        const bool any_slow = !slow_cur || ((ConstWord)slow_cur)[t] != 0u;
        if (slow_next && blockIdx.y == 0 && blockIdx.z == 0 && threadIdx.x == 0) slow_next[t] = 0u;
        for (int b0 = 0; any_slow && b0 < nobj; b0 += 64) {
          const int ol = opaque_lane();
          const SegDesc db = (P.desc + (size_t)t * P.M)[min(m_lo + b0 + ol, m_hi - 1)];
          unsigned long long multi = __ballot((db.info & (kSegMulti | kSegQuiet)) && b0 + ol < nobj);
          while (multi) {
            const int j = __builtin_ctzll(multi);
            multi &= multi - 1;
            single_object(t, m_lo + b0 + j, x_scale, true, seg_k(__shfl(db.info, j)));
          }
        }
        bool bad = false;
#pragma unroll
        for (int r = 0; r < NRT; r++)
#pragma unroll
          for (int c = 0; c < NCT; c++)
#pragma unroll
            for (int e = 0; e < 4; e++) bad |= !(__builtin_fabsf(tot0[r][c][e]) < INFINITY) || !(__builtin_fabsf(tot1[r][c][e]) < INFINITY);
        if (__ballot(bad)) {
          if (lane == 0) redo_tiles[w] |= 1ull << ka;
          clear_totals();
        } else {
          flush_tile(t, 1.0f / x_scale, true);
        }
        ka++;
      }
    };
    auto advance = [&]() __attribute__((always_inline)) {
      if (sa.c == nch - 1) tile_end(sa.tile);
      sa = sb;
      sb = sc;
      sc = next_stage(sc);
      left--;
    };
#pragma unroll 1
    while (left > 0) {
      chunk(0, X0);
      advance();
      if (left <= 0) break;
      chunk(1, X1);
      advance();
    }
  }
  for (int k = 0; k < my_tiles; k++) {
    if (nch > 0 && !((redo_tiles[w] >> (k & 63)) & 1ull)) continue;
    const int t = tile_at(vb0 + k * vstep);
    if (nch == 0 && slow_next && blockIdx.y == 0 && blockIdx.z == 0 && threadIdx.x == 0) slow_next[t] = 0u;
    for (int m = m_lo; m < m_hi; m++) single_object(t, m, 1.0f, false);
    flush_tile(t, 1.0f, false);
  }
  };
  if constexpr (FORM == 2) {
    if (!wide_cur || (*wide_cur & 1u) != 0u) body(std::true_type{});
    else body(std::false_type{});
  } else {
    body(std::integral_constant<bool, FORM == 1>{});
  }
}

}
```

libear_amd/csrc/gain_kernels.h:

```cpp
#pragma once

#include <hip/hip_runtime.h>

#include <cstdint>

#include "search.h"

namespace earhip {

struct PointRec {
  int64_t time;
  float scale;
  uint32_t flat;
};
static_assert(sizeof(PointRec) == 16, "PointRec is loaded as one dwordx4");

struct ObjHdr {
  int32_t off, cnt;
  int64_t first, last;
  int64_t reserved;
};
static_assert(sizeof(ObjHdr) == 32, "an object's header is two dwordx4 loads");
struct PointStore {
  const ObjHdr *hdr;
  const int32_t *off;
  const int32_t *cnt;
  const int64_t *time;
  const uint8_t *flat;
  const PointRec *rec;
  const float *gain;
  int row;
  int bus_cols;
  int nbus;
  int zero_row;
  int npoints;
  int rows;
  int kink_row0;
  int force_ramp;
};

struct SegDesc {
  int32_t row;
  int32_t d0;
  float scale;
  int32_t info;
};
static_assert(sizeof(SegDesc) == 16, "SegDesc is loaded as one dwordx4");

constexpr int kSegRamp = 1;
constexpr int kSegMulti = 2;
constexpr int kSegQuiet = (int)0x80000000u;
constexpr int kMaxPointsPerObject = (1 << 18) - 1;
static_assert((((unsigned)kMaxPointsPerObject << 13) & (unsigned)kSegQuiet) == 0u, "the segment index must not reach the quiet flag");
__host__ __device__ __forceinline__ int seg_r1(int info) { return (info >> 4) & 0x1ff; }
__host__ __device__ __forceinline__ int seg_k(int info) { return (info >> 13) & 0x3ffff; }


__device__ __forceinline__ int xcd_tile(int b, int n) {
  const int per = n >> 3;
  if (b >= per * 8) return b;
  return (b & 7) * per + (b >> 3);
}

__device__ __forceinline__ SegDesc describe_segment(const PointStore &ps, int base,
                                                    int n, int k, int64_t t0,
                                                    int64_t t_end) {
  SegDesc d;
  if (ps.force_ramp) k = 1;
  const int allflat = (1 << ps.nbus) - 1;
  const int fb = (k > 0 && k < n) ? (ps.flat[base + k] & allflat) : allflat;
  const bool ramp = ps.force_ramp || fb != allflat;
  const bool multi = !ps.force_ramp && k < n && ps.time[base + k] < t_end;
  const int r1 = min((int)((multi ? ps.time[base + k] : t_end) - t0), 511);
  d.info = (k << 13) | (r1 << 4) | (fb << 2) | (multi ? kSegMulti : 0) | (ramp ? kSegRamp : 0);
  if (ramp) {
    const int64_t start = ps.time[base + k - 1], end = ps.time[base + k];
    d.row = base + k - 1;
    d.d0 = (int32_t)(t0 - start);
    d.scale = 1.0f / (float)(end - start);
  } else {
    d.row = base + (k == n ? k - 1 : k);
    d.d0 = 0;
    d.scale = 0.0f;
  }
  return d;
}

__device__ __forceinline__ SegDesc describe_segment_rec(const PointStore &ps, int base, int n, int k, int64_t t0,
                                                        int64_t t_end) {
  if (ps.force_ramp) return describe_segment(ps, base, n, k, t0, t_end);
  const int allflat = (1 << ps.nbus) - 1;
  PointRec r, q;
  r.time = t_end;
  r.scale = 0.0f;
  r.flat = (uint32_t)allflat;
  q = r;
  if (k < n) r = ps.rec[base + k];
  if (k > 0) q = ps.rec[base + k - 1];
  const int fb = (k > 0 && k < n) ? ((int)r.flat & allflat) : allflat;
  const bool ramp = fb != allflat;
  const bool multi = k < n && r.time < t_end;
  const int r1 = min((int)((multi ? r.time : t_end) - t0), 511);
  SegDesc d;
  d.info = (k << 13) | (r1 << 4) | (fb << 2) | (multi ? kSegMulti : 0) | (ramp ? kSegRamp : 0);
  if (ramp) {
    d.row = base + k - 1;
    d.d0 = (int32_t)(t0 - q.time);
    d.scale = r.scale;
  } else {
    d.row = base + (k == n ? k - 1 : k);
    d.d0 = 0;
    d.scale = 0.0f;
  }
  return d;
}

struct LevelProbe {
  const float *in = nullptr;
  size_t in_stride = 0;
  int nsamples = 0;
  int every = 1;
  unsigned *level = nullptr;
  unsigned *obj_level = nullptr;
};
constexpr int kQuietBinades = 20;
constexpr int kPlainBinades = 8;
__host__ __device__ __forceinline__ bool level_is_quiet(unsigned obj_level, unsigned call_level) {
  return obj_level != 0u && call_level != 0u && (int)(obj_level >> 23) < (int)(call_level >> 23) - kQuietBinades;
}
constexpr int kProbeInstants = 64, kProbeObjects = 16;
static __global__ void __launch_bounds__(64 * kProbeObjects)
k_level_probe(const float *in, size_t in_stride, int nsamples, int M, unsigned *level, unsigned *obj_level, int cap, int nruns) {
  __shared__ unsigned wmax[kProbeObjects];
  const int lane = threadIdx.x & 63, wv = threadIdx.x >> 6, m = blockIdx.x * kProbeObjects + wv;
  const int nvec = nsamples >> 2, ninst = min(kProbeInstants, nvec);
  unsigned v = 0u;
  if (m < M && lane < ninst) {
    const unsigned sh = (unsigned)__builtin_ctz((unsigned)nruns), per = 64u >> sh;
    const unsigned nrun = max((unsigned)ninst / per, 1u), g = min((unsigned)lane / per, nrun - 1u), sub = (unsigned)lane & (per - 1u);
    const unsigned stretch = (unsigned)nvec / nrun;
    const unsigned h = ((unsigned)m * 2654435761u) ^ (g * 40503u);
    const unsigned room = stretch > per ? stretch - per + 1u : 1u;
    const int at = (int)min(g * stretch + __umulhi(h, room) + sub, (unsigned)nvec - 1u);
    const float4 px = *reinterpret_cast<const float4 *>(in + (size_t)m * in_stride + 4 * (size_t)at);
    v = max(max(__float_as_uint(px.x) & 0x7fffffffu, __float_as_uint(px.y) & 0x7fffffffu),
            max(__float_as_uint(px.z) & 0x7fffffffu, __float_as_uint(px.w) & 0x7fffffffu));
  }
  unsigned hi_v = v, lo_v = v ? v : 0xffffffffu;
#pragma unroll
  for (int d = 32; d >= 1; d >>= 1) {
    hi_v = max(hi_v, (unsigned)__shfl_xor((int)hi_v, d));
    lo_v = min(lo_v, (unsigned)__shfl_xor((int)lo_v, d));
  }
  if (lane == 0) {
    wmax[wv] = hi_v;
    if (m < M) {
      obj_level[m] = hi_v;
      obj_level[cap + m] = lo_v == 0xffffffffu ? 0u : lo_v;
    }
  }
  __syncthreads();
  if (threadIdx.x == 0) {
    unsigned he = 0u;
#pragma unroll
    for (int i = 0; i < kProbeObjects; i++) he = max(he, wmax[i]);
    he &= 0x7f800000u;
    if (he != 0 && he > __atomic_load_n(level, __ATOMIC_RELAXED)) atomicMax(level, he);
  }
}

constexpr int kHingeSpreadBinades = 16;
constexpr unsigned kGateHingeUnsafe = 2u;
constexpr int kGateQuietShift = 8;
__host__ __device__ __forceinline__ bool hinge_span_exceeded(unsigned word, int M) {
  const int limit = M / 64 > 4 ? M / 64 : 4;
  return (word & kGateHingeUnsafe) != 0u || (int)(word >> kGateQuietShift) > limit;
}
static __global__ void __launch_bounds__(256)
k_hinge_gate(const unsigned *obj_level, int cap, int M, const unsigned *level_cur, unsigned *gate, bool wide, bool count_quiet) {
  const int m = blockIdx.x * 256 + threadIdx.x;
  bool unsafe = false, quiet = false;
  if (m < M) {
    const unsigned hi = obj_level[m], lo = obj_level[cap + m], call = *level_cur;
    const bool exact_anyway = hi != 0u && call != 0u && (int)(hi >> 23) < (int)(call >> 23) - kHingeSpreadBinades;
    unsafe = !exact_anyway && lo != 0u && call != 0u && (int)(lo >> 23) < (int)(call >> 23) - kHingeSpreadBinades;
    quiet = exact_anyway;
  }
  if (__syncthreads_or(unsafe ? 1 : 0) && threadIdx.x == 0) atomicOr(gate, kGateHingeUnsafe);
  if (count_quiet) {
    const int nq = __syncthreads_count(quiet ? 1 : 0);
    if (nq > 0 && threadIdx.x == 0) atomicAdd(gate, (unsigned)nq << kGateQuietShift);
  }
  if (wide) {
    bool wd = false;
    if (m < M) {
      const unsigned lo = obj_level[cap + m], call = *level_cur;
      wd = lo != 0u && call != 0u && (int)(lo >> 23) < (int)(call >> 23) - kPlainBinades;
    }
    if (__syncthreads_or(wd ? 1 : 0) && threadIdx.x == 0) atomicOr(gate, 1u);
  }
}

struct QuietMark {
  const unsigned *obj_level = nullptr;
  int cap = 0;
  const unsigned *level = nullptr;
  unsigned *wide = nullptr;
};
template <int kPrepRun>
// ... 411 lines not shown
```

Before: 1.096 million.

## Add rule form to h2 kernel computing segment descriptors from regular grid rules

Adds a per-object GridRule (first tile, point count, power-of-two spacing) for objects whose points fall on a regular 512-sample grid with uniform ramp segments. When every object is regular and the call is aligned, the h2 kernel derives each SegDesc arithmetically from the rule instead of reading a per-tile descriptor table. The separate descriptor-build and quiet-marking pass is skipped, and the kernel computes quiet and wide flags itself from object levels. This removes the descriptor-build launch and its memory traffic, at the cost of extra per-thread arithmetic, a per-block scan over all objects' levels at startup, and a narrower set of inputs that take the fast path.

```diff
diff --git a/include/earhip.h b/include/earhip.h
--- a/include/earhip.h
+++ b/include/earhip.h
@@ -268,6 +268,7 @@
 int earhip_render_hinge_standby(earhip_render *r, int *standby);
 int earhip_render_hinge_robust(earhip_render *r, int *robust);
 int earhip_render_wide_form(earhip_render *r, int *wide);
+int earhip_render_last_rule(const earhip_render *r, int *rule);
 int earhip_render_last_plan(const earhip_render *r, int out[4]);
 int earhip_render_last_list_layout(const earhip_render *r, int *paired);
 int earhip_render_last_tail_blocks(const earhip_render *r, int *blocks);
diff --git a/libear_amd/capi.py b/libear_amd/capi.py
--- a/libear_amd/capi.py
+++ b/libear_amd/capi.py
@@ -837,6 +837,11 @@
         check(load().earhip_render_wide_form(self.h, C.byref(flag)))
         return None if flag.value < 0 else bool(flag.value)
 
+    def last_rule(self):
+        flag = C.c_int(0)
+        check(load().earhip_render_last_rule(self.h, C.byref(flag)))
+        return bool(flag.value)
+
     def scratch_bytes(self):
         v = C.c_size_t(0)
         check(load().earhip_render_scratch_bytes(self.h, C.byref(v)))
diff --git a/libear_amd/csrc/api_core.hip b/libear_amd/csrc/api_core.hip
--- a/libear_amd/csrc/api_core.hip
+++ b/libear_amd/csrc/api_core.hip
@@ -58,6 +58,9 @@
   unsigned *gate = nullptr;
   ctx->last_gate_idx = -1;
   ctx->last_wide_idx = -1;
+  ctx->last_rule = ml.rule;
+  if (ml.rule && !(ml.split && ml.tile() == kRuleTile && ml.gsplit == 1 && nsamples % kRuleTile == 0 && cs.rule_call(t_call)))
+    fail_internal("rule form planned for a call it does not cover");
   unsigned *const record = ctx->record_slot;
   ctx->record_slot = nullptr;
   const bool hg_robust = ml.hinge && ctx->get(OPT_HG_ROBUST, 1) != 0;
@@ -178,7 +181,7 @@
     EARHIP_BUILD_CASE(1) EARHIP_BUILD_CASE(2) EARHIP_BUILD_CASE(4) EARHIP_BUILD_CASE(8)
 #undef EARHIP_BUILD_CASE
   }
-  if (!fused_prep && !one_pass) {
+  if (!fused_prep && !one_pass && !ml.rule) {
     const dim3 ogrid((M + 15) / 16);
     QuietMark qm;
     if (probe.obj_level) {
@@ -296,7 +299,12 @@
                      gs, level_cur, level_next, slow_cur, slow_next, wide_cur, wide_next);
 #define EARHIP_H2_CASE(NCT_)                                                                                        \
   if (cp.nct == NCT_) {                                                                                             \
-    if (ml.tile() == 512) {                                                                                         \
+    if (ml.rule) {                                                                                                  \
+                         \
+      P.desc = reinterpret_cast<const SegDesc *>(cs.rules());                                                       \
+      hipLaunchKernelGGL((k_gain_mix_h2<NCT_, 8, 3>), bgrid, dim3(64 * 8), 0, ctx->stream, P, ctx->obj_level_cap, xs, \
+                         gs, level_cur, level_next, probe.obj_level, slow_next, wide_cur, wide_next);               \
+    } else if (ml.tile() == 512) {                                                                                  \
       if (wide_cur && !two_launches) EARHIP_H2_LAUNCH(NCT_, 8, 2)                                                   \
       else {                                                                                                        \
         if (wide_cur) EARHIP_H2_LAUNCH(NCT_, 8, 0)                                                                  \
@@ -440,7 +448,7 @@
 
 static const char *const kOptNames[OPT_COUNT] = {
     "SPL", "MFMA", "XSCALE", "WAVES", "TPW", "NRT", "H2_TILE", "H2_WGS", "H2_RUNS", "P2_TILE", "P2_PAIRS", "P2_WGS", "HINGE", "HG_TILE", "HBUILD_TPW",
-    "BUILD_TPW", "K2_WG", "K2_OWN_BLOCK", "RUN", "GSPLIT", "PROBE_RUNS", "BLOCK_GROUPS", "DEBUG_TIMING", "TAILCUT", "HOST_CHUNK_MB", "HOST_THREADS", "HG_ROBUST", "BUILD_2K", "HOST_BIND", "HOST_NT", "HOST_FIRST", "H2_PAIR"};
+    "BUILD_TPW", "K2_WG", "K2_OWN_BLOCK", "RUN", "GSPLIT", "PROBE_RUNS", "BLOCK_GROUPS", "DEBUG_TIMING", "TAILCUT", "HOST_CHUNK_MB", "HOST_THREADS", "HG_ROBUST", "BUILD_2K", "HOST_BIND", "HOST_NT", "HOST_FIRST", "H2_PAIR", "H2_RULE"};
 
 static int parse_option_value(const std::string &key, const char *text) {
   char *end = nullptr;
diff --git a/libear_amd/csrc/api_render.hip b/libear_amd/csrc/api_render.hip
--- a/libear_amd/csrc/api_render.hip
+++ b/libear_amd/csrc/api_render.hip
@@ -263,6 +263,7 @@
   long scratch_regrows = 0;
   DevBuf<unsigned> rec;
   bool last_gated = false;
+  bool last_rule = false;
   bool last_device_form = false;
   bool last_hg_robust = false;
   int last_kind = -1;
@@ -373,7 +374,7 @@
     MixLaunch ml = plan_mix(ctx, curves->plan(), M, nsamples, ctx->strict, max_gsplit, curves->aligned_tile(t),
                             curves->ramp_share(), curves->gain_scale(), curves->point_density_all(), curves->pair_waste(256), curves->pair_waste(512),
                             curves->hinge_exact_share(in_stride, (size_t)nsamples), curves->tiles_aligned(kF32GridTile, t),
-                            curves->deltas_per_pair(256));
+                            curves->deltas_per_pair(256), curves->rule_call(t));
     const size_t bus_stride = ((size_t)nsamples + 3) & ~(size_t)3;
     while (ml.gsplit > 1 && bus_stride * K * N * ml.gsplit > bus.n) ml.gsplit /= 2;
     return ml;
@@ -387,6 +388,11 @@
     for (size_t nb : lens) {
       const MixLaunch ml = plan_call(nb, last_in_stride ? last_in_stride : nb * (size_t)B);
       need = std::max(need, scratch_units(*curves, ml, M));
+      if (ml.rule) {
+        MixLaunch with_desc = ml;
+        with_desc.rule = false;
+        need = std::max(need, scratch_units(*curves, with_desc, M));
+      }
       hinge = hinge || ml.hinge;
     }
     if (hinge) curves->ensure_kinks(ctx);
@@ -463,9 +469,10 @@
           const size_t scratch = last_scratch_bytes;
           const bool gated = last_gated, device_form = last_device_form, hg_robust = last_hg_robust;
           const int paired = last_paired;
+          const bool rule = last_rule;
           process_span(nblocks - main_blocks, in_dev + main_samples, in_stride, out_dev + main_samples, out_stride, true);
           last_kind = kind;
-          last_gated = gated, last_device_form = device_form, last_paired = paired, last_hg_robust = hg_robust;
+          last_gated = gated, last_device_form = device_form, last_paired = paired, last_hg_robust = hg_robust, last_rule = rule;
           for (int i = 0; i < 3; i++) last_plan[i] = plan3[i];
           last_scratch_bytes = scratch;
           last_tail_blocks = (int)(nblocks - main_blocks);
@@ -584,6 +591,7 @@
     if (timed) pending.push_back(pd);
     last_gated = ctx->last_gate_idx >= 0;
     last_device_form = ctx->last_wide_idx >= 0;
+    last_rule = ctx->last_rule;
     last_hg_robust = last_gated && ctx->last_hinge_robust;
     if (ctx->lazy_allocs != lazy_before) scratch_regrows++;
     t += nsamples;
@@ -1339,6 +1347,13 @@
   });
 }
 
+int earhip_render_last_rule(const earhip_render *r, int *rule) {
+  return guarded([&] {
+    require(r != nullptr && rule != nullptr, "NULL argument");
+    *rule = r->last_rule ? 1 : 0;
+  });
+}
+
 int earhip_render_scratch_bytes(const earhip_render *r, size_t *bytes) {
   return guarded([&] {
     require(r != nullptr && bytes != nullptr, "NULL argument");
diff --git a/libear_amd/csrc/common.h b/libear_amd/csrc/common.h
--- a/libear_amd/csrc/common.h
+++ b/libear_amd/csrc/common.h
@@ -117,7 +117,7 @@
   OPT_H2_TILE, OPT_H2_WGS, OPT_H2_RUNS, OPT_P2_TILE, OPT_P2_PAIRS, OPT_P2_WGS, OPT_HINGE, OPT_HG_TILE, OPT_HBUILD_TPW, OPT_BUILD_TPW,
   OPT_K2_WG, OPT_K2_OWN_BLOCK, OPT_RUN, OPT_GSPLIT,
   OPT_PROBE_RUNS, OPT_BLOCK_GROUPS, OPT_DEBUG_TIMING, OPT_TAILCUT, OPT_HOST_CHUNK_MB, OPT_HOST_THREADS, OPT_HG_ROBUST, OPT_BUILD_2K,
-  OPT_HOST_BIND, OPT_HOST_NT, OPT_HOST_FIRST, OPT_H2_PAIR, OPT_COUNT
+  OPT_HOST_BIND, OPT_HOST_NT, OPT_HOST_FIRST, OPT_H2_PAIR, OPT_H2_RULE, OPT_COUNT
 };
 struct OptVal {
   bool set = false;
@@ -142,6 +142,7 @@
   int level_idx = 0;
   int last_gate_idx = -1;
   bool last_hinge_robust = false;
+  bool last_rule = false;
   int last_wide_idx = -1;
   earhip::DevBuf<unsigned> tile_slow;
   size_t tile_slow_cap = 0;
diff --git a/libear_amd/csrc/curves.h b/libear_amd/csrc/curves.h
--- a/libear_amd/csrc/curves.h
+++ b/libear_amd/csrc/curves.h
@@ -49,12 +49,13 @@
   uint8_t *flat;
   PointRec *rec;
   float *gain;
+  GridRule *rule;
 };
 static __global__ void __launch_bounds__(256)
 k_curve_upload(CurveImage src, CurveImage dst, const int32_t *changed, int row) {
   const int m = changed[blockIdx.x];
   const int off = src.off[m], n = src.cnt[m];
-  if (threadIdx.x == 0) dst.off[m] = off, dst.cnt[m] = n, dst.hdr[m] = src.hdr[m];
+  if (threadIdx.x == 0) dst.off[m] = off, dst.cnt[m] = n, dst.hdr[m] = src.hdr[m], dst.rule[m] = src.rule[m];
   for (int i = threadIdx.x; i < n; i += 256) {
     dst.time[off + i] = src.time[off + i];
     dst.flat[off + i] = src.flat[off + i];
@@ -210,8 +211,8 @@
       full_upload = true;
     }
     if (!h_off_.p) {
-      h_off_.reserve(M_), h_cnt_.reserve(M_), h_changed_.reserve(M_), h_gcol_.reserve(row), h_hdr_.reserve(M_);
-      d_off_.alloc(M_), d_cnt_.alloc(M_), d_gcol_.alloc(row), d_hdr_.alloc(M_);
+      h_off_.reserve(M_), h_cnt_.reserve(M_), h_changed_.reserve(M_), h_gcol_.reserve(row), h_hdr_.reserve(M_), h_rule_.reserve(M_);
+      d_off_.alloc(M_), d_cnt_.alloc(M_), d_gcol_.alloc(row), d_hdr_.alloc(M_), d_rule_.alloc(M_);
     }
     EARHIP_LAP(1);
     const float old_scale = gain_scale();
@@ -237,6 +238,7 @@
       o.st = stats_of(o, cm);
       admit(o.st, cm);
       o.has_stats = true;
+      h_rule_.p[m] = o.st.rule;
     }
     if (cmax_shrunk) {
       for (size_t c = 0; c < row; c++) {
@@ -268,14 +270,15 @@
       EARHIP_HIP(hipMemcpyAsync(d_off_.p, h_off_.p, M_ * sizeof(int32_t), hipMemcpyHostToDevice, ctx->stream));
       EARHIP_HIP(hipMemcpyAsync(d_cnt_.p, h_cnt_.p, M_ * sizeof(int32_t), hipMemcpyHostToDevice, ctx->stream));
       EARHIP_HIP(hipMemcpyAsync(d_hdr_.p, h_hdr_.p, M_ * sizeof(ObjHdr), hipMemcpyHostToDevice, ctx->stream));
+      EARHIP_HIP(hipMemcpyAsync(d_rule_.p, h_rule_.p, M_ * sizeof(GridRule), hipMemcpyHostToDevice, ctx->stream));
       EARHIP_HIP(hipMemcpyAsync(d_time_.p, h_time_.p, arena_used_ * sizeof(int64_t), hipMemcpyHostToDevice, ctx->stream));
       EARHIP_HIP(hipMemcpyAsync(d_flat_.p, h_flat_.p, arena_used_, hipMemcpyHostToDevice, ctx->stream));
       EARHIP_HIP(hipMemcpyAsync(d_rec_.p, h_rec_.p, arena_used_ * sizeof(PointRec), hipMemcpyHostToDevice, ctx->stream));
       EARHIP_HIP(hipMemcpyAsync(d_gain_.p, h_gain_.p, arena_used_ * row * sizeof(float), hipMemcpyHostToDevice, ctx->stream));
     } else {
       for (size_t i = 0; i < dirty_list_.size(); i++) h_changed_.p[i] = dirty_list_[i];
-      CurveImage src{h_hdr_.p, h_off_.p, h_cnt_.p, h_time_.p, h_flat_.p, h_rec_.p, h_gain_.p};
-      CurveImage dst{d_hdr_.p, d_off_.p, d_cnt_.p, d_time_.p, d_flat_.p, d_rec_.p, d_gain_.p};
+      CurveImage src{h_hdr_.p, h_off_.p, h_cnt_.p, h_time_.p, h_flat_.p, h_rec_.p, h_gain_.p, h_rule_.p};
+      CurveImage dst{d_hdr_.p, d_off_.p, d_cnt_.p, d_time_.p, d_flat_.p, d_rec_.p, d_gain_.p, d_rule_.p};
       hipLaunchKernelGGL(k_curve_upload, dim3((unsigned)dirty_list_.size()), dim3(256), 0, ctx->stream, src, dst, h_changed_.p,
                          (int)row);
       EARHIP_HIP(hipGetLastError());
@@ -314,6 +317,13 @@
     const int64_t d = t_call >= t_ref_ ? t_call - t_ref_ : t_ref_ - t_call;
     return d % tile == 0 && grid_ % (uint64_t)tile == 0;
   }
+
+  bool all_regular() const { return tot_.irregular == 0 && grid_off_[0] == 0 && !force_ramp_; }
+  bool rule_call(int64_t t_call) const {
+    const int64_t G = kRuleTile, tile = t_call >> kRuleTileLog2;
+    return all_regular() && (((t_call - grid_phase_[0]) % G) + G) % G == 0 && tile > -kRuleMaxTile && tile < kRuleMaxTile;
+  }
+  const GridRule *rules() const { return d_rule_.p; }
 
   int aligned_tile(int64_t t_call) const {
     const int grids[2] = {512, 256};
@@ -400,6 +410,7 @@
     double span = 0, ramp = 0, npts = 0, bad = 0, points = 0;
     double incid[2] = {0, 0}, touched[2] = {0, 0}, tiles[2] = {0, 0};
     int maxr[2] = {0, 0};
+    GridRule rule = {0, 0, 0, 0, 0};
   };
   struct Obj {
     std::vector<int64_t> t;
@@ -433,12 +444,25 @@
       bool same = s.gcd % (uint64_t)G == 0;
       s.phase[gi] = same ? p0 : -1;
     }
+    bool regular = !force_ramp_;
+    int c_log2 = 0;
+    if (n > 1) {
+      const int64_t d0 = t[1] - t[0];
+      while (c_log2 < kRuleMaxSpacingLog2 && ((int64_t)kRuleTile << c_log2) != d0) c_log2++;
+      regular = regular && ((int64_t)kRuleTile << c_log2) == d0;
+    }
     for (size_t k = 1; k < n; k++) {
       const int64_t len = t[k] - t[k - 1];
       const bool is_ramp = (o.flat[k] & allflat) != allflat;
       s.span += (double)len;
       if (is_ramp) s.ramp += (double)len;
       if (len < kHingeMinLen) s.bad += is_ramp ? 1.0 + (double)len / kHingeTile : 0.5;
+      regular = regular && is_ramp && len == ((int64_t)kRuleTile << c_log2);
+    }
+    {
+      const int64_t first_tile = t[0] >> kRuleTileLog2;
+      regular = regular && first_tile > -kRuleMaxTile && first_tile < kRuleMaxTile;
+      s.rule = GridRule{o.off, (int32_t)n, regular ? (int32_t)first_tile : 0, (uint16_t)c_log2, (uint16_t)(regular ? kRuleRegular : 0)};
     }
     if (n > 1) s.npts = (double)(n - 1);
     for (int gi = 0; gi < 2; gi++) {
@@ -486,6 +510,7 @@
   bool retire(const ObjStats &s, const float *cm) {
     tot_.span -= s.span, tot_.ramp -= s.ramp, tot_.npts -= s.npts, tot_.bad -= s.bad, tot_.points -= s.points;
     tot_.moving -= s.npts > 0 ? 1 : 0;
+    tot_.irregular -= (s.rule.flags & kRuleRegular) ? 0 : 1;
     for (int gi = 0; gi < 2; gi++) {
       tot_.incid[gi] -= s.incid[gi], tot_.touched[gi] -= s.touched[gi], tot_.tiles[gi] -= s.tiles[gi];
       tot_.sum_r15[gi] -= std::min(s.maxr[gi], kPieceMaxPerObject), tot_.sum_r7[gi] -= std::min(s.maxr[gi], kPairMaxPerObject);
@@ -502,6 +527,7 @@
   void admit(const ObjStats &s, const float *cm) {
     tot_.span += s.span, tot_.ramp += s.ramp, tot_.npts += s.npts, tot_.bad += s.bad, tot_.points += s.points;
     tot_.moving += s.npts > 0 ? 1 : 0;
+    tot_.irregular += (s.rule.flags & kRuleRegular) ? 0 : 1;
     for (int gi = 0; gi < 2; gi++) {
       tot_.incid[gi] += s.incid[gi], tot_.touched[gi] += s.touched[gi], tot_.tiles[gi] += s.tiles[gi];
       tot_.sum_r15[gi] += std::min(s.maxr[gi], kPieceMaxPerObject), tot_.sum_r7[gi] += std::min(s.maxr[gi], kPairMaxPerObject);
@@ -554,6 +580,7 @@
   struct Totals {
     double span = 0, ramp = 0, npts = 0, bad = 0, points = 0;
     long moving = 0;
+    long irregular = 0;
     double incid[2] = {0, 0}, touched[2] = {0, 0}, tiles[2] = {0, 0};
     long sum_r15[2] = {0, 0}, sum_r7[2] = {0, 0};
   } tot_;
@@ -582,6 +609,8 @@
   DevBuf<int32_t> d_off_, d_cnt_;
   DevBuf<ObjHdr> d_hdr_;
   PinBuf<ObjHdr> h_hdr_;
+  DevBuf<GridRule> d_rule_;
+  PinBuf<GridRule> h_rule_;
   DevBuf<int64_t> d_time_;
   DevBuf<uint8_t> d_flat_;
   DevBuf<PointRec> d_rec_;
@@ -599,6 +628,7 @@
   bool mfma;
   bool split = false;
   bool wide = false;
+  bool rule = false;
   bool pieces = false;
   int pw = 2;
   bool paired = false;
@@ -616,7 +646,7 @@
                           bool strict, int max_gsplit, int aligned_tile = 0, double ramp_share = 1.0,
                           float gain_scale = 0.0f, double point_density = 0.0, double pair_waste256 = 1.0,
                           double pair_waste512 = 1.0, double hinge_exact_share = 2.0, bool grid512_strict = false,
-                          double deltas256 = 0.0) {
+                          double deltas256 = 0.0, bool rule_call = false) {
   const bool aligned = aligned_tile >= 256;
   MixLaunch L;
   L.mfma = !strict && ctx->use_mfma;
@@ -657,6 +687,7 @@
   L.spl = ctx->spl;
   L.nrt = ctx->nrt;
   L.ntiles = (nsamples + L.tile() - 1) / L.tile();
+  L.rule = rule_call && L.split && L.wide && nsamples % kRuleTile == 0 && ctx->get(OPT_H2_RULE, 1) != 0 && ctx->get(OPT_H2_PAIR, 0) == 0;
   if (L.split || L.pieces || L.hinge || L.f32grid) {
     L.wsplit = 1;
     L.tpw = 1;
@@ -664,6 +695,7 @@
     const int nz = cp.mnz * cp.mgroups;
     while (g < max_gsplit && L.ntiles * nz * g < 2 * ctx->num_cus && M / (g * 2) >= 64) g *= 2;
     L.gsplit = g;
+    if (g != 1) L.rule = false;
     return L;
   }
   if (strict) {
@@ -702,6 +734,7 @@
                     piece_units((size_t)M, pnt, (size_t)cs.piece_cap(64 * ml.pw, ml.paired)) + (size_t)M * pnt);
   }
   if (ml.pieces) return piece_units((size_t)M, nt, (size_t)cs.piece_cap(ml.tile(), ml.paired)) + (size_t)M * nt;
+  if (ml.rule) return 1;
   if (ml.split || ml.f32grid || !ml.mfma) return (size_t)M * nt + 1;
   return desc_units((size_t)M, nt);
 }
diff --git a/libear_amd/csrc/gain_h2.h b/libear_amd/csrc/gain_h2.h
--- a/libear_amd/csrc/gain_h2.h
+++ b/libear_amd/csrc/gain_h2.h
@@ -51,7 +51,14 @@
 __global__ void __launch_bounds__(64 * NW, NCT == 1 && NW == 8 ? 2 : (NW == 4 ? 2 : 1))
 k_gain_mix_h2(GainMixParams P, int zero_row, float x_scale, const float *__restrict__ gcol, const unsigned *level_cur,
               unsigned *level_next, const unsigned *slow_cur, unsigned *slow_next, const unsigned *wide_cur, unsigned *wide_next) {
-  if (FORM != 2 && wide_cur && ((*wide_cur & 1u) != 0u) != (FORM == 1)) return;
+  constexpr bool RULE = FORM == 3;
+  static_assert(!RULE || NW == 8, "the rule form exists for the 8-wave kernel that carries both bodies");
+  [[maybe_unused]] bool rule_any_quiet = false, rule_wide = true;
+  [[maybe_unused]] unsigned rule_call_level = 0u;
+  [[maybe_unused]] const unsigned *const obj_level = slow_cur;
+  [[maybe_unused]] const int obj_level_cap = zero_row;
+  if constexpr (RULE) zero_row = P.ps.zero_row;
+  if (FORM < 2 && wide_cur && ((*wide_cur & 1u) != 0u) != (FORM == 1)) return;
   constexpr int NRT = 4, TS = 16 * NRT, CH = kSplitChunk;
   constexpr int NQ = CH / NW;
   constexpr int NFRAG = 2 * NCT * 3;
@@ -76,7 +83,11 @@
   auto tile_at = [&](int vb) { return runs ? min(vb, ntl - 1) : xcd_tile(vb, ntl); };
   if (blockIdx.x == 0 && blockIdx.y == 0 && blockIdx.z == 0 && threadIdx.x == 0) {
     if (wide_next) *wide_next = 0u;
-    record_mode(P, wide_cur != nullptr);
+    if constexpr (RULE) {
+      if (P.record) *P.record = (P.mode_word ? *P.mode_word : 0u) | (rule_wide ? 1u : 0u) | kModeRecorded;
+    } else {
+      record_mode(P, wide_cur != nullptr);
+    }
   }
   if (level_cur) {
     const unsigned lv = *level_cur;
@@ -258,7 +269,8 @@
       SegDesc d[NQ];
     };
     auto load_desc = [&](const Stage &st) {
-      ConstDesc dp = (ConstDesc)(P.desc + (size_t)st.tile * P.M + chunk_base(st.c) + w * NQ);
+      ConstDesc dp = RULE ? (ConstDesc)(P.desc + (chunk_base(st.c) + w * NQ))
+                          : (ConstDesc)(P.desc + (size_t)st.tile * P.M + chunk_base(st.c) + w * NQ);
       ChunkDesc D;
 #pragma unroll
       for (int q = 0; q < NQ; q++) {
@@ -272,11 +284,18 @@
     struct ChunkCoef {
       float p0[NQ], scale[NQ];
     };
-    auto load_gains = [&](const ChunkDesc &R, int cc, ChunkCoef &D, float (&S)[NQ], float (&E)[NQ]) {
+    auto load_gains = [&](const ChunkDesc &R, int cc, [[maybe_unused]] int tile, ChunkCoef &D, float (&S)[NQ], float (&E)[NQ]) {
       const int m0 = chunk_base(cc) + w * NQ;
 #pragma unroll
       for (int q = 0; q < NQ; q++) {
-        const SegDesc d = R.d[q];
+        SegDesc d = R.d[q];
+        if constexpr (RULE) {
+          d = rule_segment(d.row, d.d0, __builtin_bit_cast(int32_t, d.scale), d.info & 0xffff, (int)(P.t_call >> kRuleTileLog2) + tile);
+          if (rule_any_quiet) {
+            typedef const unsigned __attribute__((address_space(4))) *ConstWord;
+            if (level_is_quiet(((ConstWord)obj_level)[m0 + q], rule_call_level)) d.info |= kSegQuiet;
+          }
+        }
         const bool valid = m0 + q >= m_lo + cc * CH && !(d.info & (kSegMulti | kSegQuiet));
         const unsigned rs = (unsigned)(valid ? d.row : zero_row);
         const unsigned re = (valid && (d.info & kSegRamp)) ? (unsigned)d.row + 1u : rs;
@@ -329,7 +348,7 @@
       float S[NQ], E[NQ];
       ChunkCoef D;
       L = load_desc(sa);
-      load_gains(L, 0, D, S, E);
+      load_gains(L, 0, sa.tile, D, S, E);
       load_x(sa, true, X0);
       load_x(sb, left > 1, X1);
       store_b(D, S, E, 0, 0);
@@ -340,7 +359,7 @@
       __syncthreads();
       float S[NQ], E[NQ];
       ChunkCoef D;
-      load_gains(L, sb.c, D, S, E);
+      load_gains(L, sb.c, sb.tile, D, S, E);
       L = load_desc(sc);
       __builtin_amdgcn_sched_barrier(0);
 
@@ -421,10 +440,19 @@
     auto tile_end = [&](int t) __attribute__((always_inline)) {
       {
         typedef const unsigned __attribute__((address_space(4))) *ConstWord;
-        const bool any_slow = !slow_cur || ((ConstWord)slow_cur)[t] != 0u;
+        const bool any_slow = RULE ? rule_any_quiet : (!slow_cur || ((ConstWord)slow_cur)[t] != 0u);
         if (slow_next && blockIdx.y == 0 && blockIdx.z == 0 && threadIdx.x == 0) slow_next[t] = 0u;
         for (int b0 = 0; any_slow && b0 < nobj; b0 += 64) {
           const int ol = opaque_lane();
+          if constexpr (RULE) {
+            unsigned long long quiet = __ballot(level_is_quiet(obj_level[min(m_lo + b0 + ol, m_hi - 1)], rule_call_level) && b0 + ol < nobj);
+            while (quiet) {
+              const int j = __builtin_ctzll(quiet);
+              quiet &= quiet - 1;
+              single_object(t, m_lo + b0 + j, x_scale, true, -1);
+            }
+            continue;
+          }
           const SegDesc db = (P.desc + (size_t)t * P.M)[min(m_lo + b0 + ol, m_hi - 1)];
           unsigned long long multi = __ballot((db.info & (kSegMulti | kSegQuiet)) && b0 + ol < nobj);
           while (multi) {
@@ -473,7 +501,22 @@
     flush_tile(t, 1.0f, false);
   }
   };
-  if constexpr (FORM == 2) {
+  if constexpr (RULE) {
+    if (level_cur && obj_level) {
+      const unsigned call = *level_cur;
+      bool quiet = false, wd = false;
+      for (int m = threadIdx.x & 63; m < P.M; m += 64) {
+        const unsigned hi = obj_level[m], lo = obj_level[obj_level_cap + m];
+        quiet |= level_is_quiet(hi, call);
+        wd |= lo != 0u && call != 0u && (int)(lo >> 23) < (int)(call >> 23) - kPlainBinades;
+      }
+      rule_call_level = call;
+      rule_any_quiet = __ballot(quiet) != 0ull;
+      rule_wide = !wide_cur || __ballot(wd) != 0ull;
+    }
+    if (rule_wide) body(std::true_type{});
+    else body(std::false_type{});
+  } else if constexpr (FORM == 2) {
     if (!wide_cur || (*wide_cur & 1u) != 0u) body(std::true_type{});
     else body(std::false_type{});
   } else {
diff --git a/libear_amd/csrc/gain_kernels.h b/libear_amd/csrc/gain_kernels.h
--- a/libear_amd/csrc/gain_kernels.h
+++ b/libear_amd/csrc/gain_kernels.h
@@ -55,6 +55,31 @@
 __host__ __device__ __forceinline__ int seg_r1(int info) { return (info >> 4) & 0x1ff; }
 __host__ __device__ __forceinline__ int seg_k(int info) { return (info >> 13) & 0x3ffff; }
 
+
+struct GridRule {
+  int32_t row0;
+  int32_t n;
+  int32_t first_tile;
+  uint16_t c_log2;
+  uint16_t flags;
+};
+static_assert(sizeof(GridRule) == 16, "GridRule is loaded as one dwordx4");
+constexpr int kRuleRegular = 1;
+constexpr int kRuleTile = 512, kRuleTileLog2 = 9, kRuleMaxSpacingLog2 = 3;
+constexpr int64_t kRuleMaxTile = (int64_t)1 << 29;
+__host__ __device__ __forceinline__ SegDesc rule_segment(int row0, int n, int first_tile, int c_log2, int at) {
+  const int a = at - first_tile;
+  const int nseg = (n - 1) << c_log2;
+  const bool before = a < 0, ramp = !before && a < nseg;
+  const int km1 = a >> c_log2, r = a & ((1 << c_log2) - 1);
+  const int k = before ? 0 : ramp ? km1 + 1 : n;
+  SegDesc d;
+  d.row = row0 + (before ? 0 : ramp ? km1 : n - 1);
+  d.d0 = ramp ? r << kRuleTileLog2 : 0;
+  d.scale = ramp ? __builtin_bit_cast(float, (uint32_t)(127 - kRuleTileLog2 - c_log2) << 23) : 0.0f;
+  d.info = (k << 13) | (511 << 4) | (ramp ? kSegRamp : 0);
+  return d;
+}
 
 __device__ __forceinline__ int xcd_tile(int b, int n) {
   const int per = n >> 3;
```

After: 1.041 million. -5.0%, worse.
